# antonilo/unsupervised_detection

Measured on AMD Instinct MI355X. Metric: frame-pairs/sec per adversarial step, DAVIS 480p batch4, 1/2/4/8 GPU, higher is better.
Workload: dtype f32

## Files before the change

include/udet_debug.h:

```cpp
#ifndef UDET_DEBUG_H
#define UDET_DEBUG_H
#include <stddef.h>
#ifdef __cplusplus
extern "C" {
#endif
void udet_debug_force_conv(int bm, int bn, int ks);
void udet_debug_conv_fp16(int on);
void udet_debug_conv_fp16_grad_scale(float s);
void udet_debug_force_wgrad(int nsplit, int dma);
int udet_debug_last_wgrad(void);
int udet_debug_last_wgrad_reduce(void);
int udet_debug_conv2d_backward_filter_ex(const float* x, int ldx, int x_coff, const float* dy, int ldy, int y_coff, const float* y_saved, int act,
                                         float alpha, const float* w, const float* b, const float* gamma, float bn_c, float* dw, float* db,
                                         float* dgamma, float* dbeta, int n, int h, int wd, int cin, int cout, int k, int stride, int dilation,
                                         int up, void* workspace, size_t workspace_bytes, void* stream);
void udet_debug_upb_min_pixels(long v);
void udet_debug_set_tuning(int on);
void udet_debug_force_pair(int on);
int udet_debug_last_pair(void);
int udet_debug_conv2d_pair(const float* xa, const float* xb, const float* wa, const float* wb, const float* ba, const float* bb, float* ya, float* yb,
                           int na, int nb, int h, int w, int cin, int cout, int k, int stride, int dilation, int act, float alpha, void* workspace,
                           size_t workspace_bytes, void* stream);
#define UDET_DEBUG_UPCONV_WSETS_OFFSET 6400
size_t udet_debug_upconv_lowres_workspace_bytes(int ldx, int cin, int cout);
int udet_debug_upconv_lowres_fwd(const float* x, int ldx, const float* w, const float* bias, int act, float alpha, float* y, int ldy, int y_coff,
                                 float* xhat, int n, int h, int wd, int cin, int cout, int split, void* workspace, size_t workspace_bytes,
                                 void* stream);
int udet_debug_upconv_lowres_bwd(const float* dy, int ldy, int y_coff, const float* w, float* dx, int ldx, float* dxhat, int n, int h, int wd,
                                 int cin, int cout, void* workspace, size_t workspace_bytes, void* stream);
int udet_debug_upconv_tables(int h, int w, int backward, int* nseg, int* seg, int* seg_tap, int* taps, int taps_cap, int* ntaps);
int udet_debug_max_segs(void);
int udet_debug_last_conv(void);
#ifdef __cplusplus
}
#endif
#endif
```

unsupervised_detection_amd/_devel.py:

```python
from __future__ import annotations

import ctypes
import os

from ._ffi import check as _check, lib as _lib

_PATH = os.path.join(os.path.dirname(os.path.abspath(__file__)), "libudet_debug.so")
if not os.path.exists(_PATH):
    raise RuntimeError(f"{_PATH} is missing: build it with `make -C unsupervised_detection_amd/csrc`")
dbg = ctypes.CDLL(_PATH, mode=ctypes.RTLD_GLOBAL)
dbg.udet_debug_force_conv.restype = None
dbg.udet_debug_force_conv.argtypes = [ctypes.c_int, ctypes.c_int, ctypes.c_int]
dbg.udet_debug_last_conv.restype = ctypes.c_int
dbg.udet_debug_last_conv.argtypes = []
dbg.udet_debug_conv_fp16.restype = None
dbg.udet_debug_conv_fp16.argtypes = [ctypes.c_int]
dbg.udet_debug_conv_fp16_grad_scale.restype = None
dbg.udet_debug_conv_fp16_grad_scale.argtypes = [ctypes.c_float]
dbg.udet_debug_force_wgrad.restype = None
dbg.udet_debug_force_wgrad.argtypes = [ctypes.c_int, ctypes.c_int]
dbg.udet_debug_upb_min_pixels.restype = None
dbg.udet_debug_upb_min_pixels.argtypes = [ctypes.c_long]
dbg.udet_debug_set_tuning.restype = None
dbg.udet_debug_set_tuning.argtypes = [ctypes.c_int]
dbg.udet_debug_last_wgrad.restype = ctypes.c_int
dbg.udet_debug_last_wgrad.argtypes = []
dbg.udet_debug_force_pair.restype = None
dbg.udet_debug_force_pair.argtypes = [ctypes.c_int]
dbg.udet_debug_last_pair.restype = ctypes.c_int
dbg.udet_debug_last_pair.argtypes = []
dbg.udet_debug_conv2d_pair.restype = ctypes.c_int
dbg.udet_debug_conv2d_pair.argtypes = [ctypes.c_void_p] * 8 + [ctypes.c_int] * 10 + [ctypes.c_float, ctypes.c_void_p, ctypes.c_size_t, ctypes.c_void_p]
dbg.udet_debug_last_wgrad_reduce.restype = ctypes.c_int
dbg.udet_debug_last_wgrad_reduce.argtypes = []
_p, _i, _f = ctypes.c_void_p, ctypes.c_int, ctypes.c_float
dbg.udet_debug_conv2d_backward_filter_ex.restype = ctypes.c_int
dbg.udet_debug_conv2d_backward_filter_ex.argtypes = ([_p, _i, _i, _p, _i, _i, _p, _i, _f, _p, _p, _p, _f, _p, _p, _p, _p] + [_i] * 9
                                                     + [_p, ctypes.c_size_t, _p])
UPCONV_WSETS_OFFSET = 6400
dbg.udet_debug_upconv_lowres_workspace_bytes.restype = ctypes.c_size_t
dbg.udet_debug_upconv_lowres_workspace_bytes.argtypes = [_i, _i, _i]
dbg.udet_debug_upconv_lowres_fwd.restype = ctypes.c_int
dbg.udet_debug_upconv_lowres_fwd.argtypes = [_p, _i, _p, _p, _i, _f, _p, _i, _i, _p] + [_i] * 6 + [_p, ctypes.c_size_t, _p]
dbg.udet_debug_upconv_lowres_bwd.restype = ctypes.c_int
dbg.udet_debug_upconv_lowres_bwd.argtypes = [_p, _i, _i, _p, _p, _i, _p] + [_i] * 5 + [_p, ctypes.c_size_t, _p]
dbg.udet_debug_upconv_tables.restype = ctypes.c_int
dbg.udet_debug_upconv_tables.argtypes = [_i, _i, _i] + [_p] * 4 + [_i, _p]
dbg.udet_debug_max_segs.restype = ctypes.c_int
dbg.udet_debug_max_segs.argtypes = []


def upconv_tables(h: int, w: int, backward: bool):
    cap = 1024
    nseg, ntaps = ctypes.c_int(0), ctypes.c_int(0)
    seg, seg_tap, taps = (ctypes.c_int * 64)(), (ctypes.c_int * 17)(), (ctypes.c_int * (3 * cap))()
    st = dbg.udet_debug_upconv_tables(h, w, 1 if backward else 0, ctypes.addressof(nseg), ctypes.addressof(seg), ctypes.addressof(seg_tap),
                                      ctypes.addressof(taps), cap, ctypes.addressof(ntaps))
    _check(st)
    ns, nt = nseg.value, ntaps.value
    return dict(nseg=ns, seg=[tuple(seg[4 * s:4 * s + 4]) for s in range(ns)], seg_tap=list(seg_tap[:ns + 1]),
                taps=[tuple(taps[3 * t:3 * t + 3]) for t in range(nt)])
```

unsupervised_detection_amd/csrc/common.h:

```cpp
#pragma once
#include <hip/hip_runtime.h>
#include <hip/hip_ext.h>
#include <stdint.h>
#include <stdio.h>
#include <string>

#include "../../include/udet.h"

namespace udet {

void set_error(const char* fmt, ...);
int hip_fail(hipError_t e, const char* what);
#define UDET_HIP(x)                                   \
  do {                                                \
    hipError_t _e = (x);                              \
    if (_e != hipSuccess) return udet::hip_fail(_e, #x); \
  } while (0)
#define UDET_TRY(x)            \
  do {                         \
    int _s = (x);              \
    if (_s != 0) return _s;    \
  } while (0)

struct LaunchSink {
  hipEvent_t* ev;
  int n, cap;
};
extern thread_local LaunchSink* g_launch_sink;
bool launch_sink_next(hipEvent_t* a, hipEvent_t* b);
#define UDET_LAUNCH(kernel, grid, block, shmem, stream, ...)                                             \
  do {                                                                                                   \
    hipEvent_t ea_, eb_;                                                                                 \
    if (udet::g_launch_sink && udet::launch_sink_next(&ea_, &eb_))                                       \
      hipExtLaunchKernelGGL(kernel, grid, block, shmem, stream, ea_, eb_, 0, __VA_ARGS__);               \
    else                                                                                                 \
      hipLaunchKernelGGL(kernel, grid, block, shmem, stream, __VA_ARGS__);                               \
  } while (0)

enum Act { ACT_NONE = UDET_ACT_NONE, ACT_LEAKY = UDET_ACT_LEAKY, ACT_ELU = UDET_ACT_ELU };

__device__ __forceinline__ float elu_negative(float v) {
  const float e = __expf(v) - 1.0f;
  const float t = v * (1.f + v * (0.5f + v * (0.16666667f + v * (0.041666668f + v * (0.0083333338f + v * 0.0013888889f)))));
  return v > -0.25f ? t : e;
}
__device__ __forceinline__ float act_fwd(float v, int act, float alpha) {
  const float slope = act == ACT_LEAKY ? alpha : 1.f;
  float r = v > 0.f ? v : v * slope;
  if (act == ACT_ELU) r = v > 0.f ? v : elu_negative(v);
  return r;
}
__device__ __forceinline__ float act_dfo(float a, int act, float alpha) {
  const float ue = act == ACT_ELU ? 1.f : 0.f, us = act == ACT_LEAKY ? alpha : 1.f;
  return a > 0.f ? 1.f : fmaf(a, ue, us);
}

#define UDET_MAX_TAPS 49
struct ConvTap {
  int dy, dx, widx;
};

struct FastDiv {
  unsigned d, mul, sh;
};
inline FastDiv make_fastdiv(unsigned d) {
  FastDiv f;
  f.d = d; f.mul = 0; f.sh = 0;
  if (d > 1) {
    unsigned l = 0;
    while ((1u << l) < d) ++l;
    const unsigned long long pw = 1ull << (31 + l);
    f.mul = (unsigned)((pw + d - 1) / d);
    f.sh = l - 1;
  }
  return f;
}
__device__ __forceinline__ unsigned fdiv(unsigned n, const FastDiv& f) { return f.d == 1 ? n : (__umulhi(n, f.mul) >> f.sh); }

__host__ __device__ __forceinline__ constexpr int xcd_tile_order(int bid, int nwg) {
  const int q = nwg >> 3, r = nwg & 7, xcd = bid & 7, idx = bid >> 3;
  return (xcd < r ? xcd * (q + 1) : r * (q + 1) + (xcd - r) * q) + idx;
}
constexpr bool xcd_tile_order_permutes(int nwg) {
  unsigned long long seen = 0;
  for (int b = 0; b < nwg; ++b) {
    const int l = xcd_tile_order(b, nwg);
    if (l < 0 || l >= nwg || ((seen >> l) & 1)) return false;
    seen |= 1ull << l;
  }
  return true;
}
static_assert(xcd_tile_order_permutes(1) && xcd_tile_order_permutes(7) && xcd_tile_order_permutes(8), "xcd_tile_order");
static_assert(xcd_tile_order_permutes(9) && xcd_tile_order_permutes(13) && xcd_tile_order_permutes(64), "xcd_tile_order");
static_assert(xcd_tile_order(1, 13) == 2 && xcd_tile_order(8, 13) == 1 && xcd_tile_order(5, 13) == 10, "xcd 0..4 of 13 hold two tiles, 5..7 one");

struct ConvSeg {
  int oy, ox;
  int h, w;
  int prow0;
  FastDiv fd_hw, fd_w;
};
#define UDET_MAX_SEGS 16

struct ConvParams {
  const float* x;
  int ldx, x_coff;
  int N, H, W;
  int up_shift;
  const float* xa;
  int xact;
  float xalpha;
  const float* wp;
  int Kc, ldw;
  const float* bias;
  float* y;
  int ldy, y_coff, Cout;
  int OH, OW;
  int OHq, OWq;
  int osy, osx, ooy, oox;
  int isy, isx;
  int ntaps;
  ConvTap taps[UDET_MAX_TAPS];
  int ncls;
  int cls_tap[5];
  int nseg;
  ConvSeg seg[UDET_MAX_SEGS];
  int seg_tap[UDET_MAX_SEGS + 1];
  const ConvTap* tap_tab;
  int Mall;
  FastDiv fd_ohw, fd_ow;
  int kfast;
  const float* zero16;
  int act;
  float alpha;
  const float* res;
  int ldres, res_coff;
  float* y2;
  int ldy2, y2_coff;
  int accumulate;
  float* uo;
  int ldu, u_coff;
  const float* ua;
  int ldua, ua_coff, uact;
  float ualpha;
  int u_c0, u_c1;
  int ksplit;
  float* partial;
  size_t partial_cap;
  int ldp;
  int fold;
  int* tickets;
  int tail_full, tail_ks, tail_prow0;
  int f16;
  float f16_xscale;
  const float* wino_u;
  int wino_np;
  int kreal;
};
#define UDET_MAX_TICKETS 4096

int launch_conv(ConvParams& p, hipStream_t stream);
int launch_conv_pair(ConvParams& a, ConvParams& b, hipStream_t stream);
int launch_tap_gather(const ConvParams& g, const float* z, int ldz, hipStream_t stream);

struct PackJob {
  long src_off, dst_off, gamma_off, beta_off;
  long total;
  int T, R, C, Kc, ldw, k_split, k_gap, mode;
};

struct WgradParams {
  const float* x;
  int ldx, x_coff;
  int N, H, W, up_shift;
  int Cin;
  const float* dy;
  const float* ya;
  int ldy, y_coff, Cout;
  int yact;
  float yalpha;
  int OH, OW, isy, isx;
  int ycls, OHf, OWf;
  int ntaps;
  ConvTap taps[UDET_MAX_TAPS];
  float* dw;
  float* db;
  float* partial;
  size_t partial_floats;
  const float* zero16;
  int swapped, oCin, oCout, bias_m;
  int Cin4, Mpad;
  float* pbias;
  FastDiv fd_ohw, fd_ow;
  const float* w;
  const float* b;
  const float* gamma;
  float* dgamma;
  float* dbeta;
  float bn_c;
  int f16;
  float f16_yscale;
};
int launch_wgrad_T(WgradParams& p, int T, hipStream_t stream);
int launch_wgrad_up_T(const WgradParams& q, int H, int W, hipStream_t stream);
int launch_bn_finalize(float* dw, int T, int Cin, int Cout, const float* w, const float* b, const float* gamma, float bn_c, float* pd,
                       float* db, float* dgamma, float* dbeta, hipStream_t stream);
int launch_wgrad_up_combine(const float* deff, float* dw, int Cin, int Cout, hipStream_t stream);
size_t wgrad_partial_floats_needed(int T, int Cin, int Cout);

}
```

unsupervised_detection_amd/csrc/conv_igemm.hip:

```cpp
#include "conv_igemm_common.h"

namespace udet {

#define UDET_TILE_ROW(BM, BN, WM, WN) {BM, BN},
const int CONV_GEMM_TILES[CONV_GEMM_NTILES][2] = {UDET_GEMM_TILES(UDET_TILE_ROW)};
#undef UDET_TILE_ROW
bool conv_gemm_tile(int bm, int bn) {
  for (auto& t : CONV_GEMM_TILES)
    if (bm == t[0] && bn == t[1]) return true;
  return false;
}

int conv_xblocks(const ConvParams& p, int bm) {
  if (p.nseg == 0) return p.ncls * ((p.N * p.OHq * p.OWq + bm - 1) / bm);
  int x = 0;
  for (int s = 0; s < p.nseg; ++s) x += (p.N * p.seg[s].h * p.seg[s].w + bm - 1) / bm;
  return x;
}

static int launch_cfg(ConvParams& p, const ConvCfg& c, hipStream_t stream) {
  const int Mtot = p.N * p.OHq * p.OWq;
  dim3 grid(conv_xblocks(p, c.bm), (p.Cout + c.bn - 1) / c.bn, p.ksplit > 1 ? p.ksplit : 1);
  if (p.tail_ks > 1) {
    const int mtiles = (Mtot + c.bm - 1) / c.bm;
    p.tail_prow0 = (p.tail_full / mtiles) * Mtot + (p.tail_full % mtiles) * c.bm;
    grid.x = p.tail_full + (grid.x - p.tail_full) * p.tail_ks;
    grid.z = 1;
  }
  if (c.family == FAM_SELF_STAGING) UDET_TRY(launch_igemm_self(p, c.bm, c.bn, p.f16 != 0, grid, stream));
  else if (is_lds_dma(c.family)) UDET_TRY(launch_igemm_ring(p, c.bm, c.bn, c.family == FAM_DMA2 ? 2 : (c.family == FAM_DMA3 ? 3 : 4), p.f16 != 0, grid, stream));
  else UDET_TRY(launch_igemm_staged(p, c.bm, c.bn, c.family != FAM_PLAIN, grid, stream));
  if (p.tail_ks > 1) UDET_TRY(launch_splitk_tail_pass(p, stream));
  else if (p.ksplit > 1 && !p.fold) UDET_TRY(launch_splitk_second_pass(p, stream));
  return UDET_OK;
}

static int launch_pair_cfg(ConvParams& a, ConvParams& b, const ConvCfg& c, hipStream_t stream) {
  ConvPair pp;
  pp.p[0] = a; pp.p[1] = b;
  pp.xa = conv_xblocks(a, c.bm);
  dim3 grid(pp.xa + conv_xblocks(b, c.bm), (a.Cout + c.bn - 1) / c.bn, a.ksplit > 1 ? a.ksplit : 1);
  UDET_TRY(launch_igemm_ring_pair(pp, c.bm, c.bn, c.family == FAM_DMA3 ? 3 : 2, grid, stream));
  if (a.ksplit > 1) UDET_TRY(launch_splitk_pair_pass(pp, stream));
  return UDET_OK;
}

int launch_conv_gemm(ConvParams& p, const ConvCfg& c, hipStream_t stream) {
  if (!conv_gemm_tile(c.bm, c.bn)) return no_gemm_tile("conv", c.bm, c.bn);
  p.ksplit = c.ks > 1 ? c.ks : 1;
  p.fold = 0;
  p.tail_full = 0; p.tail_ks = 0; p.tail_prow0 = 0;
  if (p.ksplit > 1) {
    p.ldp = (p.Cout + 3) & ~3;
    p.fold = c.fold && p.tickets && cfg_tiles(p, c.bm, c.bn) <= UDET_MAX_TICKETS;
    const int Mtot = p.N * p.OHq * p.OWq, mtiles = (Mtot + c.bm - 1) / c.bm, xb = p.ncls * mtiles;
    if (c.tail > 0 && c.tail < xb && !p.nseg && is_lds_dma(c.family) && !(reinterpret_cast<uintptr_t>(p.partial) & 15)) {
      const long prow0 = (long)(c.tail / mtiles) * Mtot + (long)(c.tail % mtiles) * c.bm;
      if ((size_t)((long)p.ncls * Mtot - prow0) * p.ldp * p.ksplit <= p.partial_cap) {
        p.tail_full = c.tail; p.tail_ks = p.ksplit; p.ksplit = 1; p.fold = 0;
      }
    }
  }
  return launch_cfg(p, c, stream);
}

int launch_conv_gemm_pair(ConvParams& a, ConvParams& b, const ConvCfg& c, hipStream_t stream) {
  if (!conv_gemm_tile(c.bm, c.bn)) return no_gemm_tile("conv pair", c.bm, c.bn);
  const int cap = pair_max_ksplit(a, b);
  const int ks = c.ks > cap ? cap : (c.ks < 1 ? 1 : c.ks);
  for (ConvParams* q : {&a, &b}) {
    q->ksplit = ks; q->fold = 0; q->tail_full = 0; q->tail_ks = 0; q->tail_prow0 = 0;
    q->ldp = (q->Cout + 3) & ~3;
  }
  float* const base = a.partial;
  if (ks > 1) {
    if ((reinterpret_cast<uintptr_t>(base) & 15) != 0) { set_error("conv pair: unaligned split-K scratch"); return UDET_ERR_ALIGN; }
    size_t off = (size_t)ks * a.Mall * a.ldp;
    off = (off + 15) & ~(size_t)15;
    b.partial = base + off;
  }
  const int rc = launch_pair_cfg(a, b, c, stream);
  b.partial = base;
  return rc;
}

}
```

unsupervised_detection_amd/csrc/conv_igemm_ring.h:

```cpp
#pragma once
#include "conv_igemm_common.h"

namespace udet {

template <int BM, int BN, int WAVES_M, int WAVES_N, int NS, bool F16>
__device__ __forceinline__ void conv_igemm_dma_body(const ConvParams& p, const int bid_x, const int grid_x) {
  static_assert(NS >= 2 && NS <= 4, "stages");
  static_assert(WAVES_M * WAVES_N == 4, "4 MFMA waves");
  constexpr int BK = 32;
  constexpr int WTM = BM / WAVES_M, WTN = BN / WAVES_N;
  constexpr int TM = WTM / 32, TN = WTN / 32;
  static_assert(TM * 32 == WTM && TN * 32 == WTN && BM % 32 == 0, "tile");
  constexpr int A_LD = BM / 32;
  constexpr int B_F4_ROW = BN / 4;
  constexpr int B_LD = BK * B_F4_ROW / 256;
  static_assert(B_LD * 256 == BK * B_F4_ROW, "BK*BN/4 must be a multiple of 256");
  typedef __attribute__((address_space(3))) void* lds_ptr;

  __shared__ __attribute__((aligned(16))) float As[NS][BM][BK];
  __shared__ __attribute__((aligned(16))) float Bs[NS][BK][BN];
  __shared__ int rowoff[BM];
  __shared__ int2 tap_yx[UDET_MAX_TAPS];
  __shared__ int tap_w[UDET_MAX_TAPS];
  __shared__ int s_last;

  IGEMM_STAMP(0);
  const int tid = threadIdx.x;
  int spec_dy = 0, spec_dx = 0, spec_widx = 0;
  if (tid < UDET_MAX_TAPS) {
    spec_dy = p.taps[tid].dy;
    spec_dx = p.taps[tid].dx;
    spec_widx = p.taps[tid].widx;
  }
  const int role = __builtin_amdgcn_readfirstlane(tid >> 8);
  const int t = tid & 255;
  const int lane = t & 63, wave = __builtin_amdgcn_readfirstlane(t >> 6);
  const int wm = wave / WAVES_N, wn = wave % WAVES_N;
  const int li = lane & 31, lh = lane >> 5;

  int bid = bid_x;
  int kz = blockIdx.z, knz = p.ksplit;
  {
    int nwg = grid_x;
    if (p.tail_ks > 1) {
      nwg = p.tail_full;
      knz = 1;
      if (bid >= p.tail_full) {
        const int r = bid - p.tail_full;
        kz = r % p.tail_ks;
        bid = p.tail_full + r / p.tail_ks;
        knz = p.tail_ks;
      }
    }
    if (bid < nwg) {
      const int q = nwg >> 3, r = nwg & 7, xcd = bid & 7, idx = bid >> 3;
      bid = (xcd < r ? xcd * (q + 1) : r * (q + 1) + (xcd - r) * q) + idx;
    }
  }
  const TileCls tc = tile_cls<BM>(p, bid);
  const int OHWq = tc.OHWq, Mtot = tc.Mtot , m0 = tc.m0, tap0 = tc.tap0, ntc = tc.ntc, ooy = tc.ooy, oox = tc.oox;
  const int n0 = blockIdx.y * BN;
  const int Hs = p.H >> p.up_shift, Ws = p.W >> p.up_shift;
  IGEMM_STAMP(6);

  if (p.nseg == 0 && tap0 == 0) {
    if (tid < ntc) {
      tap_yx[tid] = make_int2(spec_dy, spec_dx);
      tap_w[tid] = spec_widx;
    }
  } else {
    for (int i = tid; i < ntc; i += 512) {
      const ConvTap tp = conv_tap(p, tap0 + i);
      tap_yx[i] = make_int2(tp.dy, tp.dx);
      tap_w[i] = tp.widx;
    }
  }
  const int Kc = p.Kc;
  const int tsh = Kc == 4 ? 3 : (Kc == 8 ? 2 : 1);
  const int tps = (p.kfast & 4) ? 1 << tsh : 1;
  const int nchunks = (p.kfast & 1) ? ntc * ((Kc + 31) >> 5) : ((p.kfast & 4) ? (ntc + tps - 1) >> tsh : (ntc * Kc + BK - 1) / BK);
  int c_begin = 0, c_end = nchunks;
  if (knz > 1) {
    c_begin = (int)((unsigned)(nchunks * kz) / (unsigned)knz);
    c_end = (int)((unsigned)(nchunks * (kz + 1)) / (unsigned)knz);
  }
  const long slab_off = p.tail_ks > 1 ? ((long)kz * (p.Mall - p.tail_prow0) - p.tail_prow0) * p.ldp : (long)kz * p.Mall * p.ldp;
  IGEMM_STAMP(7);

  if (role == 1) {
    __builtin_amdgcn_s_setprio(3);
    const int kq = lane & 7;
    const int kqs = kq ^ ((wave * 4 + (lane >> 4)) & 7);
    int a_base[A_LD], a_iy0[A_LD], a_ix0[A_LD];
#pragma unroll
    for (int j = 0; j < A_LD; ++j) {
      const int m = m0 + j * 32 + wave * 8 + (lane >> 3);
      if (m < Mtot) {
        const int n = (int)fdiv(m, tc.fd_ohw), rem = m - n * OHWq;
        const int qy = (int)fdiv(rem, tc.fd_ow), qx = rem - qy * tc.OWq;
        a_base[j] = n * Hs * Ws;
        a_iy0[j] = qy * p.isy;
        a_ix0[j] = qx * p.isx;
      } else {
        a_base[j] = 0;
        a_iy0[j] = -(1 << 28);
        a_ix0[j] = 0;
      }
    }
    const float* zero = p.zero16;
    const KOrder ko = korder(Kc, ntc);
    KCursor ka, kb[B_LD];
    ka.blk = ka.tap = ka.c = ka.w = 0;
#pragma unroll
    for (int j = 0; j < B_LD; ++j) kb[j] = ka;
    if (!(p.kfast & 5)) {
      ka = kc_init(ko, c_begin * BK + kqs * 4);
#pragma unroll
      for (int j = 0; j < B_LD; ++j) kb[j] = kc_init(ko, c_begin * BK + (t + j * 256) / B_F4_ROW);
    }
    auto issue_generic = [&](int buf) {
      int dy = 0, dx = 0;
      const bool a_ok = kc_valid(ko, ka);
      const int a_c = kc_chan(ko, ka);
      if (a_ok) {
        const int2 yx = tap_yx[ka.tap];
        dy = yx.x;
        dx = yx.y;
      }
#pragma unroll
      for (int j = 0; j < A_LD; ++j) {
        int iy = a_iy0[j] + dy, ix = a_ix0[j] + dx;
        const bool ok = a_ok && (unsigned)iy < (unsigned)p.H && (unsigned)ix < (unsigned)p.W;
        iy >>= p.up_shift;
        ix >>= p.up_shift;
        const float* src = ok ? p.x + ((size_t)(a_base[j] + iy * Ws + ix) * p.ldx + p.x_coff + a_c) : zero;
        __builtin_amdgcn_global_load_lds(src, (lds_ptr)&As[buf][j * 32 + wave * 8][0], 16, 0, 0);
      }
#pragma unroll
      for (int j = 0; j < B_LD; ++j) {
        const int c4 = (t + j * 256) % B_F4_ROW;
        const int n = n0 + c4 * 4;
        const bool ok = kc_valid(ko, kb[j]) && n < p.ldw;
        const int wi = ok ? tap_w[kb[j].tap] : 0;
        const float* src = ok ? p.wp + (((size_t)wi * Kc + kc_chan(ko, kb[j])) * p.ldw + n) : zero;
        __builtin_amdgcn_global_load_lds(src, (lds_ptr)(&Bs[buf][0][0] + (j * 256 + wave * 64) * 4), 16, 0, 0);
      }
      kc_advance(ko, ka, BK);
#pragma unroll
      for (int j = 0; j < B_LD; ++j) kc_advance(ko, kb[j], BK);
    };
    int a_off[A_LD];
#pragma unroll
    for (int j = 0; j < A_LD; ++j)
      a_off[j] = a_iy0[j] < -(1 << 27) ? 0 : (a_base[j] + a_iy0[j] * Ws + a_ix0[j]) * p.ldx + p.x_coff + kqs * 4;
    int b_off[B_LD], b_row[B_LD];
    bool b_col[B_LD];
#pragma unroll
    for (int j = 0; j < B_LD; ++j) {
      const int idx = t + j * 256, row = idx / B_F4_ROW, n = n0 + (idx - row * B_F4_ROW) * 4;
      b_row[j] = row;
      b_off[j] = row * p.ldw + n;
      b_col[j] = n < p.ldw;
    }
    int s_blk = c_begin == 0 ? 0 : __builtin_amdgcn_readfirstlane(c_begin / (ntc > 0 ? ntc : 1));
    int s_tap = __builtin_amdgcn_readfirstlane(c_begin - s_blk * ntc);
    auto issue_fast = [&](int buf) {
      const int2 yx = tap_yx[s_tap];
      const int dy = yx.x, dx = yx.y, c0 = s_blk << 5;
      const int tap_off = (dy * Ws + dx) * p.ldx + c0;
      const bool ch_ok = c0 + kqs * 4 < Kc;
#pragma unroll
      for (int j = 0; j < A_LD; ++j) {
        const int iy = a_iy0[j] + dy, ix = a_ix0[j] + dx;
        const bool ok = ch_ok && (unsigned)iy < (unsigned)p.H && (unsigned)ix < (unsigned)p.W;
        const float* src = ok ? p.x + (a_off[j] + tap_off) : zero;
        __builtin_amdgcn_global_load_lds(src, (lds_ptr)&As[buf][j * 32 + wave * 8][0], 16, 0, 0);
      }
      const float* wrow = p.wp + ((size_t)tap_w[s_tap] * Kc + c0) * p.ldw;
#pragma unroll
      for (int j = 0; j < B_LD; ++j) {
        const bool ok = b_col[j] && c0 + b_row[j] < Kc;
        const float* src = ok ? wrow + b_off[j] : zero;
        __builtin_amdgcn_global_load_lds(src, (lds_ptr)(&Bs[buf][0][0] + (j * 256 + wave * 64) * 4), 16, 0, 0);
      }
      if (++s_tap == ntc) { s_tap = 0; ++s_blk; }
    };
    const int ksh = Kc == 4 ? 2 : (Kc == 8 ? 3 : 4);
    const int a_sub = (kqs * 4) >> ksh, a_ch = (kqs * 4) - (a_sub << ksh);
    int b_sub[B_LD], b_poff[B_LD];
#pragma unroll
    for (int j = 0; j < B_LD; ++j) {
      b_sub[j] = b_row[j] >> ksh;
      b_poff[j] = (b_row[j] - (b_sub[j] << ksh)) * p.ldw + (b_off[j] - b_row[j] * p.ldw);
    }
    auto issue_pack = [&](int buf, int s_stage) {
      const int ta = s_stage * tps + a_sub;
      const bool ta_ok = ta < ntc;
      const int2 yx = tap_yx[ta_ok ? ta : 0];
      const int dy = yx.x, dx = yx.y;
      const int tap_off = (dy * Ws + dx) * p.ldx + a_ch - kqs * 4;
#pragma unroll
      for (int j = 0; j < A_LD; ++j) {
        const int iy = a_iy0[j] + dy, ix = a_ix0[j] + dx;
        const bool ok = ta_ok && (unsigned)iy < (unsigned)p.H && (unsigned)ix < (unsigned)p.W;
        const float* src = ok ? p.x + (a_off[j] + tap_off) : zero;
        __builtin_amdgcn_global_load_lds(src, (lds_ptr)&As[buf][j * 32 + wave * 8][0], 16, 0, 0);
      }
#pragma unroll
      for (int j = 0; j < B_LD; ++j) {
        const int tb = s_stage * tps + b_sub[j];
        const bool ok = b_col[j] && tb < ntc;
        const float* src = ok ? p.wp + ((size_t)tap_w[ok ? tb : 0] * Kc * p.ldw + b_poff[j]) : zero;
        __builtin_amdgcn_global_load_lds(src, (lds_ptr)(&Bs[buf][0][0] + (j * 256 + wave * 64) * 4), 16, 0, 0);
      }
// ... 136 lines not shown
```

unsupervised_detection_amd/csrc/conv_igemm_self.hip:

```cpp
#include "conv_igemm_dma.h"

namespace udet {

template <int BM, int BN, int WAVES_M, int WAVES_N, bool F16 = false>
__global__ __launch_bounds__(256, 3) void conv_igemm_dma4_kernel(const ConvParams p) {
  static_assert(WAVES_M * WAVES_N == 4, "4 waves");
  constexpr int BK = 16;
  constexpr int WTM = BM / WAVES_M, WTN = BN / WAVES_N;
  constexpr int TM = WTM / 32, TN = WTN / 32;
  static_assert(TM * 32 == WTM && TN * 32 == WTN && BM % 64 == 0 && BN % 32 == 0, "tile");
  using Lane = DmaLane<BM, BN, BK>;
  constexpr int B_LD = Lane::B_LD;

  __shared__ __attribute__((aligned(16))) float As[2][BM][BK];
  __shared__ __attribute__((aligned(16))) float Bs[2][BK][BN];
  __shared__ int rowoff[BM];
  __shared__ int2 tap_yx[UDET_MAX_TAPS];
  __shared__ int tap_w[UDET_MAX_TAPS];
  __shared__ int s_last;

  const int t = threadIdx.x;
  const int lane = t & 63, wave = __builtin_amdgcn_readfirstlane(t >> 6);
  const int wm = wave / WAVES_N, wn = wave % WAVES_N;
  const int li = lane & 31, lh = lane >> 5;

  const int bid = xcd_tile_order(blockIdx.x, gridDim.x);
  const TileCls tc = tile_cls<BM>(p, bid);
  const int Mtot = tc.Mtot , m0 = tc.m0, ntc = tc.ntc;
  const int n0 = blockIdx.y * BN;
  const int Hs = p.H >> p.up_shift, Ws = p.W >> p.up_shift;

  fill_tap_tables<256>(p, tc, tap_yx, tap_w, t);
  fill_rowoff<BM, 256>(p, tc, rowoff, t);
  const int Kc = p.Kc;
  const bool kfast = (p.kfast & 2) != 0;
  const int nchunks = kfast ? ntc * ((Kc + 15) >> 4) : (ntc * Kc + BK - 1) / BK;
  int c_begin, c_end;
  k_slice(nchunks, blockIdx.z, p.ksplit, c_begin, c_end);
  __syncthreads();

  Lane ln;
  dma_lane_init(ln, p, tc, t, lane, wave, n0, Hs, Ws);
  const KOrder ko = korder(Kc, ntc);
  ln.ka = kc_init(ko, kfast ? 0 : c_begin * BK + ln.kqs * 4);
#pragma unroll
  for (int j = 0; j < B_LD; ++j) ln.kb[j] = kc_init(ko, kfast ? 0 : c_begin * BK + (t + j * 256) / Lane::B_F4_ROW);
  const int ntc_ = ntc > 0 ? ntc : 1;
  int s_blk = __builtin_amdgcn_readfirstlane(c_begin / ntc_);
  int s_tap = __builtin_amdgcn_readfirstlane(c_begin - s_blk * ntc_);
  auto issue = [&](int buf) {
    if (kfast) dma_issue_fast<true>(p, ln, tap_yx, tap_w, As, Bs, buf, ntc, s_blk, s_tap);
    else dma_issue_generic<true>(p, ln, ko, tap_yx, tap_w, As, Bs, buf);
  };
  auto meet = [&]() {
    asm volatile("s_waitcnt vmcnt(0) lgkmcnt(0)" ::: "memory");
    __builtin_amdgcn_s_barrier();
    asm volatile("" ::: "memory");
  };

  floatx16 acc[TM][TN];
  acc_zero(acc);
  const float xscale = F16 ? p.f16_xscale : 1.f;

  if (c_begin < c_end) issue(0);
  meet();
  {
    int buf = 0;
    for (int c = c_begin; c < c_end; ++c) {
      if (c + 1 < c_end) issue(buf ^ 1);
      dma_compute_chunk<TM, TN, WTM, WTN, F16>(As, Bs, buf, acc, wm, wn, li, lh, xscale);
      meet();
      buf ^= 1;
    }
  }
  if constexpr (F16) acc_unscale(acc, xscale);
  igemm_store<TM, TN, WTM, WTN>(p, acc, rowoff, wm, wn, li, lh, n0, tc.prow0 + m0, Mtot, p.ksplit > 1,
                                (long)blockIdx.z * p.Mall * p.ldp, xpose_scratch<sizeof(As), sizeof(Bs)>(&As[0][0][0], &Bs[0][0][0], wave));
  if (p.ksplit > 1 && p.fold) splitk_fold<BM, BN, 256>(p, rowoff, &s_last, t, n0, tc.prow0 + m0, Mtot, blockIdx.y * gridDim.x + bid);
}

constexpr int self_waves_m(int bm, int bn) { return (bm % 64 == 0 && bn % 64 == 0 && bm <= 128) ? 2 : ((bn == 32 && bm % 128 == 0) ? 4 : 0); }
template <int BM, int BN, bool F16>
static void launch_self(const ConvParams& p, dim3 grid, hipStream_t stream) {
  constexpr int WM = self_waves_m(BM, BN);
  if constexpr (WM != 0) UDET_LAUNCH((conv_igemm_dma4_kernel<BM, BN, WM, 4 / WM, F16>), grid, dim3(256), 0, stream, p);
}
bool conv_self_staging_tile(int bm, int bn) { return conv_gemm_tile(bm, bn) && self_waves_m(bm, bn) != 0; }

int launch_igemm_self(const ConvParams& p, int bm, int bn, bool f16, dim3 grid, hipStream_t stream) {
  if (!conv_self_staging_tile(bm, bn)) {
    set_error("conv: no self-staging kernel for tile %dx%d", bm, bn);
    return UDET_ERR_UNSUPPORTED;
  }
#define UDET_TILE_LAUNCH(BM, BN, WM, WN)          \
  if (bm == BM && bn == BN) {                     \
    if (f16) launch_self<BM, BN, true>(p, grid, stream); \
    else launch_self<BM, BN, false>(p, grid, stream);    \
  }
  UDET_GEMM_TILES(UDET_TILE_LAUNCH)
#undef UDET_TILE_LAUNCH
  UDET_HIP(hipGetLastError());
  return UDET_OK;
}

}
```

unsupervised_detection_amd/csrc/conv_igemm_staged.hip:

```cpp
#include "conv_igemm_common.h"

namespace udet {

template <int BM, int BN, int BK, int WAVES_M, int WAVES_N, bool WS>
__global__ __launch_bounds__(WS ? 512 : 256, WS ? 4 : 2) void conv_igemm_kernel(const ConvParams p) {
  static_assert(WAVES_M * WAVES_N == 4, "4 waves");
  constexpr int NT = WS ? 512 : 256;
  constexpr int WTM = BM / WAVES_M, WTN = BN / WAVES_N;
  constexpr int TM = WTM / 32, TN = WTN / 32;
  static_assert(TM * 32 == WTM && TN * 32 == WTN, "wave tile must be a multiple of 32");
  constexpr int KQ = BK / 4;
  constexpr int LDA = BM + 32 / BK;
  constexpr int A_ROWS = 256 / KQ;
  constexpr int A_LD = BM / A_ROWS;
  static_assert(A_LD * A_ROWS == BM, "BM must be a multiple of 256/(BK/4)");
  constexpr int B_F4_ROW = BN / 4;
  constexpr int B_LD = BK * B_F4_ROW / 256;
  static_assert(B_LD * 256 == BK * B_F4_ROW, "BK*BN/4 must be a multiple of 256");

  __shared__ __attribute__((aligned(16))) float As[2][BK][LDA];
  __shared__ __attribute__((aligned(16))) float Bs[2][BK][BN];
  __shared__ int rowoff[BM];
  __shared__ int2 tap_yx[UDET_MAX_TAPS];
  __shared__ int tap_w[UDET_MAX_TAPS];
  __shared__ int s_last;

  const int tid = threadIdx.x;
  const int role = __builtin_amdgcn_readfirstlane(tid >> 8);
  const int t = tid & 255;
  const int lane = t & 63, wave = t >> 6;
  const int wm = wave / WAVES_N, wn = wave % WAVES_N;
  const int li = lane & 31, lh = lane >> 5;

  int bid = blockIdx.x;
  {
    const int nwg = gridDim.x, q = nwg >> 3, r = nwg & 7, xcd = bid & 7, idx = bid >> 3;
    bid = (xcd < r ? xcd * (q + 1) : r * (q + 1) + (xcd - r) * q) + idx;
  }
  const TileCls tc = tile_cls<BM>(p, bid);
  const int OHWq = tc.OHWq, Mtot = tc.Mtot , m0 = tc.m0, tap0 = tc.tap0, ntc = tc.ntc, ooy = tc.ooy, oox = tc.oox;
  const int n0 = blockIdx.y * BN;
  const int Hs = p.H >> p.up_shift, Ws = p.W >> p.up_shift;

  for (int i = tid; i < ntc; i += NT) {
    const ConvTap tp = conv_tap(p, tap0 + i);
    tap_yx[i] = make_int2(tp.dy, tp.dx);
    tap_w[i] = tp.widx;
  }
  for (int r = tid; r < BM; r += NT) {
    const int m = m0 + r;
    int off = -1;
    if (m < Mtot) {
      const int n = (int)fdiv(m, tc.fd_ohw), rem = m - n * OHWq;
      const int qy = (int)fdiv(rem, tc.fd_ow), qx = rem - qy * tc.OWq;
      off = (n * p.OH + qy * p.osy + ooy) * p.OW + qx * p.osx + oox;
    }
    rowoff[r] = off;
  }
  const int a_kq = t % KQ;
  int a_base[A_LD], a_iy0[A_LD], a_ix0[A_LD];
#pragma unroll
  for (int j = 0; j < A_LD; ++j) {
    const int r = t / KQ + j * A_ROWS;
    const int m = m0 + r;
    if (m < Mtot) {
      const int n = (int)fdiv(m, tc.fd_ohw), rem = m - n * OHWq;
      const int qy = (int)fdiv(rem, tc.fd_ow), qx = rem - qy * tc.OWq;
      a_base[j] = n * Hs * Ws;
      a_iy0[j] = qy * p.isy;
      a_ix0[j] = qx * p.isx;
    } else {
      a_base[j] = 0;
      a_iy0[j] = -(1 << 28);
      a_ix0[j] = 0;
    }
  }

  floatx16 acc[TM][TN];
#pragma unroll
  for (int i = 0; i < TM; ++i)
#pragma unroll
    for (int j = 0; j < TN; ++j)
#pragma unroll
      for (int r = 0; r < 16; ++r) acc[i][j][r] = 0.f;

  const int Kc = p.Kc;
  const int nchunks = (ntc * Kc + BK - 1) / BK;
  int c_begin = 0, c_end = nchunks;
  if (p.ksplit > 1) {
    c_begin = (int)((unsigned)(nchunks * blockIdx.z) / (unsigned)p.ksplit);
    c_end = (int)((unsigned)(nchunks * (blockIdx.z + 1)) / (unsigned)p.ksplit);
  }
  const KOrder ko = korder(Kc, ntc);
  KCursor ka = kc_init(ko, c_begin * BK + a_kq * 4), kb[B_LD];
#pragma unroll
  for (int j = 0; j < B_LD; ++j) kb[j] = kc_init(ko, c_begin * BK + (t + j * 256) / B_F4_ROW);
  __syncthreads();

  float4 ra[A_LD], rb[B_LD];
  auto load_chunk = [&]() {
    int dy = 0, dx = 0;
    const bool a_ok = kc_valid(ko, ka);
    const int a_c = kc_chan(ko, ka);
    if (a_ok) {
      const int2 yx = tap_yx[ka.tap];
      dy = yx.x;
      dx = yx.y;
    }
#pragma unroll
    for (int j = 0; j < A_LD; ++j) {
      int iy = a_iy0[j] + dy, ix = a_ix0[j] + dx;
      const bool ok = a_ok && (unsigned)iy < (unsigned)p.H && (unsigned)ix < (unsigned)p.W;
      float4 v = make_float4(0.f, 0.f, 0.f, 0.f);
      if (ok) {
        iy >>= p.up_shift;
        ix >>= p.up_shift;
        const size_t off = (size_t)(a_base[j] + iy * Ws + ix) * p.ldx + p.x_coff + a_c;
        v = *reinterpret_cast<const float4*>(p.x + off);
        if (p.xa) {
          const float4 a = *reinterpret_cast<const float4*>(p.xa + off);
          v.x *= act_dfo(a.x, p.xact, p.xalpha);
          v.y *= act_dfo(a.y, p.xact, p.xalpha);
          v.z *= act_dfo(a.z, p.xact, p.xalpha);
          v.w *= act_dfo(a.w, p.xact, p.xalpha);
        }
      }
      ra[j] = v;
    }
#pragma unroll
    for (int j = 0; j < B_LD; ++j) {
      const int c4 = (t + j * 256) % B_F4_ROW;
      const int n = n0 + c4 * 4;
      float4 v = make_float4(0.f, 0.f, 0.f, 0.f);
      if (kc_valid(ko, kb[j]) && n < p.ldw)
        v = *reinterpret_cast<const float4*>(p.wp + ((size_t)tap_w[kb[j].tap] * Kc + kc_chan(ko, kb[j])) * p.ldw + n);
      rb[j] = v;
    }
    kc_advance(ko, ka, BK);
#pragma unroll
    for (int j = 0; j < B_LD; ++j) kc_advance(ko, kb[j], BK);
  };
  auto store_chunk = [&](int buf) {
#pragma unroll
    for (int j = 0; j < A_LD; ++j) {
      const int r = t / KQ + j * A_ROWS;
      As[buf][a_kq * 4 + 0][r] = ra[j].x;
      As[buf][a_kq * 4 + 1][r] = ra[j].y;
      As[buf][a_kq * 4 + 2][r] = ra[j].z;
      As[buf][a_kq * 4 + 3][r] = ra[j].w;
    }
#pragma unroll
    for (int j = 0; j < B_LD; ++j) {
      const int idx = t + j * 256;
      const int krow = idx / B_F4_ROW, c4 = idx - krow * B_F4_ROW;
      *reinterpret_cast<float4*>(&Bs[buf][krow][c4 * 4]) = rb[j];
    }
  };

  auto compute_chunk = [&](int buf) {
    float a[2][TM], b[2][TN];
    auto frag = [&](int s, int kk) {
#pragma unroll
      for (int i = 0; i < TM; ++i) a[s][i] = As[buf][kk * 2 + lh][wm * WTM + i * 32 + li];
#pragma unroll
      for (int j = 0; j < TN; ++j) b[s][j] = Bs[buf][kk * 2 + lh][wn * WTN + j * 32 + li];
    };
    frag(0, 0);
#pragma unroll
    for (int kk = 0; kk < BK / 2; ++kk) {
      if (kk + 1 < BK / 2) frag((kk + 1) & 1, kk + 1);
#pragma unroll
      for (int i = 0; i < TM; ++i)
#pragma unroll
        for (int j = 0; j < TN; ++j)
          acc[i][j] = __builtin_amdgcn_mfma_f32_32x32x2f32(a[kk & 1][i], b[kk & 1][j], acc[i][j], 0, 0, 0);
      if (kk + 1 < BK / 2) __builtin_amdgcn_sched_group_barrier(0x100, TM + TN, 0);
      __builtin_amdgcn_sched_group_barrier(0x008, TM * TN, 0);
    }
  };

  if constexpr (WS) {
    auto handover = [&]() {
      asm volatile("s_waitcnt lgkmcnt(0)" ::: "memory");
      __builtin_amdgcn_s_barrier();
    };
    if (role == 1) {
      __builtin_amdgcn_s_setprio(3);
      if (c_begin < c_end) {
        load_chunk();
        store_chunk(0);
        if (c_begin + 1 < c_end) load_chunk();
      }
      handover();
      int buf = 0;
// ... 53 lines not shown
```

unsupervised_detection_amd/csrc/conv_select.hip:

```cpp
#include <mutex>

#include "common.h"
#include "conv_select.h"

namespace udet {

struct TileGeoms;
size_t conv_tile_lds_bytes(const ConvParams& p, int th, int cbmax, TileGeoms* gout, bool* big);
int launch_conv_tile(const ConvParams& p, int th, int cbmax, hipStream_t stream);

static int max_class_taps(const ConvParams& p) {
  int mx = 0;
  for (int c = 0; c < p.nseg; ++c) mx = p.seg_tap[c + 1] - p.seg_tap[c] > mx ? p.seg_tap[c + 1] - p.seg_tap[c] : mx;
  if (p.nseg) return mx;
  for (int c = 0; c < p.ncls; ++c) mx = p.cls_tap[c + 1] - p.cls_tap[c] > mx ? p.cls_tap[c + 1] - p.cls_tap[c] : mx;
  return mx;
}
static int ksplit_capacity(const ConvParams& p, size_t floats_per_split) {
  const int nchunks = (max_class_taps(p) * p.Kc + 31) / 32;
  int ks = nchunks / 2 > 64 ? 64 : nchunks / 2;
  while (ks > 1 && floats_per_split * ks > p.partial_cap) --ks;
  return ks < 1 ? 1 : ks;
}
int max_ksplit(const ConvParams& p) { return p.partial ? ksplit_capacity(p, (size_t)p.Mall * ((p.Cout + 3) & ~3)) : 1; }
int pair_max_ksplit(const ConvParams& a, const ConvParams& b) { return ksplit_capacity(a, ((size_t)a.Mall + b.Mall) * ((a.Cout + 3) & ~3) + 64); }
bool tile_ok(const ConvParams& p, int th, int cb) {
  if (p.nseg) return false;
  if (cb == 16 && p.Kc <= 16) return false;
  const size_t b = conv_tile_lds_bytes(p, th, cb, nullptr, nullptr);
  return b > 0 && b <= 96 * 1024 && p.Kc <= 256 && p.Cout <= 256;
}
bool dma_ok(const ConvParams& p) { return p.xa == nullptr && p.zero16 != nullptr && !(reinterpret_cast<uintptr_t>(p.zero16) & 15); }
bool tail_for_rounds(const ConvParams& p, int bm, int bn, int r, int kcap, int* full_x, int* ks) {
  if (p.nseg) return false;
  const int Mtot = p.N * p.OHq * p.OWq, X = p.ncls * ((Mtot + bm - 1) / bm), Y = (p.Cout + bn - 1) / bn;
  const long S = 256L * r, T = (long)X * Y, fullT = T / S * S;
  if (fullT == 0 || fullT == T) return false;
  const int fx = (int)(fullT / Y), rem_x = X - fx;
  if (fx <= 0 || rem_x <= 0) return false;
  long k = S / ((long)rem_x * Y);
  if (k > kcap) k = kcap;
  if (k < 2) return false;
  *full_x = fx;
  *ks = (int)k;
  return true;
}

static int heuristic_ksplit(long tiles, int cap) {
  const int ks = (int)((512 + tiles - 1) / tiles), half = cap / 2 > 0 ? cap / 2 : 1;
  return ks > half ? half : ks;
}
ConvCfg heuristic_cfg(const ConvParams& p) {
  ConvCfg c;
  c.family = FAM_WAVE_SPEC; c.tail = 0;
  if (p.Cout <= 32) { c.bn = 32; c.bm = 256; if (cfg_tiles(p, 256, 32) < 384) c.bm = 128; }
  else if (p.Cout <= 64) { c.bn = 64; c.bm = 128; if (cfg_tiles(p, 128, 64) < 384) c.bm = 64; }
  else if (p.Cout <= 96) { c.bn = 96; c.bm = 128; }
  else { c.bn = 128; c.bm = 128; if (cfg_tiles(p, 128, 128) < 320) { c.bn = 64; if (cfg_tiles(p, 128, 64) < 384) c.bm = 64; } }
  const long tiles = cfg_tiles(p, c.bm, c.bn);
  c.ks = tiles < 256 ? heuristic_ksplit(tiles, max_ksplit(p)) : 1;
  c.fold = 0;
  if (p.f16 && dma_ok(p)) c.family = FAM_DMA2;
  return c;
}
static ConvCfg pair_heuristic(const ConvParams& a, const ConvParams& b) {
  ConvCfg c = heuristic_cfg(b.Mall >= a.Mall ? b : a);
  c.family = FAM_DMA2; c.fold = 0; c.tail = 0;
  const long tiles = cfg_tiles(a, c.bm, c.bn) + cfg_tiles(b, c.bm, c.bn);
  c.ks = tiles < 256 ? heuristic_ksplit(tiles, pair_max_ksplit(a, b)) : 1;
  return c;
}

int run_conv_cfg(ConvParams& p, const ConvCfg& c, hipStream_t stream) {
  if (is_direct(c.family)) {
    p.ksplit = 1; p.fold = 0; p.tail_full = 0; p.tail_ks = 0;
    return c.family == FAM_THIN_K ? launch_conv_thin_k(p, stream) : launch_conv_thin_n(p, stream);
  }
  if (c.family == FAM_WINO) return launch_conv_wino(p, c.wino_variant(), c.ks, stream);
  if (c.family == FAM_TILE) {
    p.ksplit = 1;
    p.fold = 0;
    return launch_conv_tile(p, c.tile_height(), c.tile_channels(), stream);
  }
  return launch_conv_gemm(p, c, stream);
}

static ConvCfg runnable_cfg(const ConvParams& p, ConvCfg c) {
  const bool known = c.family == FAM_TILE ? (c.bm == 4 || c.bm == 8) && (c.bn == 16 || c.bn == 32)
                     : c.family == FAM_WINO ? c.bm >= 0 && c.bm <= 4
                     : is_direct(c.family) || (is_gemm(c.family) && conv_gemm_tile(c.bm, c.bn));
  if (!known) return heuristic_cfg(p);
  const int cap = c.family == FAM_WINO ? 16 : max_ksplit(p);
  if (c.ks < 1) c.ks = 1;
  if (c.ks > cap) { c.ks = cap; c.tail = 0; }
  c.fold = c.fold && p.tickets ? 1 : 0;
  if (c.tail < 0) c.tail = 0;
  if (stages_by_dma(c.family) && !dma_ok(p)) c.family = FAM_WAVE_SPEC;
  if (c.family == FAM_SELF_STAGING && !conv_self_staging_tile(c.bm, c.bn)) c.family = FAM_DMA2;
  if (p.f16 && dma_ok(p) && (c.family == FAM_PLAIN || c.family == FAM_WAVE_SPEC)) c.family = FAM_DMA2;
  if (is_direct(c.family) && (p.f16 || !(c.family == FAM_THIN_K ? conv_thin_k_ok(p) : conv_thin_n_ok(p)))) return heuristic_cfg(p);
  if (c.family == FAM_TILE && !tile_ok(p, c.tile_height(), c.tile_channels())) return heuristic_cfg(p);
  if (c.family == FAM_WINO && (!conv_wino_ok(p) || !conv_wino_variant_ok(p, c.wino_variant()))) return heuristic_cfg(p);
  return c;
}

struct ConvForce {
  int bm = 0, bn = 0, ks = -1, family = -1, fold = -1, tail_rounds = 0;
  bool any() const { return bm || family >= 0 || ks >= 0; }
};
static ConvForce g_force;
void conv_force_config(int bm, int bn, int ks) {
  ConvForce f;
  f.bm = bm & 0xffff; f.bn = bn;
  f.ks = ks < 0 ? ks : (ks & 0xff);
  f.tail_rounds = ks < 0 ? 0 : ((ks >> 8) & 0xff);
  f.fold = (bm >> 20) & 1 ? 0 : ((bm >> 21) & 1 ? 1 : -1);
  static const int BITS[][2] = {{16, FAM_PLAIN}, {17, FAM_DMA2}, {18, FAM_TILE}, {19, FAM_SELF_STAGING},
                                {22, FAM_DMA3}, {23, FAM_DMA4}, {24, FAM_THIN_K}, {25, FAM_WINO}};
  for (auto& b : BITS)
    if (f.family < 0 && ((bm >> b[0]) & 1)) f.family = b[1];
  g_force = f;
}
static void wino_operands_from_packed(ConvParams& p, hipStream_t stream) {
  int d9, w9[9];
  if (p.wino_u || p.f16 || p.xa || p.Kc % 8 != 0 || p.Kc < 8 || !conv_wino_geometry(p, &d9, w9)) return;
  static float* g_wino_scratch = nullptr;
  static size_t g_wino_cap = 0;
  static std::mutex mu;
  std::lock_guard<std::mutex> l(mu);
  const int np9 = conv_wino_np(p.Cout);
  const size_t need = (size_t)(p.Kc / 8) * 16 * 2 * np9 * 4;
  if (need > g_wino_cap) {
    (void)hipStreamSynchronize(stream);
    if (g_wino_scratch) (void)hipFree(g_wino_scratch);
    g_wino_scratch = nullptr; g_wino_cap = 0;
    if (hipMalloc(reinterpret_cast<void**>(&g_wino_scratch), need * sizeof(float)) == hipSuccess) g_wino_cap = need;
  }
  if (g_wino_scratch && launch_wino_from_packed(p, g_wino_scratch, np9, stream) == UDET_OK) { p.wino_u = g_wino_scratch; p.wino_np = np9; }
}
static void apply_forced(ConvParams& p, ConvCfg& c, hipStream_t stream) {
  const ConvForce& f = g_force;
  if (f.bm && f.family != FAM_WINO) { c.bm = f.bm; c.bn = f.bn; }
  if (f.ks >= 0) { c.ks = (f.ks > max_ksplit(p) && f.family != FAM_WINO) ? max_ksplit(p) : f.ks; c.tail = 0; }
  if (f.family >= 0) c.family = f.family;
  if (f.fold >= 0) c.fold = f.fold;
  if (f.tail_rounds > 0) {
    int fx = 0, k = 0;
    if (tail_for_rounds(p, c.bm, c.bn, f.tail_rounds, max_ksplit(p), &fx, &k)) { c.tail = fx; c.ks = c.ks >= 2 ? c.ks : k; c.fold = 0; }
  }
  if (f.family == FAM_TILE) { c.bm = f.bm == 4 ? 4 : 8; c.bn = f.bn == 16 ? 16 : 32; }
  if (f.family == FAM_THIN_K) c.family = conv_thin_k_ok(p) ? FAM_THIN_K : (conv_thin_n_ok(p) ? FAM_THIN_N : heuristic_cfg(p).family);
  if (f.family == FAM_WINO) {
    wino_operands_from_packed(p, stream);
    const int v = (f.bm & 7) == 4 ? 4 : (f.bm & 3);
    if (conv_wino_ok(p) && (conv_wino_variant_ok(p, v) || conv_wino_variant_ok(p, v ^ 1))) {
      c = ConvCfg::wino(conv_wino_variant_ok(p, v) ? v : (v ^ 1), f.ks < 0 ? 1 : c.ks);
    } else c = heuristic_cfg(p);
  }
}

static int g_debug_f16 = 0;
void conv_debug_f16(int on) { g_debug_f16 = on; }
int conv_debug_f16_on() { return g_debug_f16; }
static float g_debug_f16_grad_scale = 0.f;
void conv_debug_f16_grad_scale(float s) { g_debug_f16_grad_scale = s > 0.f ? s : 0.f; }
float conv_debug_f16_grad_scale_now() { return g_debug_f16 ? g_debug_f16_grad_scale : 0.f; }
static int conv_prepare(ConvParams& p) {
  if (g_debug_f16) p.f16 = 1;
  if (p.f16 && !(p.f16_xscale > 0.f)) p.f16_xscale = 1.f;
  if (p.f16 && conv_tuning_on()) p.f16_xscale = 1.f;
  if (p.Kc % 4 != 0 || p.ldx % 4 != 0 || p.x_coff % 4 != 0 || p.ldw % 4 != 0) {
    set_error("conv: Kc=%d ldx=%d x_coff=%d ldw=%d violate the 4-float alignment contract", p.Kc, p.ldx, p.x_coff, p.ldw);
    return UDET_ERR_ALIGN;
  }
  if (p.ntaps < 0 || p.ntaps > UDET_MAX_TAPS) {
    set_error("conv: ntaps=%d out of range", p.ntaps);
    return UDET_ERR_SHAPE;
  }
  if ((reinterpret_cast<uintptr_t>(p.x) | reinterpret_cast<uintptr_t>(p.wp)) & 15) {
    set_error("conv: x / packed weights must be 16-byte aligned");
    return UDET_ERR_ALIGN;
  }
  if (p.nseg) {
    if (p.nseg < 0 || p.nseg > UDET_MAX_SEGS || !p.tap_tab || p.up_shift || p.xa) {
      set_error("conv: malformed segmented launch");
      return UDET_ERR_ARG;
    }
    int prow = 0;
    for (int s = 0; s < p.nseg; ++s) {
      ConvSeg& g = p.seg[s];
      if (g.h < 1 || g.w < 1 || p.seg_tap[s + 1] - p.seg_tap[s] > UDET_MAX_TAPS || p.seg_tap[s + 1] < p.seg_tap[s]) {
        set_error("conv: segment %d is empty or has more than %d taps", s, UDET_MAX_TAPS);
        return UDET_ERR_SHAPE;
      }
      g.prow0 = prow;
      prow += p.N * g.h * g.w;
      g.fd_hw = make_fastdiv((unsigned)(g.h * g.w));
      g.fd_w = make_fastdiv((unsigned)g.w);
    }
    p.Mall = prow;
    p.ncls = 1; p.ntaps = 0; p.cls_tap[0] = p.cls_tap[1] = 0;
    p.OHq = p.seg[0].h; p.OWq = p.seg[0].w;
  } else {
    if (p.ncls != 4) {
      p.ncls = 1;
      p.cls_tap[0] = 0;
      p.cls_tap[1] = p.ntaps;
    }
    p.Mall = p.ncls * p.N * p.OHq * p.OWq;
  }
  p.fd_ohw = make_fastdiv((unsigned)(p.OHq * p.OWq));
  p.fd_ow = make_fastdiv((unsigned)p.OWq);
  p.kfast = 0;
  if (p.up_shift == 0) p.kfast = p.Kc >= 32 ? 3 : ((p.Kc >= 16 ? 2 : 0) | ((p.Kc == 4 || p.Kc == 8 || p.Kc == 16) ? 4 : 0));
  return UDET_OK;
}
static int g_last_cfg = 0;
int conv_last_config() { return g_last_cfg; }
static int config_word(const ConvCfg& c) { return (c.family & 0xff) | ((c.bm & 0xfff) << 8) | ((c.ks & 0xff) << 20); }

int launch_conv(ConvParams& p, hipStream_t stream) {
  UDET_TRY(conv_prepare(p));
  ConvCfg c;
  const uint64_t key = conv_key(p);
  if (!conv_cache_find(key, &c)) {
    if (conv_tuning_on()) {
      c = tune_conv(p, key, stream);
    } else {
      c = heuristic_cfg(p);
      if (!g_force.bm && !p.f16 && conv_thin_n_ok(p)) c.family = FAM_THIN_N;
      else if (!g_force.bm && !p.f16 && conv_thin_k_ok(p)) c.family = FAM_THIN_K;
    }
  }
  apply_forced(p, c, stream);
  c = runnable_cfg(p, c);
  g_last_cfg = config_word(c) | ((c.ks > 1 && c.fold && c.family != FAM_TILE ? 1 : 0) << 28) | ((c.ks > 1 && c.tail > 0 ? 1 : 0) << 29);
  return run_conv_cfg(p, c, stream);
}

static int g_force_pair = -1;
void conv_force_pair(int on) { g_force_pair = on; }
static int g_last_pair = 0;
int conv_last_pair() { return g_last_pair; }
static bool pair_compatible(const ConvParams& a, const ConvParams& b) {
  if (a.nseg || b.nseg || a.f16 || b.f16 || a.up_shift || b.up_shift || !dma_ok(a) || !dma_ok(b)) return false;
  if (a.Kc != b.Kc || a.Cout != b.Cout || a.ldw != b.ldw || a.ntaps != b.ntaps || a.ncls != b.ncls) return false;
  if (a.isy != b.isy || a.isx != b.isx || a.osy != b.osy || a.osx != b.osx || a.kfast != b.kfast) return false;
  if (!a.partial || a.partial != b.partial) return false;
  for (int c = 0; c <= a.ncls; ++c)
    if (a.cls_tap[c] != b.cls_tap[c]) return false;
  for (int t = 0; t < a.ntaps; ++t)
    if (a.taps[t].dy != b.taps[t].dy || a.taps[t].dx != b.taps[t].dx) return false;
  return true;
}
int launch_conv_pair(ConvParams& a, ConvParams& b, hipStream_t stream) {
  g_last_pair = 0;
  UDET_TRY(conv_prepare(a));
  UDET_TRY(conv_prepare(b));
  if (g_force_pair == 0 || (g_force.any() && g_force_pair != 1) || !pair_compatible(a, b)) {
    UDET_TRY(launch_conv(a, stream));
    return launch_conv(b, stream);
  }
  ConvCfg c;
  const uint64_t key = pair_key(a, b);
  if (pair_cache_find(key, &c)) {
    if (c.family >= 0) {
      if (!conv_gemm_tile(c.bm, c.bn) || (c.family != FAM_DMA2 && c.family != FAM_DMA3)) c = pair_heuristic(a, b);
      if (c.ks < 1) c.ks = 1;
    }
  } else {
    c = conv_tuning_on() ? tune_conv_pair(a, b, key, stream) : pair_heuristic(a, b);
  }
  if (g_force_pair == 1 && c.family < 0) c = pair_heuristic(a, b);
  if (c.family < 0) {
    UDET_TRY(launch_conv(a, stream));
    return launch_conv(b, stream);
  }
  g_last_pair = 1;
  g_last_cfg = config_word(c) | (1 << 30);
  return launch_conv_gemm_pair(a, b, c, stream);
}

}
```

unsupervised_detection_amd/csrc/conv_splitk.hip:

```cpp
#include "conv_igemm_common.h"

namespace udet {

template <int SL>
__global__ __launch_bounds__(256) void conv_splitk_epilogue_kernel(const ConvParams p) {
  const int Mall = p.Mall;
  const long total = (long)Mall * p.Cout;
  const int sl = threadIdx.x % SL;
  for (long e = ((long)blockIdx.x * 256 + threadIdx.x) / SL; e < total; e += (long)gridDim.x * (256 / SL)) {
    const int ma = (int)(e / p.Cout), n = (int)(e - (long)ma * p.Cout);
    float v = 0.f;
    const float* src = p.partial + (size_t)ma * p.ldp + n;
    const size_t slab = (size_t)Mall * p.ldp;
    int s = sl;
    for (; s + 3 * SL < p.ksplit; s += 4 * SL) {
      const float a0 = src[(size_t)s * slab], a1 = src[(size_t)(s + SL) * slab];
      const float a2 = src[(size_t)(s + 2 * SL) * slab], a3 = src[(size_t)(s + 3 * SL) * slab];
      v += a0;
      v += a1;
      v += a2;
      v += a3;
    }
    for (; s < p.ksplit; s += SL) v += src[(size_t)s * slab];
#pragma unroll
    for (int d = SL / 2; d > 0; d >>= 1) v += __shfl_xor(v, d, SL);
    if (sl != 0) continue;
    const int off = row_pixel_off(p, ma);
    conv_epilogue(p, off, n, v);
  }
}

__device__ __forceinline__ void splitk_epilogue4_body(const ConvParams& p, const int row0, const int ksplit, const int bid, const int grid) {
  const int nq = p.ldp >> 2;
  const long total = (long)(p.Mall - row0) * nq;
  const size_t slab = (size_t)(p.Mall - row0) * p.ldp;
  const bool vec = epilogue4_out_ok(p);
  for (long e = (long)bid * 256 + threadIdx.x; e < total; e += (long)grid * 256) {
    const int mr = (int)(e / nq), n = (int)(e - (long)mr * nq) * 4;
    const float4 v = splitk_sum4<load4_plain>(p.partial + (size_t)mr * p.ldp + n, slab, ksplit);
    const int off = row_pixel_off(p, row0 + mr);
    if (vec) {
      if (n < p.Cout) conv_epilogue4(p, off, n, v);
      continue;
    }
    if (n < p.Cout) conv_epilogue(p, off, n, v.x);
    if (n + 1 < p.Cout) conv_epilogue(p, off, n + 1, v.y);
    if (n + 2 < p.Cout) conv_epilogue(p, off, n + 2, v.z);
    if (n + 3 < p.Cout) conv_epilogue(p, off, n + 3, v.w);
  }
}
__global__ __launch_bounds__(256) void conv_splitk_epilogue4_kernel(const ConvParams p) {
  const bool tail = p.tail_ks > 1;
  splitk_epilogue4_body(p, tail ? p.tail_prow0 : 0, tail ? p.tail_ks : p.ksplit, blockIdx.x, gridDim.x);
}
__global__ __launch_bounds__(256) void conv_splitk_epilogue4_pair_kernel(const ConvPair pp) {
  const int second = __builtin_amdgcn_readfirstlane((int)blockIdx.x >= pp.xa ? 1 : 0);
  const ConvParams& p = pp.p[second];
  splitk_epilogue4_body(p, 0, p.ksplit, (int)blockIdx.x - (second ? pp.xa : 0), second ? (int)gridDim.x - pp.xa : pp.xa);
}

int launch_splitk_second_pass(const ConvParams& p, hipStream_t stream) {
  const long total = (long)p.Mall * p.Cout;
  const int sl = (p.ksplit >= 16 && total * 16 <= 262144) ? 16 : ((p.ksplit >= 4 && total * 4 <= 262144) ? 4 : 1);
  long nbl = (total * sl + 255) / 256;
  const int nb = (int)(nbl > 4096 ? 4096 : nbl);
  if (sl == 16) UDET_LAUNCH(conv_splitk_epilogue_kernel<16>, dim3(nb), dim3(256), 0, stream, p);
  else if (sl == 4) UDET_LAUNCH(conv_splitk_epilogue_kernel<4>, dim3(nb), dim3(256), 0, stream, p);
  else if (p.ldp % 4 == 0 && !(reinterpret_cast<uintptr_t>(p.partial) & 15)) {
    const long nb4l = ((long)p.Mall * (p.ldp >> 2) + 255) / 256;
    UDET_LAUNCH(conv_splitk_epilogue4_kernel, dim3((int)(nb4l > 4096 ? 4096 : nb4l)), dim3(256), 0, stream, p);
  } else UDET_LAUNCH(conv_splitk_epilogue_kernel<1>, dim3(nb), dim3(256), 0, stream, p);
  UDET_HIP(hipGetLastError());
  return UDET_OK;
}

int launch_splitk_tail_pass(const ConvParams& p, hipStream_t stream) {
  const long nb4l = ((long)(p.Mall - p.tail_prow0) * (p.ldp >> 2) + 255) / 256;
  UDET_LAUNCH(conv_splitk_epilogue4_kernel, dim3((int)(nb4l > 4096 ? 4096 : nb4l)), dim3(256), 0, stream, p);
  UDET_HIP(hipGetLastError());
  return UDET_OK;
}
int launch_splitk_pair_pass(ConvPair& pp, hipStream_t stream) {
  const ConvParams &a = pp.p[0], &b = pp.p[1];
  const long na = ((long)a.Mall * (a.ldp >> 2) + 255) / 256, nb = ((long)b.Mall * (b.ldp >> 2) + 255) / 256;
  pp.xa = (int)(na > 2048 ? 2048 : na);
  const int xb = (int)(nb > 2048 ? 2048 : nb);
  UDET_LAUNCH(conv_splitk_epilogue4_pair_kernel, dim3(pp.xa + xb), dim3(256), 0, stream, pp);
  UDET_HIP(hipGetLastError());
  return UDET_OK;
}

}
```

unsupervised_detection_amd/csrc/conv_thin.hip:

```cpp
#include "common.h"

namespace udet {

__device__ __forceinline__ void thin_epilogue(const ConvParams& p, int off, int n, float v) {
  if (p.bias) v += p.bias[n];
  v = act_fwd(v, p.act, p.alpha);
  if (p.y2) p.y2[(size_t)off * p.ldy2 + p.y2_coff + n] = v;
  if (p.res) v += p.res[(size_t)off * p.ldres + p.res_coff + n];
  float* dst = p.y + (size_t)off * p.ldy + p.y_coff + n;
  if (p.accumulate) v += *dst;
  *dst = v;
  if (p.uo && n >= p.u_c0 && n < p.u_c1)
    p.uo[(size_t)off * p.ldu + p.u_coff + n] = v * act_dfo(p.ua[(size_t)off * p.ldua + p.ua_coff + n], p.uact, p.ualpha);
}

template <int W>
__device__ __forceinline__ void thin_row_fetch(const ConvParams& p, int off0, int nvalid, int n, float (&accv)[W], float (&resv)[W], float (&uav)[W]) {
  const bool emit = p.uo && n >= p.u_c0 && n < p.u_c1;
#pragma unroll
  for (int u = 0; u < W; ++u) {
    const size_t off = (size_t)(off0 + u * p.osx);
    const bool on = u < nvalid;
    accv[u] = (p.accumulate && on) ? p.y[off * p.ldy + p.y_coff + n] : 0.f;
    resv[u] = (p.res && on) ? p.res[off * p.ldres + p.res_coff + n] : 0.f;
// ... 126 lines not shown
  const float* xb = p.x + (size_t)n * p.H * p.W * p.ldx + p.x_coff;
  const float* xt = xs_ + (2 * ty) * PW + tx;
  float a0 = 0.f, a1 = 0.f, b0 = 0.f, b1 = 0.f;
  constexpr int NX = (PIX * (CB / 4) + 255) / 256, NW = (T * CB + 255) / 256;
  float4 rx[NX];
  float2 rw[NW];
  auto fetch = [&](int c0) {
    const int cw = p.Kc - c0 < CB ? p.Kc - c0 : CB, cq = cw >> 2;
#pragma unroll
    for (int j = 0; j < NX; ++j) {
      const int e = t + j * 256;
      const int pix = e / (CB / 4), c4 = e - pix * (CB / 4);
      const int py = pix / PW, px = pix - py * PW;
      const int iy = iy0 + py, ix = ix0 + px;
      float4 v = make_float4(0.f, 0.f, 0.f, 0.f);
      if (e < PIX * (CB / 4) && c4 < cq && (unsigned)iy < (unsigned)p.H && (unsigned)ix < (unsigned)p.W)
        v = *reinterpret_cast<const float4*>(xb + (size_t)(iy * p.W + ix) * p.ldx + c0 + c4 * 4);
      rx[j] = v;
    }
#pragma unroll
    for (int j = 0; j < NW; ++j) {
      const int e = t + j * 256;
      const int tap = e / CB, ci = e - tap * CB;
      float2 w = make_float2(0.f, 0.f);
      if (e < T * CB && ci < cw) {
        const float* wr = p.wp + ((size_t)win.widx_at[tap] * p.Kc + c0 + ci) * p.ldw;
        w = make_float2(wr[0], p.Cout > 1 ? wr[1] : 0.f);
      }
      rw[j] = w;
    }
  };
  auto stash = [&]() {
#pragma unroll
    for (int j = 0; j < NX; ++j) {
      const int e = t + j * 256;
      if (e >= PIX * (CB / 4)) break;
      const int pix = e / (CB / 4), c4 = e - pix * (CB / 4);
      float* d = xs_ + (c4 * 4) * PIXP + pix;
      d[0] = rx[j].x; d[PIXP] = rx[j].y; d[2 * PIXP] = rx[j].z; d[3 * PIXP] = rx[j].w;
    }
#pragma unroll
    for (int j = 0; j < NW; ++j) {
      const int e = t + j * 256;
      if (e < T * CB) ws_[e] = rw[j];
    }
  };
  fetch(0);
  for (int c0 = 0; c0 < p.Kc; c0 += CB) {
    __syncthreads();
    stash();
    __syncthreads();
    if (c0 + CB < p.Kc) fetch(c0 + CB);
#pragma unroll 2
    for (int ci = 0; ci < CB; ++ci) {
      const float* xc = xt + ci * PIXP;
      const float2* wc = ws_ + ci;
      float col[KH + 1][KW];
#pragma unroll
      for (int r = 0; r < KH + 1; ++r)
#pragma unroll
        for (int c = 0; c < KW; ++c) col[r][c] = xc[r * PW + c];
#pragma unroll
      for (int r = 0; r < KH; ++r)
#pragma unroll
        for (int c = 0; c < KW; ++c) {
          const float2 w = wc[(r * KW + c) * CB];
          a0 = fmaf(col[r][c], w.x, a0);
          a1 = fmaf(col[r][c], w.y, a1);
          b0 = fmaf(col[r + 1][c], w.x, b0);
          b1 = fmaf(col[r + 1][c], w.y, b1);
        }
    }
  }
  const int ox = ox0 + tx;
  if (ox >= p.OWq) return;
#pragma unroll
  for (int h = 0; h < 2; ++h) {
    const int oy = oy0 + 2 * ty + h;
    if (oy >= p.OHq) break;
    const int off = (n * p.OH + oy * p.osy + p.ooy) * p.OW + ox * p.osx + p.oox;
    thin_epilogue(p, off, 0, h ? b0 : a0);
    if (p.Cout > 1) thin_epilogue(p, off, 1, h ? b1 : a1);
  }
}
static bool thin_n_window(const ConvParams& p, int* kh, ThinWin* win) {
  if (p.ncls > 1 || p.isy != 1 || p.isx != 1 || p.up_shift != 0 || (p.ntaps != 9 && p.ntaps != 25) || p.Kc % 4) return false;
  const int K = p.ntaps == 9 ? 3 : 5, h = (K - 1) / 2;
  for (int i = 0; i < 25; ++i) win->widx_at[i] = -1;
  for (int t = 0; t < p.ntaps; ++t) {
    const int r = p.taps[t].dy + h, c = p.taps[t].dx + h;
    if (r < 0 || r >= K || c < 0 || c >= K || win->widx_at[r * K + c] >= 0 || p.taps[t].widx < 0) return false;
    win->widx_at[r * K + c] = p.taps[t].widx;
  }
  *kh = K;
  return true;
}

static size_t thin_n_lds(const ConvParams& p, const ThinGeom& g) {
  const size_t pixp = (size_t)(g.PH * g.PW) | 1;
  return (((size_t)THIN_CB * pixp + 1) & ~(size_t)1) * sizeof(float) + (size_t)p.ntaps * THIN_CB * sizeof(float2);
}
static bool thin_n_pick(const ConvParams& p, int* th, ThinGeom* g) {
  const long t8 = (long)p.N * ((p.OHq + 7) / 8) * ((p.OWq + 31) / 32);
  for (int cand : {(t8 < 512 && p.OWq > 32) ? 4 : 8, 8}) {
    thin_geom(p, cand, 256 / cand, g);
    if (thin_n_lds(p, *g) <= 64 * 1024) { *th = cand; return true; }
  }
  return false;
}
bool conv_thin_n_ok(const ConvParams& p) {
  if (p.nseg) return false;
  if (p.Cout > 2 || p.Cout < 1 || p.xa != nullptr || p.Kc % 4 || p.ldw < 2 || p.ntaps < 1 || p.isy != p.isx || p.isy < 1 || p.isy > 2) return false;
  ThinGeom g;
  int th;
  return thin_n_pick(p, &th, &g);
}
int launch_conv_thin_n(const ConvParams& p, hipStream_t stream) {
  ThinGeom g;
  int th = 0;
  if (!conv_thin_n_ok(p) || !thin_n_pick(p, &th, &g)) { set_error("conv_thin_n: launch not eligible"); return UDET_ERR_UNSUPPORTED; }
  {
    int K = 0;
    ThinWin win;
    if (thin_n_window(p, &K, &win)) {
      const int tiles = p.N * ((p.OHq + 15) / 16) * ((p.OWq + 31) / 32);
      if (K == 3) UDET_LAUNCH((conv_thin_nw_kernel<3, 3, 8>), dim3(tiles), dim3(256), 0, stream, p, win);
      else UDET_LAUNCH((conv_thin_nw_kernel<5, 5, 8>), dim3(tiles), dim3(256), 0, stream, p, win);
      UDET_HIP(hipGetLastError());
      return UDET_OK;
    }
  }
  const int tw = 256 / th;
  const size_t lds = thin_n_lds(p, g);
  const int tiles = p.N * ((p.OHq + th - 1) / th) * ((p.OWq + tw - 1) / tw);
  if (th == 8) UDET_LAUNCH(conv_thin_n_kernel<8>, dim3(tiles), dim3(256), lds, stream, p, g);
  else UDET_LAUNCH(conv_thin_n_kernel<4>, dim3(tiles), dim3(256), lds, stream, p, g);
  UDET_HIP(hipGetLastError());
  return UDET_OK;
}

template <int T>
__global__ __launch_bounds__(256) void conv_thin_k_kernel(const ConvParams p, const ThinGeom g) {
  constexpr int TH = 8, TW = 16;
  extern __shared__ __attribute__((aligned(16))) float xs_[];
  float2* xs = reinterpret_cast<float2*>(xs_);
  const int PIX = g.PH * g.PW;
  const int t = threadIdx.x, lane = t & 63, wave = __builtin_amdgcn_readfirstlane(t >> 6);
  const int tiles_x = (p.OWq + TW - 1) / TW, tiles_y = (p.OHq + TH - 1) / TH;
  const int bid = blockIdx.x;
  const int bx = bid % tiles_x, by = (bid / tiles_x) % tiles_y, n = bid / (tiles_x * tiles_y);
  const int oy0 = by * TH, ox0 = bx * TW;
  const int iy0 = oy0 + g.min_dy, ix0 = ox0 + g.min_dx;
  const float* xb = p.x + (size_t)n * p.H * p.W * p.ldx + p.x_coff;
  const int co = blockIdx.y * 64 + lane;
  float w[T][2];
  int toff[T];
#pragma unroll
  for (int i = 0; i < T; ++i) {
    const bool on = i < p.ntaps && co < p.ldw;
    const float* src = p.wp + ((size_t)(i < p.ntaps ? p.taps[i].widx : 0) * p.Kc) * p.ldw + (co < p.ldw ? co : 0);
    w[i][0] = on ? src[0] : 0.f;
    w[i][1] = on ? src[p.ldw] : 0.f;
    toff[i] = i < p.ntaps ? (p.taps[i].dy - g.min_dy) * g.PW + (p.taps[i].dx - g.min_dx) : 0;
  }
  for (int pix = t; pix < PIX; pix += 256) {
    const int py = pix / g.PW, px = pix - py * g.PW;
    const int iy = iy0 + py, ix = ix0 + px;
    float2 v = make_float2(0.f, 0.f);
    if ((unsigned)iy < (unsigned)p.H && (unsigned)ix < (unsigned)p.W) v = *reinterpret_cast<const float2*>(xb + (size_t)(iy * p.W + ix) * p.ldx);
    xs[pix] = v;
  }
  __syncthreads();
  if (co >= p.Cout) return;
  for (int r = 0; r < 2; ++r) {
    const int ty = wave * 2 + r, oy = oy0 + ty;
    if (oy >= p.OHq) break;
    float out[TW];
#pragma unroll
    for (int tx = 0; tx < TW; tx += 4) {
      const float2* xr = xs + ty * g.PW + tx;
      float a0[4] = {0.f, 0.f, 0.f, 0.f}, a1[4] = {0.f, 0.f, 0.f, 0.f};
      if (ox0 + tx < p.OWq) {
#pragma unroll
        for (int i = 0; i < T; ++i) {
          const float2* q = xr + toff[i];
#pragma unroll
          for (int u = 0; u < 4; ++u) {
            const float2 v = q[u];
            a0[u] = fmaf(v.x, w[i][0], a0[u]);
            a1[u] = fmaf(v.y, w[i][1], a1[u]);
          }
        }
      }
#pragma unroll
      for (int u = 0; u < 4; ++u) out[tx + u] = a0[u] + a1[u];
    }
    thin_epilogue_row<TW>(p, (n * p.OH + oy * p.osy + p.ooy) * p.OW + ox0 * p.osx + p.oox, p.OWq - ox0, co, out);
  }
}

template <int KH, int KW>
__global__ __launch_bounds__(256) void conv_thin_kw_kernel(const ConvParams p, const ThinGeom g, const ThinWin win) {
  constexpr int TH = 8, TW = 16, T = KH * KW;
  extern __shared__ __attribute__((aligned(16))) float xs_[];
  float2* xs = reinterpret_cast<float2*>(xs_);
  const int PIX = g.PH * g.PW;
  const int t = threadIdx.x, lane = t & 63, wave = __builtin_amdgcn_readfirstlane(t >> 6);
  const int tiles_x = (p.OWq + TW - 1) / TW, tiles_y = (p.OHq + TH - 1) / TH;
  const int bid = blockIdx.x;
  const int bx = bid % tiles_x, by = (bid / tiles_x) % tiles_y, n = bid / (tiles_x * tiles_y);
  const int oy0 = by * TH, ox0 = bx * TW;
  const int iy0 = oy0 + g.min_dy, ix0 = ox0 + g.min_dx;
  const float* xb = p.x + (size_t)n * p.H * p.W * p.ldx + p.x_coff;
  const int co = blockIdx.y * 64 + lane;
  float w[T][2];
#pragma unroll
  for (int i = 0; i < T; ++i) {
    const float* src = p.wp + ((size_t)win.widx_at[i] * p.Kc) * p.ldw + (co < p.ldw ? co : 0);
    w[i][0] = co < p.ldw ? src[0] : 0.f;
    w[i][1] = co < p.ldw ? src[p.ldw] : 0.f;
  }
  for (int pix = t; pix < PIX; pix += 256) {
    const int py = pix / g.PW, px = pix - py * g.PW;
    const int iy = iy0 + py, ix = ix0 + px;
    float2 v = make_float2(0.f, 0.f);
    if ((unsigned)iy < (unsigned)p.H && (unsigned)ix < (unsigned)p.W) v = *reinterpret_cast<const float2*>(xb + (size_t)(iy * p.W + ix) * p.ldx);
    xs[pix] = v;
  }
  __syncthreads();
  if (co >= p.Cout) return;
  for (int r = 0; r < 2; ++r) {
    const int ty = wave * 2 + r, oy = oy0 + ty;
    if (oy >= p.OHq) break;
    const int off0 = (n * p.OH + oy * p.osy + p.ooy) * p.OW + ox0 * p.osx + p.oox;
    float accv[TW], resv[TW], uav[TW];
    thin_row_fetch<TW>(p, off0, p.OWq - ox0, co, accv, resv, uav);
    float out[TW];
#pragma unroll
    for (int tx = 0; tx < TW; tx += 4) {
      float a0[4] = {0.f, 0.f, 0.f, 0.f}, a1[4] = {0.f, 0.f, 0.f, 0.f};
      if (ox0 + tx < p.OWq) {
        const float2* xr = xs + ty * g.PW + tx;
#pragma unroll
        for (int wr = 0; wr < KH; ++wr) {
          float2 v[KW + 3];
#pragma unroll
          for (int wc = 0; wc < KW + 3; ++wc) v[wc] = xr[wr * g.PW + wc];
#pragma unroll
          for (int wc = 0; wc < KW; ++wc)
#pragma unroll
            for (int u = 0; u < 4; ++u) {
              a0[u] = fmaf(v[wc + u].x, w[wr * KW + wc][0], a0[u]);
              a1[u] = fmaf(v[wc + u].y, w[wr * KW + wc][1], a1[u]);
            }
        }
      }
#pragma unroll
      for (int u = 0; u < 4; ++u) out[tx + u] = a0[u] + a1[u];
    }
    thin_row_apply<TW>(p, off0, p.OWq - ox0, co, out, accv, resv, uav);
  }
}
static bool thin_window(const ConvParams& p, const ThinGeom& g, int* kh, int* kw, ThinWin* win) {
  const int KH = g.PH - 7, KW = g.PW - 15;
  if (!((KH == 3 && KW == 3) || (KH == 5 && KW == 5)) || p.ntaps != KH * KW) return false;
  for (int i = 0; i < 25; ++i) win->widx_at[i] = -1;
  for (int t = 0; t < p.ntaps; ++t) {
    const int pos = (p.taps[t].dy - g.min_dy) * KW + (p.taps[t].dx - g.min_dx);
    if (win->widx_at[pos] >= 0 || p.taps[t].widx < 0) return false;
    win->widx_at[pos] = p.taps[t].widx;
  }
  *kh = KH; *kw = KW;
  return true;
}

bool conv_thin_k_ok(const ConvParams& p) {
  if (p.nseg) return false;
  const int kr = p.kreal > 0 ? p.kreal : p.Kc;
  if (kr != 2 || p.Kc < 2 || p.ldx % 2 || p.x_coff % 2 || (reinterpret_cast<uintptr_t>(p.x) & 7)) return false;
  if (p.ncls == 4 || p.isy != 1 || p.isx != 1 || p.up_shift || p.xa != nullptr || p.ntaps < 1 || p.ntaps > 25 || p.Cout < 32) return false;
  ThinGeom g;
  thin_geom(p, 8, 16, &g);
  return (size_t)g.PH * g.PW * sizeof(float2) <= 32 * 1024;
}
int launch_conv_thin_k(const ConvParams& p, hipStream_t stream) {
  if (!conv_thin_k_ok(p)) { set_error("conv_thin_k: launch not eligible"); return UDET_ERR_UNSUPPORTED; }
  ThinGeom g;
  thin_geom(p, 8, 16, &g);
  const size_t lds = (size_t)g.PH * g.PW * sizeof(float2);
  const dim3 grid(p.N * ((p.OHq + 7) / 8) * ((p.OWq + 15) / 16), (p.Cout + 63) / 64);
  int kh = 0, kw = 0;
  ThinWin win;
  if (thin_window(p, g, &kh, &kw, &win)) {
    if (kh == 3) UDET_LAUNCH((conv_thin_kw_kernel<3, 3>), grid, dim3(256), lds, stream, p, g, win);
    else UDET_LAUNCH((conv_thin_kw_kernel<5, 5>), grid, dim3(256), lds, stream, p, g, win);
    UDET_HIP(hipGetLastError());
    return UDET_OK;
  }
  if (p.ntaps <= 9) UDET_LAUNCH(conv_thin_k_kernel<9>, grid, dim3(256), lds, stream, p, g);
  else UDET_LAUNCH(conv_thin_k_kernel<25>, grid, dim3(256), lds, stream, p, g);
  UDET_HIP(hipGetLastError());
  return UDET_OK;
}

}
```

unsupervised_detection_amd/csrc/conv_tile.hip:

```cpp
#include <type_traits>

#include "common.h"
#include "conv_epilogue.h"

namespace udet {

typedef float floatx16 __attribute__((ext_vector_type(16)));
typedef _Float16 halfx4 __attribute__((ext_vector_type(4)));

__device__ __forceinline__ void tile_epilogue(const ConvParams& p, int off, int n, float v) {
  if (p.bias) v += p.bias[n];
  v = act_fwd(v, p.act, p.alpha);
  if (p.y2) p.y2[(size_t)off * p.ldy2 + p.y2_coff + n] = v;
  if (p.res) v += p.res[(size_t)off * p.ldres + p.res_coff + n];
  float* dst = p.y + (size_t)off * p.ldy + p.y_coff + n;
  if (p.accumulate) v += *dst;
  *dst = v;
  if (p.uo && n >= p.u_c0 && n < p.u_c1)
    p.uo[(size_t)off * p.ldu + p.u_coff + n] = v * act_dfo(p.ua[(size_t)off * p.ldua + p.ua_coff + n], p.uact, p.ualpha);
}

struct TileGeom {
  int min_dy, min_dx, PH, PW;
};
struct TileGeoms {
  TileGeom g[4];
  int cb;
};

typedef float floatx4 __attribute__((ext_vector_type(4)));
#define TILE_MT_BIG 16
#define TILE_MW_BIG 3
#define TILE_MT_SMALL 8
#define TILE_MW_SMALL 2
template <int NW> struct TileAcc;
template <> struct TileAcc<32> { floatx16 v; };
template <> struct TileAcc<16> { floatx4 v[2]; };

template <int TH, int NW, int TILE_MT, int TILE_MW, bool F16 = false>
__global__ __launch_bounds__(256) void conv_tile_kernel(const ConvParams p, const TileGeoms gs) {
  constexpr int TW = 32;
  constexpr int TM = TH / 4;
  constexpr int NG = 64 / NW;
  constexpr int NQ4 = NW / 4;
  extern __shared__ __attribute__((aligned(16))) float4 smem4[];
  const int cls = blockIdx.z;
  const TileGeom g = gs.g[cls];
  const int tap0 = p.cls_tap[cls], ntc = p.cls_tap[cls + 1] - tap0;
  const int ooy = p.ncls > 1 ? (cls >> 1) : p.ooy, oox = p.ncls > 1 ? (cls & 1) : p.oox;
  const int PIX = g.PH * g.PW;
  const int PIXP = PIX | 1;
  const int CB = p.Kc < gs.cb ? p.Kc : gs.cb;
  const int CQB = CB >> 2;
  float4* T4 = smem4;
  float4* W4 = smem4 + (size_t)CQB * PIXP;
  int* tapoff = reinterpret_cast<int*>(W4 + ((size_t)ntc * CQB + NG) * NW);
  int* pixoff = tapoff + ntc;
  int* qoff = pixoff + PIX;

  const int t = threadIdx.x, lane = t & 63, wave = t >> 6;
  const int col = lane & (NW - 1), grp = lane / NW;
  const int tiles_x = (p.OWq + TW - 1) / TW, tiles_y = (p.OHq + TH - 1) / TH;
  const int bid = blockIdx.x;
  const int tx = bid % tiles_x, ty = (bid / tiles_x) % tiles_y, n = bid / (tiles_x * tiles_y);
  const int oy0 = ty * TH, ox0 = tx * TW;
  const int n0 = blockIdx.y * NW;
  const int iy0 = oy0 * p.isy + g.min_dy, ix0 = ox0 * p.isx + g.min_dx;
  const int Hs = p.H >> p.up_shift, Ws = p.W >> p.up_shift;
  const float* xb = p.x + (size_t)n * Hs * Ws * p.ldx + p.x_coff;

  for (int i = t; i < ntc; i += 256) tapoff[i] = (p.taps[tap0 + i].dy - g.min_dy) * g.PW + (p.taps[tap0 + i].dx - g.min_dx);
  for (int pix = t; pix < PIX; pix += 256) {
    const int py = pix / g.PW, px = pix - py * g.PW;
    const int iy = iy0 + py, ix = ix0 + px;
    int o = -1;
    if ((unsigned)iy < (unsigned)p.H && (unsigned)ix < (unsigned)p.W) o = ((iy >> p.up_shift) * Ws + (ix >> p.up_shift)) * p.ldx;
    pixoff[pix] = o;
  }

  TileAcc<NW> acc[TM];
#pragma unroll
  for (int i = 0; i < TM; ++i) {
    if constexpr (NW == 32) {
#pragma unroll
      for (int r = 0; r < 16; ++r) acc[i].v[r] = 0.f;
    } else {
#pragma unroll
      for (int h = 0; h < 2; ++h)
#pragma unroll
        for (int r = 0; r < 4; ++r) acc[i].v[h][r] = 0.f;
    }
  }
  int abase[TM];
#pragma unroll
  for (int i = 0; i < TM; ++i) abase[i] = ((wave * TM + i) * p.isy) * g.PW + col * p.isx;
  const int ahalf = 16 * p.isx;
  const float xscale = F16 ? p.f16_xscale : 1.f;

  float4 tv[TILE_MT];
  float4 wv[TILE_MW][4];
  auto fetch = [&](int c0, int cw) {
    const int cq = cw >> 2, NQ = ntc * cq;
    const int cq_shift = (cq & (cq - 1)) == 0 ? __builtin_ctz(cq) : -1;
#pragma unroll
    for (int u = 0; u < TILE_MT; ++u) {
      const int e = t + u * 256;
      tv[u] = make_float4(0.f, 0.f, 0.f, 0.f);
      if (e < PIX * cq) {
        const int pix = cq_shift >= 0 ? e >> cq_shift : e / cq, c4 = e - pix * cq;
        const int o = pixoff[pix];
        if (o >= 0) tv[u] = *reinterpret_cast<const float4*>(xb + (size_t)o + c0 + c4 * 4);
      }
    }
#pragma unroll
    for (int u = 0; u < TILE_MW; ++u) {
      const int e = t + u * 256;
      wv[u][0] = wv[u][1] = wv[u][2] = wv[u][3] = make_float4(0.f, 0.f, 0.f, 0.f);
      if (e < NQ * NQ4) {
        const int n4 = e % NQ4, q = e / NQ4;
        const int tap = cq_shift >= 0 ? q >> cq_shift : q / cq, c4 = q - tap * cq;
        const int nn = n0 + n4 * 4;
        if (nn < p.ldw) {
          const float* src = p.wp + ((size_t)p.taps[tap0 + tap].widx * p.Kc + c0 + c4 * 4) * p.ldw + nn;
          wv[u][0] = *reinterpret_cast<const float4*>(src);
          wv[u][1] = *reinterpret_cast<const float4*>(src + p.ldw);
          wv[u][2] = *reinterpret_cast<const float4*>(src + 2 * (size_t)p.ldw);
          wv[u][3] = *reinterpret_cast<const float4*>(src + 3 * (size_t)p.ldw);
        }
      }
    }
  };
  auto commit = [&](int cw) {
    const int cq = cw >> 2, NQ = ntc * cq;
    const int cq_shift = (cq & (cq - 1)) == 0 ? __builtin_ctz(cq) : -1;
#pragma unroll
    for (int u = 0; u < TILE_MT; ++u) {
      const int e = t + u * 256;
      if (e < PIX * cq) {
        const int pix = cq_shift >= 0 ? e >> cq_shift : e / cq, c4 = e - pix * cq;
        T4[(size_t)c4 * PIXP + pix] = tv[u];
      }
    }
#pragma unroll
    for (int u = 0; u < TILE_MW; ++u) {
      const int e = t + u * 256;
      if (e < NQ * NQ4) {
        const int n4 = e % NQ4, q = e / NQ4;
        float4* d = W4 + (size_t)q * NW + n4 * 4;
        d[0] = make_float4(wv[u][0].x, wv[u][1].x, wv[u][2].x, wv[u][3].x);
        d[1] = make_float4(wv[u][0].y, wv[u][1].y, wv[u][2].y, wv[u][3].y);
        d[2] = make_float4(wv[u][0].z, wv[u][1].z, wv[u][2].z, wv[u][3].z);
        d[3] = make_float4(wv[u][0].w, wv[u][1].w, wv[u][2].w, wv[u][3].w);
      }
    }
    for (int e = t; e < NG * NW; e += 256) W4[(size_t)NQ * NW + e] = make_float4(0.f, 0.f, 0.f, 0.f);
    for (int q = t; q < NQ + 3 * NG; q += 256) {
      int o = 0;
      if (q < NQ) {
        const int tap = cq_shift >= 0 ? q >> cq_shift : q / cq, c4 = q - tap * cq;
        o = c4 * PIXP + tapoff[tap];
      }
      qoff[q] = o;
    }
  };

  for (int c0 = -CB; c0 < p.Kc; c0 += CB) {
    const int cw = c0 < 0 ? CB : (p.Kc - c0 < CB ? p.Kc - c0 : CB);
    const int cq = cw >> 2, NQ = ntc * cq;
    __syncthreads();
    if (c0 >= 0) {
      commit(cw);
      __syncthreads();
    }
    if (c0 + CB < p.Kc) fetch(c0 + CB, p.Kc - (c0 + CB) < CB ? p.Kc - (c0 + CB) : CB);
    if (c0 < 0) continue;

    constexpr int NA = NW == 32 ? TM : 2 * TM;
    const int steps = (NQ + NG - 1) / NG;
    int q = grp;
    int off1 = qoff[q + NG];
    float4 b = W4[(size_t)q * NW + col];
    float4 a[NA];
    {
      const float4* ta = T4 + qoff[q];
#pragma unroll
      for (int i = 0; i < TM; ++i) {
        if constexpr (NW == 32) {
          a[i] = ta[abase[i]];
        } else {
          a[2 * i] = ta[abase[i]];
          a[2 * i + 1] = ta[abase[i] + ahalf];
        }
      }
    }
    for (int j = 0; j < steps; ++j) {
      float4 bn = b, an[NA];
#pragma unroll
      for (int i = 0; i < NA; ++i) an[i] = a[i];
      int off2 = 0;
      if (j + 1 < steps) {
        q += NG;
        off2 = qoff[q + NG];
        bn = W4[(size_t)q * NW + col];
        const float4* ta = T4 + off1;
#pragma unroll
        for (int i = 0; i < TM; ++i) {
          if constexpr (NW == 32) {
            an[i] = ta[abase[i]];
          } else {
            an[2 * i] = ta[abase[i]];
            an[2 * i + 1] = ta[abase[i] + ahalf];
          }
        }
      }
      if constexpr (F16) {
        const halfx4 bh = halfx4{(_Float16)b.x, (_Float16)b.y, (_Float16)b.z, (_Float16)b.w};
#pragma unroll
        for (int i = 0; i < TM; ++i) {
          if constexpr (NW == 32) {
// ... 34 lines not shown
      for (int i = 0; i < NA; ++i) a[i] = an[i];
      off1 = off2;
    }
  }

  if (F16 && xscale != 1.f) {
    const float inv = 1.f / xscale;
#pragma unroll
    for (int i = 0; i < TM; ++i) {
      if constexpr (NW == 32) {
#pragma unroll
        for (int r = 0; r < 16; ++r) acc[i].v[r] *= inv;
      } else {
#pragma unroll
        for (int h = 0; h < 2; ++h)
#pragma unroll
          for (int r = 0; r < 4; ++r) acc[i].v[h][r] *= inv;
      }
    }
  }
  const int nn = n0 + col;
  if (nn >= p.Cout) return;
  const bool plain = !p.y2 && !p.res && !p.accumulate && !p.uo;
  const float bias = p.bias ? p.bias[nn] : 0.f;
  auto rows = [&](auto&& emit) {
#pragma unroll
    for (int i = 0; i < TM; ++i) {
      const int oy = oy0 + wave * TM + i;
      if (oy >= p.OHq) continue;
      const int row = (n * p.OH + oy * p.osy + ooy) * p.OW + oox;
      if constexpr (NW == 32) {
#pragma unroll
        for (int r = 0; r < 16; ++r) {
          const int ox = ox0 + (r & 3) + 8 * (r >> 2) + 4 * grp;
          if (ox < p.OWq) emit(row, ox, acc[i].v[r]);
        }
      } else {
#pragma unroll
        for (int h = 0; h < 2; ++h)
#pragma unroll
          for (int r = 0; r < 4; ++r) {
            const int ox = ox0 + h * 16 + grp * 4 + r;
            if (ox < p.OWq) emit(row, ox, acc[i].v[h][r]);
          }
      }
    }
  };
  const EpiAct ea = epi_act(p);
  if (plain) {
    float* ycol = p.y + p.y_coff + nn;
    const int xstep = p.osx * p.ldy;
    if (p.act == ACT_ELU) rows([&](int row, int ox, float v) { ycol[(size_t)row * p.ldy + (size_t)ox * xstep] = act_fwd_c<true>(v + bias, ea.slope); });
    else rows([&](int row, int ox, float v) { ycol[(size_t)row * p.ldy + (size_t)ox * xstep] = act_fwd_c<false>(v + bias, ea.slope); });
    return;
  }
  const bool emit_u = p.uo && nn >= p.u_c0 && nn < p.u_c1;
  auto generic = [&](auto ELU) {
#pragma unroll
    for (int i = 0; i < TM; ++i) {
      const int oy = oy0 + wave * TM + i;
      if (oy >= p.OHq) continue;
      const int row = (n * p.OH + oy * p.osy + ooy) * p.OW + oox;
      constexpr int NE = NW == 32 ? 16 : 8;
      float rs[NE], ac[NE], ua[NE];
      int off[NE];
#pragma unroll
      for (int e = 0; e < NE; ++e) {
        const int ox = NW == 32 ? ox0 + (e & 3) + 8 * (e >> 2) + 4 * grp : ox0 + (e >> 2) * 16 + grp * 4 + (e & 3);
        off[e] = ox < p.OWq ? row + ox * p.osx : -1;
        rs[e] = ac[e] = ua[e] = 0.f;
        if (off[e] >= 0) {
          if (p.res) rs[e] = p.res[(size_t)off[e] * p.ldres + p.res_coff + nn];
          if (p.accumulate) ac[e] = p.y[(size_t)off[e] * p.ldy + p.y_coff + nn];
          if (emit_u) ua[e] = p.ua[(size_t)off[e] * p.ldua + p.ua_coff + nn];
        }
      }
#pragma unroll
      for (int e = 0; e < NE; ++e) {
        if (off[e] < 0) continue;
        float v;
        if constexpr (NW == 32) v = acc[i].v[e];
        else v = acc[i].v[e >> 2][e & 3];
        v = act_fwd_c<decltype(ELU)::value>(v + bias, ea.slope);
        if (p.y2) p.y2[(size_t)off[e] * p.ldy2 + p.y2_coff + nn] = v;
        if (p.res) v += rs[e];
        if (p.accumulate) v += ac[e];
        p.y[(size_t)off[e] * p.ldy + p.y_coff + nn] = v;
        if (emit_u) p.uo[(size_t)off[e] * p.ldu + p.u_coff + nn] = v * act_dfo_c(ua[e], ea);
      }
    }
  };
  if (p.act == ACT_ELU) generic(std::true_type());
  else generic(std::false_type());
}

size_t conv_tile_lds_bytes(const ConvParams& p, int th, int cbmax, TileGeoms* gout, bool* big) {
  if (big) *big = false;
  if (p.ntaps < 1 || p.xa != nullptr || p.Kc % 4 != 0 || p.isy != p.isx || p.isy < 1 || p.isy > 2) return 0;
  const int ncls = p.ncls > 1 ? p.ncls : 1;
  if (ncls > 4) return 0;
  if (cbmax != 32 && cbmax != 16) return 0;
  if (gout) gout->cb = cbmax;
  const size_t cb = p.Kc < cbmax ? p.Kc : cbmax;
  size_t worst = 0;
  for (int c = 0; c < ncls; ++c) {
    const int t0 = ncls > 1 ? p.cls_tap[c] : 0, t1 = ncls > 1 ? p.cls_tap[c + 1] : p.ntaps;
    int mn_y = 0, mx_y = 0, mn_x = 0, mx_x = 0;
    for (int t = t0; t < t1; ++t) {
      if (t == t0 || p.taps[t].dy < mn_y) mn_y = p.taps[t].dy;
      if (t == t0 || p.taps[t].dy > mx_y) mx_y = p.taps[t].dy;
      if (t == t0 || p.taps[t].dx < mn_x) mn_x = p.taps[t].dx;
      if (t == t0 || p.taps[t].dx > mx_x) mx_x = p.taps[t].dx;
    }
    TileGeom g;
    g.min_dy = mn_y; g.min_dx = mn_x;
    g.PH = (th - 1) * p.isy + (mx_y - mn_y) + 1;
    g.PW = 31 * p.isx + (mx_x - mn_x) + 1;
    if (gout) gout->g[c] = g;
    const size_t pix = (size_t)g.PH * g.PW, ntc = (size_t)(t1 - t0), cqb = cb / 4, nw = p.Cout <= 16 ? 16 : 32;
    const size_t ng = 64 / nw;
    const size_t bytes = (cqb * (pix | 1) + (ntc * cqb + ng) * nw) * 16 + (ntc + pix + ntc * cqb + 3 * ng + 8) * sizeof(float);
    if (pix * cqb > 256 * TILE_MT_BIG || ntc * cqb * (nw / 4) > 256 * TILE_MW_BIG) return 0;
    if (big && (pix * cqb > 256 * TILE_MT_SMALL || ntc * cqb * (nw / 4) > 256 * TILE_MW_SMALL)) *big = true;
    worst = bytes > worst ? bytes : worst;
  }
  return worst;
}

int launch_conv_tile(const ConvParams& p, int th, int cbmax, hipStream_t stream) {
  TileGeoms g;
  bool big = false;
  const size_t lds = conv_tile_lds_bytes(p, th, cbmax, &g, &big);
  if (lds == 0 || lds > 96 * 1024 || (th != 8 && th != 4)) {
    set_error("conv_tile: launch not eligible");
    return UDET_ERR_UNSUPPORTED;
  }
  typedef void (*Kern)(const ConvParams, const TileGeoms);
  static const Kern K[2][2][2] = {
      {{conv_tile_kernel<8, 32, TILE_MT_SMALL, TILE_MW_SMALL>, conv_tile_kernel<8, 32, TILE_MT_BIG, TILE_MW_BIG>},
       {conv_tile_kernel<8, 16, TILE_MT_SMALL, TILE_MW_SMALL>, conv_tile_kernel<8, 16, TILE_MT_BIG, TILE_MW_BIG>}},
      {{conv_tile_kernel<4, 32, TILE_MT_SMALL, TILE_MW_SMALL>, conv_tile_kernel<4, 32, TILE_MT_BIG, TILE_MW_BIG>},
       {conv_tile_kernel<4, 16, TILE_MT_SMALL, TILE_MW_SMALL>, conv_tile_kernel<4, 16, TILE_MT_BIG, TILE_MW_BIG>}}};
  static bool attr_set = false;
  if (!attr_set) {
    for (int a = 0; a < 2; ++a)
      for (int b = 0; b < 2; ++b)
        for (int c = 0; c < 2; ++c)
          (void)hipFuncSetAttribute(reinterpret_cast<const void*>(K[a][b][c]), hipFuncAttributeMaxDynamicSharedMemorySize, 96 * 1024);
    attr_set = true;
  }
  const int tiles = ((p.OWq + 31) / 32) * ((p.OHq + th - 1) / th) * p.N;
  const int ncls = p.ncls > 1 ? p.ncls : 1;
  const bool n16 = p.Cout <= 16;
  dim3 grid(tiles, n16 ? 1 : (p.Cout + 31) / 32, ncls);
  if (p.f16) {
    static const Kern K16[2][2][2] = {
        {{conv_tile_kernel<8, 32, TILE_MT_SMALL, TILE_MW_SMALL, true>, conv_tile_kernel<8, 32, TILE_MT_BIG, TILE_MW_BIG, true>},
         {conv_tile_kernel<8, 16, TILE_MT_SMALL, TILE_MW_SMALL, true>, conv_tile_kernel<8, 16, TILE_MT_BIG, TILE_MW_BIG, true>}},
        {{conv_tile_kernel<4, 32, TILE_MT_SMALL, TILE_MW_SMALL, true>, conv_tile_kernel<4, 32, TILE_MT_BIG, TILE_MW_BIG, true>},
         {conv_tile_kernel<4, 16, TILE_MT_SMALL, TILE_MW_SMALL, true>, conv_tile_kernel<4, 16, TILE_MT_BIG, TILE_MW_BIG, true>}}};
    static bool attr16 = false;
    if (!attr16) {
      for (int a = 0; a < 2; ++a)
        for (int b = 0; b < 2; ++b)
          for (int c = 0; c < 2; ++c)
            (void)hipFuncSetAttribute(reinterpret_cast<const void*>(K16[a][b][c]), hipFuncAttributeMaxDynamicSharedMemorySize, 96 * 1024);
      attr16 = true;
    }
    UDET_LAUNCH(K16[th == 4][n16][big], grid, dim3(256), lds, stream, p, g);
  } else {
    UDET_LAUNCH(K[th == 4][n16][big], grid, dim3(256), lds, stream, p, g);
  }
  UDET_HIP(hipGetLastError());
  return UDET_OK;
}

}
```

unsupervised_detection_amd/csrc/devel/api_debug.hip:

```cpp
#include <string.h>

#include <vector>

#include "../../../include/udet_debug.h"
#include "../conv_host.h"
#include "../plan_run.h"

using namespace udet;

extern "C" {
int udet_debug_last_conv(void) { return conv_last_config(); }
void udet_debug_force_conv(int bm, int bn, int ks) { conv_force_config(bm, bn, ks); }
void udet_debug_conv_fp16(int on) { conv_debug_f16(on); }
void udet_debug_conv_fp16_grad_scale(float s) { conv_debug_f16_grad_scale(s); }
void udet_debug_force_wgrad(int nsplit, int dma) { wgrad_force(nsplit, dma); }
int udet_debug_last_wgrad(void) { return wgrad_last_config(); }
int udet_debug_last_wgrad_reduce(void) { return wgrad_last_reduce(); }
int udet_debug_conv2d_backward_filter_ex(const float* x, int ldx, int x_coff, const float* dy, int ldy, int y_coff, const float* y_saved, int act,
                                         float alpha, const float* w, const float* b, const float* gamma, float bn_c, float* dw, float* db,
                                         float* dgamma, float* dbeta, int n, int h, int wd, int cin, int cout, int k, int stride, int dilation,
                                         int up, void* workspace, size_t workspace_bytes, void* stream_) {
  hipStream_t stream = (hipStream_t)stream_;
  if (!x || !dy || !dw || n < 1 || h < 1 || wd < 1 || cin < 1 || cout < 1 || k < 1 || k * k > UDET_MAX_TAPS || dilation < 1 ||
      (stride != 1 && stride != 2) || up < 0 || up > 2) {
    set_error("debug_backward_filter_ex: bad argument");
    return UDET_ERR_ARG;
  }
  if (ldx % 4 || x_coff % 4 || ldy % 4 || y_coff % 4) {
    set_error("debug_backward_filter_ex: ldx=%d x_coff=%d ldy=%d y_coff=%d must be multiples of 4", ldx, x_coff, ldy, y_coff);
    return UDET_ERR_ALIGN;
  }
  if (x_coff < 0 || y_coff < 0 || x_coff + round_up(cin, 4) > ldx || y_coff + round_up(cout, 4) > ldy) {
    set_error("debug_backward_filter_ex: channel window outside the buffer (x %d+%d of %d, dy %d+%d of %d)", x_coff, cin, ldx, y_coff, cout, ldy);
    return UDET_ERR_SHAPE;
  }
  if (gamma && (!w || !b || !db || !dgamma || !dbeta)) {
    set_error("debug_backward_filter_ex: a BN-folded layer needs w, b, db, dgamma and dbeta");
    return UDET_ERR_ARG;
  }
  if (up == 2 && (!gamma || y_saved || k != 3 || stride != 1 || dilation != 1)) {
    set_error("debug_backward_filter_ex: the class-structured form is a BN-folded 3x3 stride-1 layer on dU");
    return UDET_ERR_ARG;
  }
  if (!workspace || (reinterpret_cast<uintptr_t>(workspace) & 63) || workspace_bytes < 128 * sizeof(float)) {
    set_error("debug_backward_filter_ex: workspace must be 64-byte aligned and hold the zero block");
    return UDET_ERR_ARG;
  }
  float* zero = reinterpret_cast<float*>(workspace);
  const int us = up ? 1 : 0;
  WgradParams p;
  memset(&p, 0, sizeof(p));
  p.x = x; p.ldx = ldx; p.x_coff = x_coff; p.N = n; p.Cin = cin;
  p.dy = dy; p.ldy = ldy; p.y_coff = y_coff; p.Cout = cout;
  if (y_saved && act != UDET_ACT_NONE) { p.ya = y_saved; p.yact = act; p.yalpha = alpha; }
  p.dw = dw; p.db = db;
  p.partial = zero + 64; p.partial_floats = workspace_bytes / sizeof(float) - 64;
  p.zero16 = zero;
  p.f16_yscale = conv_debug_f16_grad_scale_now();
  if (gamma) { p.w = w; p.b = b; p.gamma = gamma; p.dgamma = dgamma; p.dbeta = dbeta; p.bn_c = bn_c; }
  ConvParams g;
  memset(&g, 0, sizeof(g));
  conv_setup_fwd(g, n, h << us, wd << us, k, k, stride, dilation);
  p.H = h << us; p.W = wd << us; p.up_shift = us;
  p.OH = g.OH; p.OW = g.OW; p.isy = p.isx = stride;
  p.ntaps = g.ntaps;
  memcpy(p.taps, g.taps, sizeof(g.taps));
  UDET_HIP(hipMemsetAsync(zero, 0, 64 * sizeof(float), stream));
  if (up == 2) return launch_wgrad_up_T(p, h, wd, stream);
  return launch_wgrad_T(p, k * k, stream);
}
void udet_debug_upb_min_pixels(long v) { plan_debug_upb_min_pixels(v); }
void udet_debug_force_pair(int on) { conv_force_pair(on); }
int udet_debug_last_pair(void) { return conv_last_pair(); }
int udet_debug_conv2d_pair(const float* xa, const float* xb, const float* wa, const float* wb, const float* ba, const float* bb, float* ya, float* yb,
                           int na, int nb, int h, int w, int cin, int cout, int k, int stride, int dilation, int act, float alpha, void* workspace,
                           size_t workspace_bytes, void* stream_) {
  hipStream_t stream = (hipStream_t)stream_;
  if (cin % 8 != 0 || k * k > UDET_MAX_TAPS) { set_error("debug_conv2d_pair: cin must be a multiple of 8"); return UDET_ERR_SHAPE; }
  const int kc = cin, ldw = round_up(cout, 4);
  const size_t wfl = ((size_t)k * k * kc * ldw + 63) & ~(size_t)63, part_fl = (size_t)4 << 20, zero_fl = 64 + UDET_MAX_TICKETS;
  if (workspace_bytes < (2 * wfl + part_fl + zero_fl) * sizeof(float)) { set_error("debug_conv2d_pair: workspace too small"); return UDET_ERR_ARG; }
  float* wpa = reinterpret_cast<float*>(workspace);
  float* wpb = wpa + wfl;
  float* part = wpb + wfl;
  float* zero = part + part_fl;
  UDET_HIP(hipMemsetAsync(zero, 0, zero_fl * sizeof(float), stream));
  UDET_TRY(launch_pack_weights(wa, wpa, k * k, cin, cout, kc, ldw, kc, 0, 0, nullptr, stream));
  UDET_TRY(launch_pack_weights(wb, wpb, k * k, cin, cout, kc, ldw, kc, 0, 0, nullptr, stream));
  ConvParams p[2];
  for (int i = 0; i < 2; ++i) {
    memset(&p[i], 0, sizeof(ConvParams));
    conv_setup_fwd(p[i], i ? nb : na, h, w, k, k, stride, dilation);
    p[i].x = i ? xb : xa; p[i].ldx = cin; p[i].wp = i ? wpb : wpa; p[i].Kc = kc; p[i].ldw = ldw; p[i].bias = i ? bb : ba;
    p[i].y = i ? yb : ya; p[i].ldy = cout; p[i].Cout = cout; p[i].act = act; p[i].alpha = alpha;
    p[i].partial = part; p[i].partial_cap = part_fl; p[i].zero16 = zero; p[i].tickets = reinterpret_cast<int*>(zero + 64);
  }
  return launch_conv_pair(p[0], p[1], stream);
}
}
namespace {
enum { UPC_TICKETS = 64, UPC_JOBS = UPC_TICKETS + UDET_MAX_TICKETS, UPC_JOBS_CAP = 192, UPC_TAB = UPC_JOBS + UPC_JOBS_CAP, UPC_TAB_CAP = 2048,
       UPC_WSETS = UPC_TAB + UPC_TAB_CAP, UPC_MIN_SLAB = 1 << 20 };
static_assert(UPC_WSETS == UDET_DEBUG_UPCONV_WSETS_OFFSET && UPC_WSETS % 64 == 0 && 8 * sizeof(PackJob) <= UPC_JOBS_CAP * sizeof(float), "workspace layout");
size_t upc_align64(size_t v) { return (v + 63) & ~(size_t)63; }
int upc_kct(int cout) { return round_up(cout, cout <= 4 ? 4 : 8); }
size_t upc_floats(int kc, int ldw) { return UPC_WSETS + upc_align64((size_t)4 * 36 * kc * ldw) + UPC_MIN_SLAB; }
int upc_check(const char* who, const void* a, const void* b, const void* c, const void* d, int n, int h, int wd, int cin, int cout, void* workspace,
              size_t workspace_bytes, size_t need_floats) {
  if (!a || !b || !c || !d || n < 1 || cin < 1 || cout < 1) { set_error("%s: bad argument", who); return UDET_ERR_ARG; }
  if (h < 2 || wd < 2) { set_error("%s: the source grid %d x %d must be at least 2 x 2 (one interior row / column and the last one)", who, h, wd); return UDET_ERR_SHAPE; }
  if ((long)n * (2 * h) * (2 * wd) >= (1L << 28)) { set_error("%s: grid too large", who); return UDET_ERR_SHAPE; }
  if (!workspace || (reinterpret_cast<uintptr_t>(workspace) & 63) || workspace_bytes < need_floats * sizeof(float)) {
    set_error("%s: workspace must be 64-byte aligned and hold %zu bytes", who, need_floats * sizeof(float));
    return UDET_ERR_ARG;
  }
  return UDET_OK;
}
int upc_stage(const Layer::SegLaunch& tab, const std::vector<PackJob>& jobs, const float* w, float* ws, hipStream_t stream) {
  if (tab.taps.size() * sizeof(ConvTap) > UPC_TAB_CAP * sizeof(float) || jobs.size() * sizeof(PackJob) > UPC_JOBS_CAP * sizeof(float)) {
    set_error("debug_upconv_lowres: table larger than its workspace slot");
    return UDET_ERR_ARG;
  }
  UDET_HIP(hipMemsetAsync(ws, 0, UPC_JOBS * sizeof(float), stream));
  UDET_HIP(hipMemcpyAsync(ws + UPC_JOBS, jobs.data(), jobs.size() * sizeof(PackJob), hipMemcpyHostToDevice, stream));
  UDET_HIP(hipMemcpyAsync(ws + UPC_TAB, tab.taps.data(), tab.taps.size() * sizeof(ConvTap), hipMemcpyHostToDevice, stream));
  return launch_pack_jobs(reinterpret_cast<const PackJob*>(ws + UPC_JOBS), (int)jobs.size(), w, ws, BN_C, stream);
}
UpbLane upc_lane(float* ws, size_t ws_floats, size_t sets_floats) {
  const size_t off = UPC_WSETS + upc_align64(sets_floats);
  return UpbLane{ws + off, ws_floats - off, ws, reinterpret_cast<int*>(ws + UPC_TICKETS), 0};
}
}
extern "C" {

size_t udet_debug_upconv_lowres_workspace_bytes(int ldx, int cin, int cout) {
  if (ldx < 1 || cin < 1 || cout < 1) return 0;
  const size_t f = upc_floats(ldx, round_up(cout, 4)), b = upc_floats(upc_kct(cout), round_up(cin, 4));
  return (f > b ? f : b) * sizeof(float);
}
int udet_debug_max_segs(void) { return UDET_MAX_SEGS; }

int udet_debug_upconv_lowres_fwd(const float* x, int ldx, const float* w, const float* bias, int act, float alpha, float* y, int ldy, int y_coff,
                                 float* xhat, int n, int h, int wd, int cin, int cout, int split, void* workspace, size_t workspace_bytes,
                                 void* stream_) {
  hipStream_t stream = (hipStream_t)stream_;
  const char* who = "debug_upconv_lowres_fwd";
  if (act != UDET_ACT_NONE && act != UDET_ACT_LEAKY && act != UDET_ACT_ELU) { set_error("%s: bad argument", who); return UDET_ERR_ARG; }
  if (ldx % 4 || ldy % 4 || y_coff % 4) { set_error("%s: ldx=%d ldy=%d y_coff=%d must be multiples of 4", who, ldx, ldy, y_coff); return UDET_ERR_ALIGN; }
  if (ldx < 4 || ldy < 4 || cin > ldx || y_coff < 0 || (cout >= 1 && y_coff + cout > ldy)) {
    set_error("%s: channel window outside the buffer (x %d of %d, y %d+%d of %d)", who, cin, ldx, y_coff, cout, ldy);
    return UDET_ERR_SHAPE;
  }
  if (split && cout > 16) { set_error("%s: the split form is the plan's for cout <= 16 only", who); return UDET_ERR_ARG; }
  Layer L;
  L.cin = cin; L.cout = cout;
  L.Kc = ldx; L.ldw = round_up(cout, 4);
  L.k_split = round_up(cin, cin <= 4 ? 4 : 8); L.k_gap = 0;
  L.upb = true; L.upb_bwd = false; L.upb_split = split != 0;
  L.wupb_off = UPC_WSETS;
  const size_t sets = (size_t)4 * 36 * L.Kc * L.ldw;
  UDET_TRY(upc_check(who, x, w, y, xhat, n, h, wd, cin, cout, workspace, workspace_bytes, upc_floats(L.Kc, L.ldw)));
  float* ws = reinterpret_cast<float*>(workspace);
  build_upb_launches(L, h, wd);
  std::vector<PackJob> jobs;
  PackJob base;
  memset(&base, 0, sizeof(base));
  base.gamma_off = base.beta_off = -1;
  upb_pack_jobs(L, base, jobs);
  int st = upc_stage(L.upb_f, jobs, w, ws, stream);
  if (st == UDET_OK) {
    UpbFwd a;
    a.N = n; a.h = h; a.w = wd;
    a.src = x; a.xhat = xhat; a.ld = ldx;
    a.wsets = ws + L.wupb_off; a.Kc = L.Kc; a.ldw = L.ldw; a.bias = bias;
    a.y = y; a.ldy = ldy; a.y_coff = y_coff; a.cout = cout; a.act = act; a.alpha = alpha;
    a.tab = &L.upb_f; a.tab_dev = reinterpret_cast<const ConvTap*>(ws + UPC_TAB); a.split = L.upb_split;
    a.lane = upc_lane(ws, workspace_bytes / sizeof(float), sets);
    st = upb_forward(a, stream);
  }
  (void)hipStreamSynchronize(stream);
  return st;
}

int udet_debug_upconv_lowres_bwd(const float* dy, int ldy, int y_coff, const float* w, float* dx, int ldx, float* dxhat, int n, int h, int wd,
                                 int cin, int cout, void* workspace, size_t workspace_bytes, void* stream_) {
  hipStream_t stream = (hipStream_t)stream_;
  const char* who = "debug_upconv_lowres_bwd";
  if (ldx % 4 || ldy % 4 || y_coff % 4) { set_error("%s: ldx=%d ldy=%d y_coff=%d must be multiples of 4", who, ldx, ldy, y_coff); return UDET_ERR_ALIGN; }
  const int kct = cout >= 1 ? upc_kct(cout) : 0;
  if (ldx < 4 || ldy < 4 || cin > ldx || y_coff < 0 || y_coff + kct > ldy) {
    set_error("%s: channel window outside the buffer (dy %d+%d of %d, dx %d of %d)", who, y_coff, kct, ldy, cin, ldx);
    return UDET_ERR_SHAPE;
  }
  Layer L;
  L.cin = cin; L.cout = cout;
  L.Kc = ldx; L.ldw = round_up(cout, 4);
  L.k_split = round_up(cin, cin <= 4 ? 4 : 8); L.k_gap = 0;
  L.KcT = kct; L.ldwT = round_up(cin, 4);
  L.upb = true; L.upb_bwd = true;
  L.wupbT_off = UPC_WSETS;
  const size_t sets = (size_t)4 * 36 * L.KcT * L.ldwT;
  UDET_TRY(upc_check(who, dy, w, dx, dxhat, n, h, wd, cin, cout, workspace, workspace_bytes, upc_floats(L.KcT, L.ldwT)));
  float* ws = reinterpret_cast<float*>(workspace);
  build_upb_launches(L, h, wd);
  std::vector<PackJob> all, jobs;
  PackJob base;
  memset(&base, 0, sizeof(base));
  base.gamma_off = base.beta_off = -1;
  upb_pack_jobs(L, base, all);
  for (const PackJob& j : all)
    if (j.mode == 10) jobs.push_back(j);
  int st = upc_stage(L.upb_b, jobs, w, ws, stream);
  if (st == UDET_OK) {
    UpbBwd a;
    a.N = n; a.h = h; a.w = wd;
    a.du = dy; a.lddu = ldy; a.du_coff = y_coff;
    a.wsetsT = ws + L.wupbT_off; a.KcT = L.KcT; a.ldwT = L.ldwT; a.cout = cout;
    a.dxhat = dxhat; a.dsrc = dx; a.ld = ldx; a.cin = cin;
    a.tab = &L.upb_b; a.tab_dev = reinterpret_cast<const ConvTap*>(ws + UPC_TAB);
    a.lane = upc_lane(ws, workspace_bytes / sizeof(float), sets);
    a.f16_xscale = conv_debug_f16_grad_scale_now();
    st = upb_dgrad(a, stream);
  }
  (void)hipStreamSynchronize(stream);
// ... 27 lines not shown
```

unsupervised_detection_amd/csrc/plan.h:

```cpp
#pragma once
#include <map>
#include <string>
#include <vector>

#include "common.h"

namespace udet {

struct ParamDesc {
  std::string name;
  int rank;
  int shape[4];
  size_t offset, count;
};
struct NetParams {
  std::vector<ParamDesc> p;
  size_t total = 0;
  int add(const std::string& name, int a, int b = 0, int c = 0, int d = 0);
  int find(const std::string& name) const;
};
enum { NET_PWC = 0, NET_GEN = 1, NET_REC = 2 };
const NetParams& net_params(int net);

struct Buf {
  std::string name;
  size_t off;
  int n, h, w, ld;
  size_t floats() const { return (size_t)n * h * w * ld; }
};

struct Layer {
  std::string name;
  int net;
  int kh, kw, cin, cout, stride, dil;
  bool transposed = false;
  bool up = false;
  int act = ACT_NONE;
  float alpha = 0.f;
  int w_idx = -1, b_idx = -1, g_idx = -1, be_idx = -1;
  int Kc = 0, ldw = 0, k_split = 0, k_gap = 0;
  size_t wp_off = 0;
  int KcT = 0, ldwT = 0;
  size_t wpT_off = 0;
  size_t bias_f_off = 0, scale_off = 0;
  size_t wu_off = 0, wuT_off = 0;
  size_t wino_off = 0, winoT_off = 0;
  int wino_np = 0, winoT_np = 0;
  bool upb = false;
  bool upb_bwd = false;
  bool upb_split = false;
  int xhat = -1, src = -1;
  size_t wupb_off = 0, wupbT_off = 0;
  struct SegLaunch {
    int nseg = 0;
    ConvSeg seg[UDET_MAX_SEGS];
    int seg_tap[UDET_MAX_SEGS + 1];
    std::vector<ConvTap> taps;
    size_t tab_off = 0;
  } upb_f, upb_b;
  int x = -1, x_coff = 0, y = -1, y_coff = 0;
  int res = -1, res_coff = 0, y2 = -1;
  int H = 0, W = 0;
  bool col2im = false;
  int ldz = 0, zbuf = -1;
  size_t wz_off = 0;
  bool x_in_slab = false, y_fanned_out = false;
  std::string pair_name;
};

struct Resolved {
  struct {
    int pyr[7][3];
    int est[7][5], flow[7], ctx[7][7];
    int up_feat[7], up_flow[7];
  } pwc;
  struct {
    int enc[2][9];
    int deconv[6], flow[6], upflow[6];
  } rec;
  int image, flow, mask, pred, image_next, flow_next, d_mask, flow_full;
  int pwc_x8, pwc_rflow2, pwc_c[7], pwc_slab[7];
  int gen_in, gen_a17, gen_d[18], gen_u[18];
  int rec_imgin, rec_fin, rec_conv6, rec_concat[6], rec_r[7], rec_rf[6], rec_flow[6];
  struct Grad {
    int pred, fin, conv6, u_conv6;
    int flow[6], concat[6], u_concat[6], r[7], rf[6];
    int p[6];
    int enc_du[2][9];
    int enc_dx[2][9], enc_ux[2][9];
  } grad[2];
};

struct Config {
  int batch, in_h, in_w, img_h, img_w;
  float flow_normalizer, cbn, epsilon;
  float lr, beta1, beta2, adam_eps, clip;
  unsigned long long noise_seed;
  int conv_fp16 = 0;
};

struct Plan {
  Config cfg;
  std::vector<Buf> bufs;
  std::map<std::string, int> buf_by_name;
  std::vector<Layer> pwc, gen, rec;
  size_t packed_floats = 0;
  size_t arena_floats = 0;
  enum { NLANE = 6, NCAND = 8, MAXCAND = 32 };
  std::vector<hipStream_t> cand;
  struct Placement {
    hipStream_t main = nullptr;
    hipStream_t lane[NLANE] = {};
    int queue[NLANE] = {};
    int nqueues = 1;
  };
  std::vector<Placement> placements;
  int placed = -1;
  hipEvent_t prefetch_ev = nullptr;
  hipEvent_t grad_ev[3] = {nullptr, nullptr, nullptr};
  bool prefetch_pending = false;
  std::vector<hipEvent_t> ev_pool, ev_pool_prefetch;
  size_t ev_next = 0, ev_next_prefetch = 0;
  bool in_prefetch = false;
  bool concurrent = true;
  bool enc_a_shared = false;
  size_t scratch_off[NLANE] = {}, scratch_floats = 0;
  size_t wgrad_off[NLANE] = {}, wgrad_floats = 0;
  ~Plan();
  size_t small_off = 0;
  size_t ticket_off = 0;
  size_t seg_off[3] = {0, 0, 0};
  size_t jobs_off[3] = {0, 0, 0};
  int njobs[3] = {0, 0, 0};
  struct ProfRec {
    int cat; double flops, bytes; hipEvent_t a, b; std::string name;
    double mfma_scale = 1.0;
    enum { MAXK = 16 };
    hipEvent_t kev[2 * MAXK];
    LaunchSink sink;
  };
  bool profiling = false;
  std::vector<ProfRec*> prof;
  long adam_t = 0;
  int* ovf_host = nullptr;
  hipEvent_t ovf_ev[3] = {nullptr, nullptr, nullptr};
  bool ovf_pending[3] = {false, false, false};
  long ovf_skipped = 0;
  int ovf_report_values = 0, ovf_report_nets = 0;
  bool pwc_packed = false;
  Resolved R;
  int add_buf(const std::string& name, int n, int h, int w, int ld);
  const Buf& buf(int id) const { return bufs[id]; }
  int bid(const std::string& name) const;
};

#define UDET_PACKJOB_CAP(layers) (8 * (layers) + 32)
#define UDET_SMALL_NOISE 256
#define UDET_SMALL_OVF 300
#define UDET_SMALL_SUMS 1024
Plan* plan_build(const Config& cfg);
void plan_debug_upb_min_pixels(long v);
void build_upb_launches(Layer& L, int h, int w);
void upb_pack_jobs(const Layer& L, const PackJob& base, std::vector<PackJob>& jobs);
enum { UDET_KNOB_ENC_A_LANE = 0, UDET_KNOB_REC_DEC_WGRAD_LANE = 1, UDET_KNOB_REC_ENC_WGRAD_LANE = 2, UDET_KNOB_GEN_WGRAD_LATE = 3, UDET_KNOB_NO_WGRAD_WINO = 6, UDET_KNOB_SKIP = 7, UDET_KNOB_NO_PAIRS = 8, UDET_KNOB_COUNT = 12 };
#ifdef UDET_EXPERIMENT
void plan_debug_knob(int id, long v);
long plan_knob(int id);
#else
constexpr long plan_knob(int) { return 0; }
#endif

int plan_init_workspace(Plan* P, float* ws, hipStream_t s);
int plan_pack_pwc(Plan* P, const float* w_pwc, float* ws, hipStream_t s);
int plan_pack_trainable(Plan* P, const float* w_gen, const float* w_rec, float* ws, hipStream_t s);
int plan_pwc_forward(Plan* P, const float* img1, const float* img2, float* ws, hipStream_t s);
int plan_forward(Plan* P, const float* img1, const float* img2, int ncalls, float* ws, hipStream_t s, bool prefetched = false);
int plan_prefetch(Plan* P, const float* img1, const float* img2, float* ws, hipStream_t s);
int plan_prefetch_consume(Plan* P, float* ws, hipStream_t s);
int plan_generator_forward(Plan* P, float* ws, hipStream_t s);
int plan_generator_layers(Plan* P, float* ws, hipStream_t s);
int plan_recover_forward(Plan* P, int ncalls, float* ws, hipStream_t s, bool inputs_prepacked = false, bool skip_enc_a = false, bool enc_a_input_packed = false);
int plan_losses(Plan* P, float* ws, hipStream_t s);
int plan_backward(Plan* P, int which, const float* w_gen, const float* w_rec, float* g_gen, float* g_rec, float* ws, hipStream_t s);
int plan_apply(Plan* P, int net, float* w, float* g, float* m, float* v, float* ws, hipStream_t s);
int plan_check_overflow(Plan* P, bool wait);
void plan_settle_adam_step(Plan* P);
int plan_lane_queues(Plan* P, hipStream_t s, int* queue);
int plan_pin_lanes(Plan* P, hipStream_t main, hipStream_t const* streams, int n);
enum { PROF_CONV_FWD = 0, PROF_CONV_DGRAD = 1, PROF_CONV_WGRAD = 2, PROF_WARP = 3, PROF_CORR = 4, PROF_NCAT = 5 };
void prof_begin(Plan* P, int cat, double flops, double bytes, hipStream_t s, const char* name = "");
void prof_end(Plan* P, hipStream_t s);

}
```

unsupervised_detection_amd/csrc/plan_exec.hip:

```cpp
#include <string.h>

#include "conv_select.h"
#include "elementwise.h"
#include "plan_run.h"

namespace udet {

static double layer_flops(const Layer& L, int N) {
  const int up = L.up ? 1 : 0;
  double oh, ow;
  if (L.transposed) { oh = 2.0 * L.H; ow = 2.0 * L.W; }
  else { oh = (double)(((L.H << up) + L.stride - 1) / L.stride); ow = (double)(((L.W << up) + L.stride - 1) / L.stride); }
  double taps = (double)L.kh * L.kw;
  if (L.transposed) taps /= 4.0;
  return 2.0 * N * oh * ow * L.cout * L.cin * taps;
}
static double layer_bytes(const Layer& L, int N) {
  const int up = L.up ? 1 : 0;
  const double ih = (double)(L.H << up), iw = (double)(L.W << up);
  double oh, ow;
  if (L.transposed) { oh = 2.0 * L.H; ow = 2.0 * L.W; }
  else { oh = (double)(((L.H << up) + L.stride - 1) / L.stride); ow = (double)(((L.W << up) + L.stride - 1) / L.stride); }
  return 4.0 * (N * ih * iw * L.cin + N * oh * ow * L.cout + (double)L.kh * L.kw * L.cin * L.cout + L.cout);
}

static inline bool skip_launch(int kind, int net) {
  const long k = plan_knob(UDET_KNOB_SKIP);
  if (!k) return false;
  const int bit = kind == 2 ? (net == NET_GEN ? 0 : 1) : (kind == 1 ? (net == NET_GEN ? 2 : 3) : (net == NET_PWC ? 4 : (net == NET_GEN ? 5 : 6)));
  return (k >> bit) & 1;
}

static inline int up_off(int parity, int t) { return parity == 0 ? (t == 0 ? -1 : 0) : (t == 0 ? 0 : 1); }
void setup_up_fwd(ConvParams& p, int N, int H, int W) {
  p.N = N; p.H = H; p.W = W;
  p.OH = 2 * H; p.OW = 2 * W; p.OHq = H; p.OWq = W;
  p.osy = p.osx = 2; p.ooy = p.oox = 0; p.isy = p.isx = 1;
  p.ncls = 4; p.ntaps = 16;
  for (int c = 0; c < 4; ++c) {
    p.cls_tap[c] = 4 * c;
    for (int t = 0; t < 4; ++t) {
      ConvTap& tp = p.taps[4 * c + t];
      tp.dy = up_off(c >> 1, t >> 1); tp.dx = up_off(c & 1, t & 1); tp.widx = 4 * c + t;
    }
  }
  p.cls_tap[4] = 16;
}
static void setup_up_dgrad(ConvParams& p, int N, int H, int W) {
  p.N = N; p.H = 2 * H; p.W = 2 * W;
  p.OH = H; p.OW = W; p.OHq = H; p.OWq = W;
  p.osy = p.osx = 1; p.ooy = p.oox = 0; p.isy = p.isx = 2;
  p.ncls = 1; p.ntaps = 16;
  for (int c = 0; c < 4; ++c)
    for (int t = 0; t < 4; ++t) {
      ConvTap& tp = p.taps[4 * c + t];
      tp.dy = (c >> 1) - 2 * up_off(c >> 1, t >> 1); tp.dx = (c & 1) - 2 * up_off(c & 1, t & 1); tp.widx = 4 * c + t;
    }
}

static void fill_segments(ConvParams& p, const Layer::SegLaunch& g, const ConvTap* tab_dev, int first = 0) {
  p.nseg = g.nseg - first;
  memcpy(p.seg, g.seg + first, sizeof(ConvSeg) * p.nseg);
  memcpy(p.seg_tap, g.seg_tap + first, sizeof(int) * (p.nseg + 1));
  p.tap_tab = tab_dev;
}
static void fill_lane(ConvParams& p, const UpbLane& ln, float f16_xscale) {
  p.partial = ln.partial; p.partial_cap = ln.partial_cap;
  p.zero16 = ln.zero16; p.tickets = ln.tickets;
  p.f16 = ln.f16; p.f16_xscale = f16_xscale;
}
int upb_forward(const UpbFwd& a, hipStream_t s) {
  const int h = a.h, w = a.w;
  UDET_TRY(launch_upb_ring(a.src, a.ld, a.N, h, w, a.xhat, s));
  ConvParams p;
  memset(&p, 0, sizeof(p));
  p.N = a.N; p.H = h + 2; p.W = w + 2;
  p.OH = 2 * h; p.OW = 2 * w;
  p.osy = p.osx = 2; p.isy = p.isx = 1;
  p.x = a.xhat; p.ldx = a.ld; p.x_coff = 0;
  p.wp = a.wsets; p.Kc = a.Kc; p.ldw = a.ldw; p.bias = a.bias;
  p.y = a.y; p.ldy = a.ldy; p.y_coff = a.y_coff; p.Cout = a.cout;
  p.act = a.act; p.alpha = a.alpha;
  fill_lane(p, a.lane, 1.f);
  const Layer::SegLaunch& F = *a.tab;
  if (a.split) {
    ConvParams q = p;
    q.OHq = h - 1; q.OWq = w - 1;
    q.ncls = 4;
    for (int c = 0; c < 4; ++c) {
      q.cls_tap[c] = q.ntaps;
      for (int t = F.seg_tap[c]; t < F.seg_tap[c + 1]; ++t) q.taps[q.ntaps++] = F.taps[t];
    }
    q.cls_tap[4] = q.ntaps;
    UDET_TRY(launch_conv(q, s));
    fill_segments(p, F, a.tab_dev, 4);
  } else {
    fill_segments(p, F, a.tab_dev);
  }
  return launch_conv(p, s);
}
int upb_dgrad(const UpbBwd& a, hipStream_t s) {
  const int h = a.h, w = a.w;
  ConvParams p;
  memset(&p, 0, sizeof(p));
  p.N = a.N; p.H = 2 * h; p.W = 2 * w;
  p.OH = h + 2; p.OW = w + 2;
  p.osy = p.osx = 1; p.isy = p.isx = 2;
  fill_segments(p, *a.tab, a.tab_dev);
  p.x = a.du; p.ldx = a.lddu; p.x_coff = a.du_coff;
  p.wp = a.wsetsT; p.Kc = a.KcT; p.ldw = a.ldwT; p.kreal = a.cout;
  p.y = a.dxhat; p.ldy = a.ld; p.y_coff = 0; p.Cout = a.cin;
  fill_lane(p, a.lane, a.f16_xscale);
  UDET_TRY(launch_conv(p, s));
  return launch_upb_ring_fold(a.dxhat, a.ld, a.N, h, w, a.dsrc, s);
}

#define UDET_F16_GRAD_SCALE 4096.f
static void fill_common(Plan* P, ConvParams& p, float* ws, int slot) {
  p.partial = ws + P->scratch_off[slot];
  p.partial_cap = P->scratch_floats;
  p.zero16 = ws + P->small_off + 60000;
  p.tickets = reinterpret_cast<int*>(ws + P->ticket_off) + (size_t)slot * UDET_MAX_TICKETS;
  p.f16 = P->cfg.conv_fp16;
  p.f16_xscale = 1.f;
}

static void bind_x(ConvParams& p, const Buf& b, int coff, float* ws) { p.x = ws + b.off; p.ldx = b.ld; p.x_coff = coff; }
static void bind_y(ConvParams& p, const Buf& b, int coff, int cout, float* ws) { p.y = ws + b.off; p.ldy = b.ld; p.y_coff = coff; p.Cout = cout; }
static void bind_w(ConvParams& p, size_t off, int Kc, int ldw, float* ws) { p.wp = ws + off; p.Kc = Kc; p.ldw = ldw; }
static void bind_res(ConvParams& p, const Buf& b, int coff, float* ws) { p.res = ws + b.off; p.ldres = b.ld; p.res_coff = coff; }
static void bind_y2(ConvParams& p, const Buf& b, float* ws) { p.y2 = ws + b.off; p.ldy2 = b.ld; p.y2_coff = 0; }
static void bind_wino(ConvParams& p, size_t off, int np, float* ws) { p.wino_u = ws + off; p.wino_np = np; }
static void bind_emit(Plan* P, ConvParams& p, const Emit& em, int coff, float* ws) {
  const Buf &bu = P->buf(em.ubuf), &bua = P->buf(em.abuf);
  p.uo = ws + bu.off; p.ldu = bu.ld; p.u_coff = coff;
  p.ua = ws + bua.off; p.ldua = bua.ld; p.ua_coff = coff;
  p.uact = em.act; p.ualpha = em.alpha; p.u_c0 = em.c0; p.u_c1 = em.c1;
}

static UpbLane upb_lane(Plan* P, float* ws, int slot) {
  ConvParams c;
  fill_common(P, c, ws, slot);
  return UpbLane{c.partial, c.partial_cap, c.zero16, c.tickets, c.f16};
}

static int run_fwd_upb(Plan* P, const Layer& L, int N, float* ws, const Lane& ln) {
  hipStream_t s = ln.s;
  const Buf &bs = P->buf(L.src), &bp = P->buf(L.xhat), &by = P->buf(L.y);
  prof_begin(P, PROF_CONV_FWD, layer_flops(L, N) * 9.0 / 16.0, layer_bytes(L, N), s, L.name.c_str());
  UpbFwd a;
  a.N = N; a.h = bs.h; a.w = bs.w;
  a.src = ws + bs.off; a.xhat = ws + bp.off; a.ld = bp.ld;
  a.wsets = ws + L.wupb_off; a.Kc = L.Kc; a.ldw = L.ldw; a.bias = ws + L.bias_f_off;
  a.y = ws + by.off; a.ldy = by.ld; a.y_coff = L.y_coff; a.cout = L.cout;
  a.act = L.act; a.alpha = L.alpha;
  a.tab = &L.upb_f; a.tab_dev = reinterpret_cast<const ConvTap*>(ws + L.upb_f.tab_off); a.split = L.upb_split;
  a.lane = upb_lane(P, ws, ln.slot);
  UDET_TRY(upb_forward(a, s));
  prof_end(P, s);
  return UDET_OK;
}

int run_dgrad_upb(Plan* P, const Layer& L, int N, int du, int dxhat, int dsrc, float* ws, const Lane& ln) {
  hipStream_t s = ln.s;
  if (skip_launch(1, L.net)) return UDET_OK;
  const Buf &bu = P->buf(du), &bp = P->buf(dxhat), &bd = P->buf(dsrc);
  prof_begin(P, PROF_CONV_DGRAD, layer_flops(L, N) * 9.0 / 16.0, layer_bytes(L, N), s, L.name.c_str());
  UpbBwd a;
  a.N = N; a.h = bd.h; a.w = bd.w;
  a.du = ws + bu.off; a.lddu = bu.ld; a.du_coff = L.y_coff;
  a.wsetsT = ws + L.wupbT_off; a.KcT = L.KcT; a.ldwT = L.ldwT; a.cout = L.cout;
  a.dxhat = ws + bp.off; a.dsrc = ws + bd.off; a.ld = bp.ld; a.cin = L.cin;
  a.tab = &L.upb_b; a.tab_dev = reinterpret_cast<const ConvTap*>(ws + L.upb_b.tab_off);
  a.lane = upb_lane(P, ws, ln.slot);
  a.f16_xscale = UDET_F16_GRAD_SCALE;
  UDET_TRY(upb_dgrad(a, s));
  prof_end(P, s);
  return UDET_OK;
}

static bool up_form(const Layer& L) { return L.up && L.wu_off; }
static int fwd_launches(const Layer& L) { return L.transposed ? conv_dgrad_classes(2, 2 * L.H, 2 * L.W) : 1; }
static bool fwd_is_plain(const Layer& L) { return !L.transposed && !L.up && !L.upb && !L.col2im; }
static bool fwd_params(Plan* P, const Layer& L, int N, int cls, float* ws, int slot, ConvParams& p) {
  memset(&p, 0, sizeof(p));
  if (L.transposed) {
    if (!conv_setup_dgrad(p, cls, N, 2 * L.H, 2 * L.W, L.kh, L.kw, 2, 1)) return false;
  } else if (up_form(L)) {
    setup_up_fwd(p, N, L.H, L.W);
  } else {
    conv_setup_fwd(p, N, L.H << (L.up ? 1 : 0), L.W << (L.up ? 1 : 0), L.kh, L.kw, L.stride, L.dil);
    p.up_shift = L.up ? 1 : 0;
  }
  bind_x(p, P->buf(L.x), L.x_coff, ws);
  bind_w(p, up_form(L) ? L.wu_off : L.wp_off, L.Kc, L.ldw, ws); p.bias = ws + L.bias_f_off;
  bind_y(p, P->buf(L.y), L.y_coff, L.cout, ws);
  p.act = L.act; p.alpha = L.alpha;
  if (L.res >= 0) bind_res(p, P->buf(L.res), L.res_coff, ws);
  if (L.y2 >= 0) bind_y2(p, P->buf(L.y2), ws);
  if (L.wino_off) bind_wino(p, L.wino_off, L.wino_np, ws);
  fill_common(P, p, ws, slot);
  return true;
}

int run_fwd(Plan* P, const Layer& L, int N, float* ws, const Lane& ln) {
  hipStream_t s = ln.s;
  if (skip_launch(0, L.net)) return UDET_OK;
  if (L.upb) return run_fwd_upb(P, L, N, ws, ln);
  const Buf &bx = P->buf(L.x), &by = P->buf(L.y);
  prof_begin(P, PROF_CONV_FWD, layer_flops(L, N) * (up_form(L) ? 4.0 / 9.0 : 1.0), layer_bytes(L, N), s, L.name.c_str());
  bool direct_head = false;
  if (L.col2im && !P->cfg.conv_fp16 && L.Kc <= 64) {
    ConvParams q;
    memset(&q, 0, sizeof(q));
    if (L.transposed) (void)conv_setup_dgrad(q, 0, N, 2 * L.H, 2 * L.W, L.kh, L.kw, 2, 1);
    else conv_setup_fwd(q, N, L.H, L.W, L.kh, L.kw, L.stride, L.dil);
    q.Kc = L.Kc; q.ldw = L.ldw; q.Cout = L.cout;
    if (q.ncls != 4) { q.ncls = 1; q.cls_tap[0] = 0; q.cls_tap[1] = q.ntaps; }
    direct_head = conv_thin_n_ok(q);
  }
  if (L.col2im && !direct_head && fwd_launches(L) == 1) {
    const Buf& bz = P->buf(L.zbuf);
    ConvParams p;
    memset(&p, 0, sizeof(p));
    conv_setup_fwd(p, N, L.H, L.W, 1, 1, 1, 1);
    bind_x(p, bx, L.x_coff, ws);
    bind_w(p, L.wz_off, L.Kc, L.ldz, ws);
    bind_y(p, bz, 0, L.kh * L.kw * L.cout, ws);
    fill_common(P, p, ws, ln.slot);
    UDET_TRY(launch_conv(p, s));
    ConvParams g;
    memset(&g, 0, sizeof(g));
    if (L.transposed) conv_setup_dgrad(g, 0, N, 2 * L.H, 2 * L.W, L.kh, L.kw, 2, 1);
    else conv_setup_fwd(g, N, L.H, L.W, L.kh, L.kw, 1, 1);
    g.H = L.H; g.W = L.W;
    g.bias = ws + L.bias_f_off;
    bind_y(g, by, L.y_coff, L.cout, ws);
    UDET_TRY(launch_tap_gather(g, ws + bz.off, bz.ld, s));
    prof_end(P, s);
    return UDET_OK;
  }
  for (int cls = 0; cls < fwd_launches(L); ++cls) {
    ConvParams p;
    if (!fwd_params(P, L, N, cls, ws, ln.slot, p)) continue;
    UDET_TRY(launch_conv(p, s));
    if (P->profiling && (conv_last_config() & 0xff) == FAM_WINO) P->prof.back()->mfma_scale = 4.0 / 9.0;
  }
  prof_end(P, s);
  return UDET_OK;
}

static bool up_form_T(const Layer& L) { return L.up && L.wuT_off; }
static int dgrad_launches(const Layer& L) { return up_form_T(L) ? 1 : conv_dgrad_classes(L.stride, L.H << (L.up ? 1 : 0), L.W << (L.up ? 1 : 0)); }
static bool dgrad_is_plain(const Layer& L) { return !L.up && !L.upb && !L.transposed && dgrad_launches(L) == 1; }
static bool dgrad_params(Plan* P, const Layer& L, int N, int cls, int dy, bool dy_is_du, int dx, int dx_coff, int accumulate, int res,
                         const Emit& em, float* ws, int slot, ConvParams& p) {
  const int up = L.up ? 1 : 0;
  memset(&p, 0, sizeof(p));
  if (up_form_T(L)) setup_up_dgrad(p, N, L.H, L.W);
  else if (!conv_setup_dgrad(p, cls, N, L.H << up, L.W << up, L.kh, L.kw, L.stride, L.dil)) return false;
  bind_x(p, P->buf(dy), L.y_coff, ws);
  if (L.act != ACT_NONE && !dy_is_du) { p.xa = ws + P->buf(L.y2 >= 0 ? L.y2 : L.y).off; p.xact = L.act; p.xalpha = L.alpha; }
  bind_w(p, up_form_T(L) ? L.wuT_off : L.wpT_off, L.KcT, L.ldwT, ws); p.kreal = L.cout;
  bind_y(p, P->buf(dx), dx_coff, L.cin, ws);
  p.accumulate = accumulate;
  if (res >= 0) bind_res(p, P->buf(res), 0, ws);
  if (em.ubuf >= 0) bind_emit(P, p, em, dx_coff, ws);
  if (L.winoT_off && !up_form_T(L)) bind_wino(p, L.winoT_off, L.winoT_np, ws);
  fill_common(P, p, ws, slot);
  p.f16_xscale = UDET_F16_GRAD_SCALE;
  return true;
}

int run_dgrad(Plan* P, const Layer& L, int N, int dy, bool dy_is_du, int dx, int dx_coff, int accumulate, int res, const Emit& em, float* ws,
              const Lane& ln) {
  hipStream_t s = ln.s;
  if (skip_launch(1, L.net)) return UDET_OK;
  const Buf &bdy = P->buf(dy), &ba = P->buf(L.y2 >= 0 ? L.y2 : L.y);
  if (ba.ld != bdy.ld) {
    set_error("dgrad(%s): gradient/activation layout mismatch (%d vs %d)", L.name.c_str(), bdy.ld, ba.ld);
    return UDET_ERR_SHAPE;
  }
  prof_begin(P, PROF_CONV_DGRAD, layer_flops(L, N) * (up_form_T(L) ? 4.0 / 9.0 : 1.0), layer_bytes(L, N), s, L.name.c_str());
  for (int cls = 0; cls < dgrad_launches(L); ++cls) {
    ConvParams p;
    if (!dgrad_params(P, L, N, cls, dy, dy_is_du, dx, dx_coff, accumulate, res, em, ws, ln.slot, p)) continue;
    UDET_TRY(launch_conv(p, s));
    if (P->profiling && (conv_last_config() & 0xff) == FAM_WINO) P->prof.back()->mfma_scale = 4.0 / 9.0;
  }
  prof_end(P, s);
  return UDET_OK;
}

int run_wgrad(Plan* P, const Layer& L, int N, int dy, bool dy_is_du, const float* w_flat, float* g_flat, float* ws, const Lane& ln) {
  hipStream_t s = ln.s;
  if (skip_launch(2, L.net)) return UDET_OK;
  const NetParams& np = net_params(L.net);
  const int act_buf = L.y2 >= 0 ? L.y2 : L.y;
  const Buf &bx = P->buf(L.x), &bdy = P->buf(dy), &ba = P->buf(act_buf);
  const int up = L.up ? 1 : 0;
  ConvParams g;
  memset(&g, 0, sizeof(g));
  conv_setup_fwd(g, N, L.H << up, L.W << up, L.kh, L.kw, L.stride, L.dil);
  WgradParams q;
  memset(&q, 0, sizeof(q));
  q.x = ws + bx.off; q.ldx = bx.ld; q.x_coff = L.x_coff;
  q.N = N; q.H = L.H << up; q.W = L.W << up; q.up_shift = up; q.Cin = L.cin;
  q.dy = ws + bdy.off; q.ldy = bdy.ld; q.y_coff = L.y_coff; q.Cout = L.cout;
  if (L.act != ACT_NONE && !dy_is_du) { q.ya = ws + ba.off; q.yact = L.act; q.yalpha = L.alpha; }
  q.OH = g.OH; q.OW = g.OW; q.isy = q.isx = L.stride;
  q.ntaps = g.ntaps;
  memcpy(q.taps, g.taps, sizeof(g.taps));
  q.dw = g_flat + np.p[L.w_idx].offset;
  q.db = g_flat + np.p[L.b_idx].offset;
  q.partial = ws + P->wgrad_off[ln.slot];
  q.zero16 = ws + P->small_off + 60000;
  q.partial_floats = P->wgrad_floats;
  q.f16 = P->cfg.conv_fp16;
  q.f16_yscale = UDET_F16_GRAD_SCALE;
  if (L.g_idx >= 0) {
    q.w = w_flat + np.p[L.w_idx].offset;
    q.b = w_flat + np.p[L.b_idx].offset;
    q.gamma = w_flat + np.p[L.g_idx].offset;
    q.dgamma = g_flat + np.p[L.g_idx].offset;
    q.dbeta = g_flat + np.p[L.be_idx].offset;
    q.bn_c = BN_C;
  }
  if (L.up && L.wu_off && L.g_idx >= 0 && dy_is_du) {
    prof_begin(P, PROF_CONV_WGRAD, layer_flops(L, N) * 4.0 / 9.0, layer_bytes(L, N), s, L.name.c_str());
    const int rc = launch_wgrad_up_T(q, L.H, L.W, s);
    prof_end(P, s);
    return rc;
  }
  prof_begin(P, PROF_CONV_WGRAD, layer_flops(L, N), layer_bytes(L, N), s, L.name.c_str());
  const int rc = launch_wgrad_T(q, L.kh * L.kw, s);
  if (P->profiling && (wgrad_last_config() >> 20) == 3) P->prof.back()->mfma_scale = 4.0 / 9.0;
  prof_end(P, s);
  return rc;
}

int run_fwd_pair(Plan* P, const Layer& La, int Na, const Layer& Lb, int Nb, float* ws, const Lane& ln) {
  if (!pairs_on(P) || !fwd_is_plain(La) || !fwd_is_plain(Lb)) {
    UDET_TRY(run_fwd(P, La, Na, ws, ln));
    return run_fwd(P, Lb, Nb, ws, ln);
  }
  if (skip_launch(0, La.net)) return UDET_OK;
  ConvParams a, b;
  fwd_params(P, La, Na, 0, ws, ln.slot, a);
  fwd_params(P, Lb, Nb, 0, ws, ln.slot, b);
  a.wino_u = b.wino_u = nullptr; a.wino_np = b.wino_np = 0;
  prof_begin(P, PROF_CONV_FWD, layer_flops(La, Na) + layer_flops(Lb, Nb), layer_bytes(La, Na) + layer_bytes(Lb, Nb), ln.s, La.pair_name.c_str());
  const int rc = launch_conv_pair(a, b, ln.s);
  prof_end(P, ln.s);
  return rc;
}
int run_dgrad_pair(Plan* P, const DgradJob& ja, const DgradJob& jb, float* ws, const Lane& ln) {
  ConvParams a, b;
  auto one_launch = [&](const DgradJob& j, ConvParams& p) {
    return dgrad_is_plain(*j.L) && dgrad_params(P, *j.L, j.N, 0, j.dy, true, j.dx, j.dx_coff, j.accumulate, -1, j.em, ws, ln.slot, p);
  };
  if (!pairs_on(P, 1) || !one_launch(ja, a) || !one_launch(jb, b)) {
    UDET_TRY(run_dgrad(P, *ja.L, ja.N, ja.dy, true, ja.dx, ja.dx_coff, ja.accumulate, -1, ja.em, ws, ln));
    return run_dgrad(P, *jb.L, jb.N, jb.dy, true, jb.dx, jb.dx_coff, jb.accumulate, -1, jb.em, ws, ln);
  }
  if (skip_launch(1, ja.L->net)) return UDET_OK;
  a.wino_u = b.wino_u = nullptr;
  prof_begin(P, PROF_CONV_DGRAD, layer_flops(*ja.L, ja.N) + layer_flops(*jb.L, jb.N), layer_bytes(*ja.L, ja.N) + layer_bytes(*jb.L, jb.N), ln.s,
             ja.L->pair_name.c_str());
  const int rc = launch_conv_pair(a, b, ln.s);
  prof_end(P, ln.s);
  return rc;
}

}
```

unsupervised_detection_amd/csrc/plan_run.h:

```cpp
#pragma once
#include "plan.h"

namespace udet {

static const float BN_C = 0.99950037468777316f;

struct Lane {
  hipStream_t s;
  int slot;
};
Lane lane_of(Plan* P, hipStream_t main, int i);
hipEvent_t next_event(Plan* P);
void order_after(Plan* P, const Lane& from, const Lane& to);

struct Emit {
  int ubuf = -1, abuf = -1, c0 = 0, c1 = 0, act = ACT_NONE;
  float alpha = 0.f;
};
struct DgradJob {
  const Layer* L;
  int N, dy, dx, dx_coff, accumulate;
  Emit em;
};
inline bool pairs_on(const Plan* P, int dir = 0) { return !P->cfg.conv_fp16 && !((plan_knob(UDET_KNOB_NO_PAIRS) >> dir) & 1); }
int run_fwd(Plan* P, const Layer& L, int N, float* ws, const Lane& ln);
int run_fwd_pair(Plan* P, const Layer& La, int Na, const Layer& Lb, int Nb, float* ws, const Lane& ln);
int run_dgrad(Plan* P, const Layer& L, int N, int dy, bool dy_is_du, int dx, int dx_coff, int accumulate, int res, const Emit& em, float* ws,
              const Lane& ln);
int run_dgrad_pair(Plan* P, const DgradJob& ja, const DgradJob& jb, float* ws, const Lane& ln);
int run_dgrad_upb(Plan* P, const Layer& L, int N, int du, int dxhat, int dsrc, float* ws, const Lane& ln);
int run_wgrad(Plan* P, const Layer& L, int N, int dy, bool dy_is_du, const float* w_flat, float* g_flat, float* ws, const Lane& ln);
struct UpbLane {
  float* partial;
  size_t partial_cap;
  const float* zero16;
  int* tickets;
  int f16;
};
struct UpbFwd {
  int N, h, w;
  const float* src;
  float* xhat;
  int ld;
  const float* wsets;
  int Kc, ldw;
  const float* bias;
  float* y;
  int ldy, y_coff, cout, act;
  float alpha;
  const Layer::SegLaunch* tab;
  const ConvTap* tab_dev;
  bool split;
  UpbLane lane;
};
struct UpbBwd {
  int N, h, w;
  const float* du;
  int lddu, du_coff;
  const float* wsetsT;
  int KcT, ldwT, cout;
  float* dxhat;
  float* dsrc;
  int ld, cin;
  const Layer::SegLaunch* tab;
  const ConvTap* tab_dev;
  float f16_xscale;
  UpbLane lane;
};
int upb_forward(const UpbFwd& a, hipStream_t s);
int upb_dgrad(const UpbBwd& a, hipStream_t s);

}
```

unsupervised_detection_amd/csrc/plan_step.hip:

```cpp
#include "conv_host.h"
#include "elementwise.h"
#include "plan_run.h"

namespace udet {

static const int PWC_CH[7] = {0, 16, 32, 64, 96, 128, 196};
static const char* const WARP_NAME[7] = {"", "", "warp_costvol2", "warp_costvol3", "warp_costvol4", "warp_costvol5", "warp_costvol6"};

static int pwc_forward_on(Plan* P, const float* img1, const float* img2, float* ws, const Lane& L0, const Lane& LH) {
  if (!P->pwc_packed) {
    set_error("pwc_forward: call udet_pack_pwc first");
    return UDET_ERR_ARG;
  }
  const Config& c = P->cfg;
  const Resolved& R = P->R;
  const int B = c.batch;
  hipStream_t s = L0.s;
  auto fwd = [&](int layer, int N, const Lane& ln) { return run_fwd(P, P->pwc[layer], N, ws, ln); };
  UDET_TRY(launch_pack_pwc_input(img1, img2, ws + P->buf(R.pwc_x8).off, (long)B * c.in_h * c.in_w, s));
  for (int l = 1; l <= 6; ++l)
    for (int j = 0; j < 3; ++j) UDET_TRY(fwd(R.pwc.pyr[l][j], 2 * B, L0));
  for (int l = 6; l >= 2; --l) {
    const int h = c.in_h >> l, w = c.in_w >> l, C = PWC_CH[l];
    const Buf& cb = P->buf(R.pwc_c[l]);
// ... 40 lines not shown

int plan_prefetch(Plan* P, const float* img1, const float* img2, float* ws, hipStream_t s) {
  const Lane L0 = lane_of(P, s, 0), LC = lane_of(P, s, 4), LH = lane_of(P, s, 5);
  P->in_prefetch = true;
  P->ev_next_prefetch = 0;
  order_after(P, L0, LC);
  int rc = pwc_forward_on(P, img1, img2, ws, LC, LH);
  P->in_prefetch = false;
  UDET_TRY(rc);
  UDET_TRY(plan_prepare_flow(P, P->R.flow_next, ws, LC.s));
  UDET_TRY(plan_prepare_image(P, img1, P->R.image_next, ws, LC.s));
  if (!P->prefetch_ev) (void)hipEventCreateWithFlags(&P->prefetch_ev, hipEventDisableTiming);
  (void)hipEventRecord(P->prefetch_ev, LC.s);
  P->prefetch_pending = true;
  return UDET_OK;
}

int plan_generator_forward(Plan* P, float* ws, hipStream_t s) {
  const Config& c = P->cfg;
  const long HW = (long)c.img_h * c.img_w;
  const Lane L0 = lane_of(P, s, 0);
  double* part = reinterpret_cast<double*>(ws + P->small_off + 4096);
  UDET_TRY(launch_gen_input(ws + P->buf(P->R.image).off, ws + P->buf(P->R.flow).off, part, ws + P->buf(P->R.gen_in).off, c.batch, HW, s));
  for (const auto& L : P->gen) UDET_TRY(run_fwd(P, L, c.batch, ws, L0));
  return UDET_OK;
}
int plan_generator_layers(Plan* P, float* ws, hipStream_t s) {
  const Lane L0 = lane_of(P, s, 0);
  for (const auto& L : P->gen) UDET_TRY(run_fwd(P, L, P->cfg.batch, ws, L0));
  return UDET_OK;
}

static int rec_resize(Plan* P, int src, int dst, int N, float* ws, hipStream_t s) {
  const Buf &a = P->buf(src), &b = P->buf(dst);
  return launch_resize_bilinear_fwd(ws + a.off, a.ld, 0, N, a.h, a.w, ws + b.off, b.ld, 0, b.h, b.w, a.ld, 1.f, 1.f, s);
}
static int dec_src(const Resolved& R, int k) { return k == 5 ? R.rec_conv6 : R.rec_concat[k + 1]; }

static int share_enc_a_output(Plan* P, const Layer& L, int ncalls, float* ws, hipStream_t s) {
  const Buf& y = P->buf(L.y);
  if (ncalls > 1 && L.y_fanned_out) return launch_share_samples(ws + y.off, (long)P->cfg.batch * y.h * y.w, y.ld, L.y_coff, L.cout, ncalls, s);
  return UDET_OK;
}
static int plan_rec_image_branch(Plan* P, int ncalls, float* ws, const Lane& ln, bool with_layers = true) {
  const Config& c = P->cfg;
  if (ncalls < 1) return UDET_OK;
  const long Ppix = (long)c.batch * c.img_h * c.img_w;
  UDET_TRY(launch_pack_imgin(ws + P->buf(P->R.image).off, ws + P->buf(P->R.rec_imgin).off, Ppix, 1, ln.s));
  if (!with_layers) return UDET_OK;
  for (int i = 0; i < 9; ++i) {
    const Layer& L = P->rec[P->R.rec.enc[0][i]];
    UDET_TRY(run_fwd(P, L, c.batch, ws, ln));
    UDET_TRY(share_enc_a_output(P, L, ncalls, ws, ln.s));
  }
  P->enc_a_shared = true;
  return UDET_OK;
}

int plan_recover_forward(Plan* P, int ncalls, float* ws, hipStream_t s, bool inputs_prepacked, bool skip_enc_a, bool enc_a_input_packed) {
  const Config& c = P->cfg;
  const Resolved& R = P->R;
  const int B = c.batch, N = ncalls * B;
  const long Ppix = (long)B * c.img_h * c.img_w;
  const Lane L0 = lane_of(P, s, 0);
  if (!inputs_prepacked)
    UDET_TRY(launch_mask_rec_inputs(ws + P->buf(R.gen_a17).off, ws + P->buf(R.flow).off, ws + P->buf(R.mask).off, ws + P->buf(R.rec_fin).off,
                                    Ppix, ncalls, s));
  if (ncalls < 1) return UDET_OK;
  auto enc = [&](int e, int i) -> const Layer& { return P->rec[R.rec.enc[e][i]]; };
  if (!skip_enc_a && pairs_on(P)) {
    if (!inputs_prepacked && !enc_a_input_packed) UDET_TRY(plan_rec_image_branch(P, ncalls, ws, L0, false));
    for (int i = 0; i < 9; ++i) {
      const Layer& La = enc(0, i);
      UDET_TRY(run_fwd_pair(P, La, inputs_prepacked ? N : B, enc(1, i), N, ws, L0));
      if (!inputs_prepacked) UDET_TRY(share_enc_a_output(P, La, ncalls, ws, s));
    }
    P->enc_a_shared = !inputs_prepacked;
  } else {
    if (!skip_enc_a) {
      if (inputs_prepacked) {
        for (int i = 0; i < 9; ++i) UDET_TRY(run_fwd(P, enc(0, i), N, ws, L0));
        P->enc_a_shared = false;
      } else {
        UDET_TRY(plan_rec_image_branch(P, ncalls, ws, L0));
      }
    }
    for (int i = 0; i < 9; ++i) UDET_TRY(run_fwd(P, enc(1, i), N, ws, L0));
  }
  for (int k = 5; k >= 1; --k) {
    const Layer& dcl = P->rec[R.rec.deconv[k]];
    if (!dcl.upb) UDET_TRY(rec_resize(P, dec_src(R, k), R.rec_r[k + 1], N, ws, s));
    UDET_TRY(run_fwd(P, dcl, N, ws, L0));
    if (k < 5) {
      UDET_TRY(rec_resize(P, R.rec_flow[k + 1], R.rec_rf[k + 1], N, ws, s));
      UDET_TRY(run_fwd(P, P->rec[R.rec.upflow[k]], N, ws, L0));
    }
    UDET_TRY(run_fwd(P, P->rec[R.rec.flow[k]], N, ws, L0));
  }
  const Buf& f1 = P->buf(R.rec_flow[1]);
  return launch_resize_bilinear_fwd(ws + f1.off, f1.ld, 0, N, f1.h, f1.w, ws + P->buf(R.pred).off, 2, 0, c.img_h, c.img_w, 2, 1.f, 1.f, s);
}

int plan_losses(Plan* P, float* ws, hipStream_t s) {
  const Config& c = P->cfg;
  float* sm = ws + P->small_off;
  const long HW = (long)c.img_h * c.img_w;
  return launch_losses(ws + P->buf(P->R.flow).off, ws + P->buf(P->R.mask).off, ws + P->buf(P->R.pred).off, HW,
                       c.batch, c.cbn, c.epsilon, (float)(c.img_w * c.img_h * c.batch), sm + 8192, sm, sm + 16, sm + UDET_SMALL_SUMS, s);
}

int plan_prefetch_consume(Plan* P, float* ws, hipStream_t s) {
  if (!P->prefetch_pending) {
    set_error("forward_prefetched: no udet_prefetch_flow is pending");
    return UDET_ERR_ARG;
  }
  (void)hipStreamWaitEvent(s, P->prefetch_ev, 0);
  P->prefetch_pending = false;
  const Buf &fn = P->buf(P->R.flow_next), &in = P->buf(P->R.image_next);
  UDET_HIP(hipMemcpyAsync(ws + P->buf(P->R.flow).off, ws + fn.off, fn.floats() * sizeof(float), hipMemcpyDeviceToDevice, s));
  UDET_HIP(hipMemcpyAsync(ws + P->buf(P->R.image).off, ws + in.off, in.floats() * sizeof(float), hipMemcpyDeviceToDevice, s));
  return UDET_OK;
}

int plan_forward(Plan* P, const float* img1, const float* img2, int ncalls, float* ws, hipStream_t s, bool prefetched) {
  P->ev_next = 0;
  const Lane L0 = lane_of(P, s, 0), LI = lane_of(P, s, 1);
  if (prefetched) {
    UDET_TRY(plan_prefetch_consume(P, ws, s));
    img1 = img2 = nullptr;
  } else if (img1 && P->prefetch_pending) {
    (void)hipStreamWaitEvent(s, P->prefetch_ev, 0);
  }
  order_after(P, L0, LI);
  if (img1) UDET_TRY(plan_prepare_image(P, img1, P->R.image, ws, LI.s));
  hipEvent_t e_img = nullptr;
  if (LI.s != L0.s) {
    e_img = next_event(P);
    (void)hipEventRecord(e_img, LI.s);
  }
  const bool paired = pairs_on(P);
  UDET_TRY(plan_rec_image_branch(P, ncalls, ws, LI, !paired));
  if (img1) {
    UDET_TRY(pwc_forward_on(P, img1, img2, ws, L0, lane_of(P, s, 2)));
    UDET_TRY(plan_prepare_flow(P, P->R.flow, ws, s));
  }
  if (e_img) (void)hipStreamWaitEvent(s, e_img, 0);
  UDET_TRY(plan_generator_forward(P, ws, s));
  order_after(P, LI, L0);
  UDET_TRY(plan_recover_forward(P, ncalls, ws, s, false, !paired, paired));
  if (ncalls == 3) UDET_TRY(plan_losses(P, ws, s));
  return UDET_OK;
}

static int rec_backward(Plan* P, int N, const Resolved::Grad& G, bool with_wgrad, bool need_dfin, const float* w_rec, float* g_rec, float* ws,
                        const Lane& LD, const Lane& LW, const Lane* LAp = nullptr, const Lane* LWdecp = nullptr) {
  const Config& c = P->cfg;
  const Resolved& R = P->R;
  hipStream_t s = LD.s;
  const Lane LWdec = LWdecp ? *LWdecp : LW;
  auto wgrad_on = [&](const Lane& lw, const Layer& L, int dy, bool is_du, int n) -> int {
    order_after(P, LD, lw);
    return run_wgrad(P, L, n < 0 ? N : n, dy, is_du, w_rec, g_rec, ws, lw);
  };
  auto wgrad = [&](const Layer& L, int dy, bool is_du, int n = -1) -> int { return wgrad_on(LW, L, dy, is_du, n); };
  auto wgrad_dec = [&](const Layer& L, int dy, bool is_du) -> int { return wgrad_on(LWdec, L, dy, is_du, -1); };
  const Lane LA = LAp ? *LAp : LD;
  const bool a_own_lane = LA.s != LD.s;
  const int ncopies = N / c.batch;
  const bool a_shared = P->enc_a_shared && ncopies > 1;
  const Emit none;
  const float LEAK = 0.2f;
  {
    const Buf& df1 = P->buf(G.flow[1]);
    UDET_TRY(launch_resize_bilinear_bwd(ws + P->buf(G.pred).off, 2, 0, N, c.img_h, c.img_w, ws + df1.off, df1.ld, 0, df1.h, df1.w, 2, 0, s));
  }
  for (int k = 1; k <= 5; ++k) {
    const int dconcat = G.concat[k], uconcat = G.u_concat[k];
    const Layer* fl = &P->rec[R.rec.flow[k]];
    const Layer* dc = &P->rec[R.rec.deconv[k]];
    Emit em;
    em.ubuf = uconcat; em.abuf = fl->x; em.c0 = 0; em.c1 = dc->cout; em.act = ACT_LEAKY; em.alpha = LEAK;
    UDET_TRY(run_dgrad(P, *fl, N, G.flow[k], false, dconcat, 0, k == 1 ? 0 : 1, -1, em, ws, LD));
    if (with_wgrad) UDET_TRY(wgrad_dec(*fl, G.flow[k], false));
    if (k < 5) {
      const Layer* uf = &P->rec[R.rec.upflow[k]];
      if (with_wgrad) UDET_TRY(wgrad_dec(*uf, dconcat, false));
      UDET_TRY(run_dgrad(P, *uf, N, dconcat, false, G.rf[k + 1], 0, 0, -1, none, ws, LD));
      const Buf &drf = P->buf(G.rf[k + 1]), &dfn = P->buf(G.flow[k + 1]);
      UDET_TRY(launch_resize_bilinear_bwd(ws + drf.off, drf.ld, 0, N, drf.h, drf.w, ws + dfn.off, dfn.ld, 0, dfn.h, dfn.w, drf.ld, 0, s));
    }
    if (with_wgrad) {
      if (dc->upb) {
        order_after(P, LD, LWdec);
        UDET_TRY(rec_resize(P, dec_src(R, k), R.rec_r[k + 1], N, ws, LWdec.s));
      }
      UDET_TRY(wgrad_dec(*dc, uconcat, true));
    }
    if (dc->upb_bwd) {
      UDET_TRY(run_dgrad_upb(P, *dc, N, uconcat, G.p[k + 1], G.concat[k + 1], ws, LD));
      continue;
    }
    const int dr = G.r[k + 1];
    UDET_TRY(run_dgrad(P, *dc, N, uconcat, true, dr, 0, 0, -1, none, ws, LD));
    const Buf& bdr = P->buf(dr);
    const Buf& dsrc = P->buf(k == 5 ? G.conv6 : G.concat[k + 1]);
    UDET_TRY(launch_resize_bilinear_bwd(ws + bdr.off, bdr.ld, 0, N, bdr.h, bdr.w, ws + dsrc.off, dsrc.ld, 0, dsrc.h, dsrc.w,
                                        bdr.ld, 0, s));
  }
  {
    const Buf &d6 = P->buf(G.conv6), &a6 = P->buf(R.rec_conv6), &u6 = P->buf(G.u_conv6);
    UDET_TRY(launch_emit_du(ws + d6.off, ws + a6.off, ws + u6.off, (long)N * d6.h * d6.w, d6.ld, 0, d6.ld, ACT_LEAKY, LEAK, s));
  }
  if (a_own_lane) order_after(P, LD, LA);
  const bool pair_enc = pairs_on(P, 1) && with_wgrad && !a_own_lane;
  for (int i = 8; i >= 0; --i) {
    DgradJob job[2];
    int njob = 0;
    for (int e = 0; e < 2; ++e) {
      if (e == 0 && !with_wgrad) continue;
      const Layer* L = &P->rec[R.rec.enc[e][i]];
      const int du = G.enc_du[e][i];
      const bool shared = e == 0 && a_shared;
      const int Ne = shared ? c.batch : N;
      const bool own = e == 0 && a_own_lane;
      const Lane& LE = own ? LA : LD;
      hipStream_t se = LE.s;
      if (shared && i == 8) {
        const Buf& u = P->buf(du);
        UDET_TRY(launch_fold_samples(ws + u.off, (long)c.batch * u.h * u.w, u.ld, L->y_coff, L->cout, ncopies, se));
      }
      if (with_wgrad) {
        if (own) UDET_TRY(run_wgrad(P, *L, Ne, du, true, w_rec, g_rec, ws, LA));
        else UDET_TRY(wgrad(*L, du, true, Ne));
      }
      if (i == 0) {
        if (e == 1 && need_dfin) UDET_TRY(run_dgrad(P, *L, N, du, true, G.fin, 0, 0, -1, none, ws, LD));
        continue;
      }
      const int dx = G.enc_dx[e][i];
      const bool slab_in = L->x_in_slab;
      Emit em;
      em.ubuf = G.enc_ux[e][i]; em.abuf = L->x; em.c0 = 0; em.c1 = L->cin; em.act = ACT_LEAKY; em.alpha = LEAK;
      if (shared && slab_in) {
        const Buf& d = P->buf(dx);
        UDET_TRY(launch_fold_samples(ws + d.off, (long)c.batch * d.h * d.w, d.ld, L->x_coff, L->cin, ncopies, se));
      }
      if (pair_enc) {
        job[njob].L = L; job[njob].N = Ne; job[njob].dy = du; job[njob].dx = dx; job[njob].dx_coff = L->x_coff;
        job[njob].accumulate = slab_in ? 1 : 0; job[njob].em = em;
        ++njob;
        continue;
      }
      UDET_TRY(run_dgrad(P, *L, Ne, du, true, dx, L->x_coff, slab_in ? 1 : 0, -1, em, ws, LE));
    }
    if (njob == 2) UDET_TRY(run_dgrad_pair(P, job[0], job[1], ws, LD));
    else if (njob == 1) UDET_TRY(run_dgrad(P, *job[0].L, job[0].N, job[0].dy, true, job[0].dx, job[0].dx_coff, job[0].accumulate, -1, job[0].em, ws, LD));
  }
  if (a_own_lane) order_after(P, LA, LD);
  if (with_wgrad && LWdec.s != LW.s) order_after(P, LWdec, LD);
  return UDET_OK;
}

static int backward_recover(Plan* P, const float* w_rec, float* g_rec, float* ws, const Lane& LD, const Lane& LW, const Lane* LA = nullptr,
                            const Lane* LWdec = nullptr) {
  const Config& c = P->cfg;
  const Resolved& R = P->R;
  const long BHW = (long)c.batch * c.img_h * c.img_w;
  UDET_TRY(launch_rec_loss_bwd(ws + P->buf(R.flow).off, ws + P->buf(R.mask).off, ws + P->buf(R.pred).off, ws + P->buf(R.grad[0].pred).off, BHW,
                               c.cbn, 1.0f / (float)(c.img_w * c.img_h * c.batch), LD.s));
  return rec_backward(P, 3 * c.batch, R.grad[0], true, false, w_rec, g_rec, ws, LD, LW, LA, LWdec);
}

static int backward_generator(Plan* P, const float* w_gen, float* g_gen, float* ws, const Lane& LD, const Lane& LW, const Lane* LWlate = nullptr,
                              int nlate = 0) {
  const Config& c = P->cfg;
  const Resolved& R = P->R;
  const int B = c.batch;
  const long HW = (long)c.img_h * c.img_w;
  hipStream_t s = LD.s;
  float* sm = ws + P->small_off;
  UDET_TRY(launch_gen_loss_bwd(ws + P->buf(R.flow).off, ws + P->buf(R.mask).off, ws + P->buf(R.pred).off, sm + 16,
                               ws + P->buf(R.grad[1].pred).off, ws + P->buf(R.d_mask).off, HW, B, c.cbn, s));
  UDET_TRY(rec_backward(P, 2 * B, R.grad[1], false, true, nullptr, nullptr, ws, LD, LD));
  UDET_TRY(launch_mask_bwd(ws + P->buf(R.d_mask).off, ws + P->buf(R.grad[1].fin).off, ws + P->buf(R.flow).off, ws + P->buf(R.mask).off,
                           ws + P->buf(R.gen_d[17]).off, B * HW, s));
  for (int i = 16; i >= 0; --i) {
    const Layer& L = P->gen[i];
    const bool has_act = L.act != ACT_NONE;
    const int dy = has_act ? R.gen_u[i + 1] : R.gen_d[i + 1];
    const Lane& LWi = (LWlate && i < nlate) ? *LWlate : LW;
    order_after(P, LD, LWi);
    UDET_TRY(run_wgrad(P, L, B, dy, has_act, w_gen, g_gen, ws, LWi));
    if (i == 0) break;
    const int res = i == 6 ? R.gen_d[11] : (i == 3 ? R.gen_d[14] : (i == 1 ? R.gen_d[15] : -1));
    const int dx = R.gen_d[i];
    const Layer& Lp = P->gen[i - 1];
    const int ap = Lp.y2 >= 0 ? Lp.y2 : Lp.y;
    {
      Emit em;
      if (Lp.act != ACT_NONE) { em.ubuf = R.gen_u[i]; em.abuf = ap; em.c0 = 0; em.c1 = L.cin; em.act = Lp.act; em.alpha = Lp.alpha; }
      UDET_TRY(run_dgrad(P, L, B, dy, has_act, dx, 0, 0, res, em, ws, LD));
    }
  }
  return UDET_OK;
}

int plan_backward(Plan* P, int which, const float* w_gen, const float* w_rec, float* g_gen, float* g_rec, float* ws, hipStream_t s) {
  P->ev_next = 0;
  const Lane L0 = lane_of(P, s, 0), L1 = lane_of(P, s, 1), L2 = lane_of(P, s, 2), L3 = lane_of(P, s, 3);
  auto mark = [&](int net) {
    if (!P->grad_ev[net]) (void)hipEventCreateWithFlags(&P->grad_ev[net], hipEventDisableTiming);
    (void)hipEventRecord(P->grad_ev[net], s);
  };
  if (which == 3) {
    order_after(P, L0, L1);
    const int la = (int)plan_knob(UDET_KNOB_ENC_A_LANE);
    const Lane LA = lane_of(P, s, la > 0 && la < Plan::NLANE ? la : 0);
    const int lw = (int)plan_knob(UDET_KNOB_REC_DEC_WGRAD_LANE), le = (int)plan_knob(UDET_KNOB_REC_ENC_WGRAD_LANE);
    const Lane LWD = lane_of(P, s, lw > 0 && lw < Plan::NLANE ? lw : 3);
    const Lane LWE = lane_of(P, s, le > 0 && le < Plan::NLANE ? le : 2);
    UDET_TRY(backward_recover(P, w_rec, g_rec, ws, L0, LWE, la > 0 ? &LA : nullptr, &LWD));
    if (LWE.s != L2.s) order_after(P, LWE, L0);
    const long kl = plan_knob(UDET_KNOB_GEN_WGRAD_LATE);
    const int nlate = kl > 0 ? (int)kl : (kl < 0 ? 0 : 4);
    order_after(P, L2, L0);
    mark(NET_REC);
    UDET_TRY(backward_generator(P, w_gen, g_gen, ws, L1, L3, nlate > 0 ? &L2 : nullptr, nlate));
    order_after(P, L2, L0);
    order_after(P, L1, L0);
    order_after(P, L3, L0);
    mark(NET_GEN);
  } else if (which == 2) {
    UDET_TRY(backward_recover(P, w_rec, g_rec, ws, L0, L2, nullptr, &L3));
    order_after(P, L2, L0);
    mark(NET_REC);
  } else {
    UDET_TRY(backward_generator(P, w_gen, g_gen, ws, L0, L3));
    order_after(P, L3, L0);
    mark(NET_GEN);
  }
  return UDET_OK;
}

}
```

Measured before the change: 501.0.

## Skip dgrad output channel blocks for encoder-A skip segments when no wgrad

When the recovery-network backward pass runs without weight gradients, the input gradients flowing into encoder A's skip-connection channels are not needed. The change adds a column-skip range to the conv parameters, shrinks the grid's channel dimension, and remaps block indices so those output-channel blocks are never computed. It also skips them in the split-K reduce. Pairing and tuning are disabled or neutralised when a skip is active, and a debug mask can turn trimming off. The risk is wrong results if a skipped range is actually consumed downstream, or a partially covered block at the range edges.

Result: no change. 503.5 (median of 6 runs) (+0.5%).

```diff
diff --git a/include/udet_debug.h b/include/udet_debug.h
--- a/include/udet_debug.h
+++ b/include/udet_debug.h
@@ -15,6 +15,7 @@
                                          float* dgamma, float* dbeta, int n, int h, int wd, int cin, int cout, int k, int stride, int dilation,
                                          int up, void* workspace, size_t workspace_bytes, void* stream);
 void udet_debug_upb_min_pixels(long v);
+void udet_debug_rec_trim(int mask);
 void udet_debug_set_tuning(int on);
 void udet_debug_force_pair(int on);
 int udet_debug_last_pair(void);
diff --git a/unsupervised_detection_amd/_devel.py b/unsupervised_detection_amd/_devel.py
--- a/unsupervised_detection_amd/_devel.py
+++ b/unsupervised_detection_amd/_devel.py
@@ -21,6 +21,8 @@
 dbg.udet_debug_force_wgrad.argtypes = [ctypes.c_int, ctypes.c_int]
 dbg.udet_debug_upb_min_pixels.restype = None
 dbg.udet_debug_upb_min_pixels.argtypes = [ctypes.c_long]
+dbg.udet_debug_rec_trim.restype = None
+dbg.udet_debug_rec_trim.argtypes = [ctypes.c_int]
 dbg.udet_debug_set_tuning.restype = None
 dbg.udet_debug_set_tuning.argtypes = [ctypes.c_int]
 dbg.udet_debug_last_wgrad.restype = ctypes.c_int
diff --git a/unsupervised_detection_amd/csrc/common.h b/unsupervised_detection_amd/csrc/common.h
--- a/unsupervised_detection_amd/csrc/common.h
+++ b/unsupervised_detection_amd/csrc/common.h
@@ -156,7 +156,10 @@
   const float* wino_u;
   int wino_np;
   int kreal;
-};
+  int skip_c0, skip_c1;
+  int nskip_b0, nskip_nb, nskip_lo, nskip_hi;
+};
+__device__ __forceinline__ int conv_nblock(const ConvParams& p) { return (int)blockIdx.y + ((int)blockIdx.y >= p.nskip_b0 ? p.nskip_nb : 0); }
 #define UDET_MAX_TICKETS 4096
 
 int launch_conv(ConvParams& p, hipStream_t stream);
diff --git a/unsupervised_detection_amd/csrc/conv_igemm.hip b/unsupervised_detection_amd/csrc/conv_igemm.hip
--- a/unsupervised_detection_amd/csrc/conv_igemm.hip
+++ b/unsupervised_detection_amd/csrc/conv_igemm.hip
@@ -20,7 +20,7 @@
 
 static int launch_cfg(ConvParams& p, const ConvCfg& c, hipStream_t stream) {
   const int Mtot = p.N * p.OHq * p.OWq;
-  dim3 grid(conv_xblocks(p, c.bm), (p.Cout + c.bn - 1) / c.bn, p.ksplit > 1 ? p.ksplit : 1);
+  dim3 grid(conv_xblocks(p, c.bm), (p.Cout + c.bn - 1) / c.bn - p.nskip_nb, p.ksplit > 1 ? p.ksplit : 1);
   if (p.tail_ks > 1) {
     const int mtiles = (Mtot + c.bm - 1) / c.bm;
     p.tail_prow0 = (p.tail_full / mtiles) * Mtot + (p.tail_full % mtiles) * c.bm;
@@ -71,6 +71,7 @@
   for (ConvParams* q : {&a, &b}) {
     q->ksplit = ks; q->fold = 0; q->tail_full = 0; q->tail_ks = 0; q->tail_prow0 = 0;
     q->ldp = (q->Cout + 3) & ~3;
+    q->nskip_b0 = q->nskip_nb = q->nskip_lo = q->nskip_hi = 0;
   }
   float* const base = a.partial;
   if (ks > 1) {
diff --git a/unsupervised_detection_amd/csrc/conv_igemm_ring.h b/unsupervised_detection_amd/csrc/conv_igemm_ring.h
--- a/unsupervised_detection_amd/csrc/conv_igemm_ring.h
+++ b/unsupervised_detection_amd/csrc/conv_igemm_ring.h
@@ -59,7 +59,7 @@
   }
   const TileCls tc = tile_cls<BM>(p, bid);
   const int OHWq = tc.OHWq, Mtot = tc.Mtot , m0 = tc.m0, tap0 = tc.tap0, ntc = tc.ntc, ooy = tc.ooy, oox = tc.oox;
-  const int n0 = blockIdx.y * BN;
+  const int n0 = conv_nblock(p) * BN;
   const int Hs = p.H >> p.up_shift, Ws = p.W >> p.up_shift;
   IGEMM_STAMP(6);
 
diff --git a/unsupervised_detection_amd/csrc/conv_igemm_self.hip b/unsupervised_detection_amd/csrc/conv_igemm_self.hip
--- a/unsupervised_detection_amd/csrc/conv_igemm_self.hip
+++ b/unsupervised_detection_amd/csrc/conv_igemm_self.hip
@@ -27,7 +27,7 @@
   const int bid = xcd_tile_order(blockIdx.x, gridDim.x);
   const TileCls tc = tile_cls<BM>(p, bid);
   const int Mtot = tc.Mtot , m0 = tc.m0, ntc = tc.ntc;
-  const int n0 = blockIdx.y * BN;
+  const int n0 = conv_nblock(p) * BN;
   const int Hs = p.H >> p.up_shift, Ws = p.W >> p.up_shift;
 
   fill_tap_tables<256>(p, tc, tap_yx, tap_w, t);
diff --git a/unsupervised_detection_amd/csrc/conv_igemm_staged.hip b/unsupervised_detection_amd/csrc/conv_igemm_staged.hip
--- a/unsupervised_detection_amd/csrc/conv_igemm_staged.hip
+++ b/unsupervised_detection_amd/csrc/conv_igemm_staged.hip
@@ -39,7 +39,7 @@
   }
   const TileCls tc = tile_cls<BM>(p, bid);
   const int OHWq = tc.OHWq, Mtot = tc.Mtot , m0 = tc.m0, tap0 = tc.tap0, ntc = tc.ntc, ooy = tc.ooy, oox = tc.oox;
-  const int n0 = blockIdx.y * BN;
+  const int n0 = conv_nblock(p) * BN;
   const int Hs = p.H >> p.up_shift, Ws = p.W >> p.up_shift;
 
   for (int i = tid; i < ntc; i += NT) {
diff --git a/unsupervised_detection_amd/csrc/conv_select.hip b/unsupervised_detection_amd/csrc/conv_select.hip
--- a/unsupervised_detection_amd/csrc/conv_select.hip
+++ b/unsupervised_detection_amd/csrc/conv_select.hip
@@ -71,7 +71,18 @@
   return c;
 }
 
+static void set_nskip(ConvParams& p, int bn) {
+  p.nskip_b0 = p.nskip_nb = p.nskip_lo = p.nskip_hi = 0;
+  if (bn <= 0 || p.skip_c1 <= p.skip_c0 || p.skip_c0 < 0) return;
+  const int nblk = (p.Cout + bn - 1) / bn;
+  const int b0 = (p.skip_c0 + bn - 1) / bn, b1 = p.skip_c1 >= p.Cout ? nblk : p.skip_c1 / bn;
+  if (b1 <= b0 || b1 - b0 >= nblk) return;
+  p.nskip_b0 = b0; p.nskip_nb = b1 - b0;
+  p.nskip_lo = b0 * bn; p.nskip_hi = b1 * bn < p.Cout ? b1 * bn : p.Cout;
+}
+
 int run_conv_cfg(ConvParams& p, const ConvCfg& c, hipStream_t stream) {
+  set_nskip(p, c.family == FAM_THIN_K ? 64 : (c.family == FAM_TILE ? (p.Cout <= 16 ? 0 : 32) : (is_gemm(c.family) ? c.bn : 0)));
   if (is_direct(c.family)) {
     p.ksplit = 1; p.fold = 0; p.tail_full = 0; p.tail_ks = 0;
     return c.family == FAM_THIN_K ? launch_conv_thin_k(p, stream) : launch_conv_thin_n(p, stream);
@@ -225,7 +236,10 @@
   const uint64_t key = conv_key(p);
   if (!conv_cache_find(key, &c)) {
     if (conv_tuning_on()) {
+      const int s0 = p.skip_c0, s1 = p.skip_c1;
+      p.skip_c0 = p.skip_c1 = 0;
       c = tune_conv(p, key, stream);
+      p.skip_c0 = s0; p.skip_c1 = s1;
     } else {
       c = heuristic_cfg(p);
       if (!g_force.bm && !p.f16 && conv_thin_n_ok(p)) c.family = FAM_THIN_N;
@@ -244,6 +258,7 @@
 int conv_last_pair() { return g_last_pair; }
 static bool pair_compatible(const ConvParams& a, const ConvParams& b) {
   if (a.nseg || b.nseg || a.f16 || b.f16 || a.up_shift || b.up_shift || !dma_ok(a) || !dma_ok(b)) return false;
+  if (a.skip_c1 > a.skip_c0 || b.skip_c1 > b.skip_c0) return false;
   if (a.Kc != b.Kc || a.Cout != b.Cout || a.ldw != b.ldw || a.ntaps != b.ntaps || a.ncls != b.ncls) return false;
   if (a.isy != b.isy || a.isx != b.isx || a.osy != b.osy || a.osx != b.osx || a.kfast != b.kfast) return false;
   if (!a.partial || a.partial != b.partial) return false;
diff --git a/unsupervised_detection_amd/csrc/conv_splitk.hip b/unsupervised_detection_amd/csrc/conv_splitk.hip
--- a/unsupervised_detection_amd/csrc/conv_splitk.hip
+++ b/unsupervised_detection_amd/csrc/conv_splitk.hip
@@ -9,6 +9,7 @@
   const int sl = threadIdx.x % SL;
   for (long e = ((long)blockIdx.x * 256 + threadIdx.x) / SL; e < total; e += (long)gridDim.x * (256 / SL)) {
     const int ma = (int)(e / p.Cout), n = (int)(e - (long)ma * p.Cout);
+    if (n >= p.nskip_lo && n < p.nskip_hi) continue;
     float v = 0.f;
     const float* src = p.partial + (size_t)ma * p.ldp + n;
     const size_t slab = (size_t)Mall * p.ldp;
@@ -37,6 +38,7 @@
   const bool vec = epilogue4_out_ok(p);
   for (long e = (long)bid * 256 + threadIdx.x; e < total; e += (long)grid * 256) {
     const int mr = (int)(e / nq), n = (int)(e - (long)mr * nq) * 4;
+    if (n >= p.nskip_lo && n < p.nskip_hi) continue;
     const float4 v = splitk_sum4<load4_plain>(p.partial + (size_t)mr * p.ldp + n, slab, ksplit);
     const int off = row_pixel_off(p, row0 + mr);
     if (vec) {
diff --git a/unsupervised_detection_amd/csrc/conv_thin.hip b/unsupervised_detection_amd/csrc/conv_thin.hip
--- a/unsupervised_detection_amd/csrc/conv_thin.hip
+++ b/unsupervised_detection_amd/csrc/conv_thin.hip
@@ -302,7 +302,7 @@
   const int oy0 = by * TH, ox0 = bx * TW;
   const int iy0 = oy0 + g.min_dy, ix0 = ox0 + g.min_dx;
   const float* xb = p.x + (size_t)n * p.H * p.W * p.ldx + p.x_coff;
-  const int co = blockIdx.y * 64 + lane;
+  const int co = conv_nblock(p) * 64 + lane;
   float w[T][2];
   int toff[T];
 #pragma unroll
@@ -362,7 +362,7 @@
   const int oy0 = by * TH, ox0 = bx * TW;
   const int iy0 = oy0 + g.min_dy, ix0 = ox0 + g.min_dx;
   const float* xb = p.x + (size_t)n * p.H * p.W * p.ldx + p.x_coff;
-  const int co = blockIdx.y * 64 + lane;
+  const int co = conv_nblock(p) * 64 + lane;
   float w[T][2];
 #pragma unroll
   for (int i = 0; i < T; ++i) {
@@ -438,7 +438,7 @@
   ThinGeom g;
   thin_geom(p, 8, 16, &g);
   const size_t lds = (size_t)g.PH * g.PW * sizeof(float2);
-  const dim3 grid(p.N * ((p.OHq + 7) / 8) * ((p.OWq + 15) / 16), (p.Cout + 63) / 64);
+  const dim3 grid(p.N * ((p.OHq + 7) / 8) * ((p.OWq + 15) / 16), (p.Cout + 63) / 64 - p.nskip_nb);
   int kh = 0, kw = 0;
   ThinWin win;
   if (thin_window(p, g, &kh, &kw, &win)) {
diff --git a/unsupervised_detection_amd/csrc/conv_tile.hip b/unsupervised_detection_amd/csrc/conv_tile.hip
--- a/unsupervised_detection_amd/csrc/conv_tile.hip
+++ b/unsupervised_detection_amd/csrc/conv_tile.hip
@@ -64,7 +64,7 @@
   const int bid = blockIdx.x;
   const int tx = bid % tiles_x, ty = (bid / tiles_x) % tiles_y, n = bid / (tiles_x * tiles_y);
   const int oy0 = ty * TH, ox0 = tx * TW;
-  const int n0 = blockIdx.y * NW;
+  const int n0 = conv_nblock(p) * NW;
   const int iy0 = oy0 * p.isy + g.min_dy, ix0 = ox0 * p.isx + g.min_dx;
   const int Hs = p.H >> p.up_shift, Ws = p.W >> p.up_shift;
   const float* xb = p.x + (size_t)n * Hs * Ws * p.ldx + p.x_coff;
@@ -405,7 +405,7 @@
   const int tiles = ((p.OWq + 31) / 32) * ((p.OHq + th - 1) / th) * p.N;
   const int ncls = p.ncls > 1 ? p.ncls : 1;
   const bool n16 = p.Cout <= 16;
-  dim3 grid(tiles, n16 ? 1 : (p.Cout + 31) / 32, ncls);
+  dim3 grid(tiles, n16 ? 1 : (p.Cout + 31) / 32 - p.nskip_nb, ncls);
   if (p.f16) {
     static const Kern K16[2][2][2] = {
         {{conv_tile_kernel<8, 32, TILE_MT_SMALL, TILE_MW_SMALL, true>, conv_tile_kernel<8, 32, TILE_MT_BIG, TILE_MW_BIG, true>},
diff --git a/unsupervised_detection_amd/csrc/devel/api_debug.hip b/unsupervised_detection_amd/csrc/devel/api_debug.hip
--- a/unsupervised_detection_amd/csrc/devel/api_debug.hip
+++ b/unsupervised_detection_amd/csrc/devel/api_debug.hip
@@ -70,6 +70,7 @@
   return launch_wgrad_T(p, k * k, stream);
 }
 void udet_debug_upb_min_pixels(long v) { plan_debug_upb_min_pixels(v); }
+void udet_debug_rec_trim(int mask) { plan_debug_rec_trim(mask); }
 void udet_debug_force_pair(int on) { conv_force_pair(on); }
 int udet_debug_last_pair(void) { return conv_last_pair(); }
 int udet_debug_conv2d_pair(const float* xa, const float* xb, const float* wa, const float* wb, const float* ba, const float* bb, float* ya, float* yb,
diff --git a/unsupervised_detection_amd/csrc/plan.h b/unsupervised_detection_amd/csrc/plan.h
--- a/unsupervised_detection_amd/csrc/plan.h
+++ b/unsupervised_detection_amd/csrc/plan.h
@@ -160,6 +160,7 @@
 #define UDET_SMALL_SUMS 1024
 Plan* plan_build(const Config& cfg);
 void plan_debug_upb_min_pixels(long v);
+void plan_debug_rec_trim(int mask);
 void build_upb_launches(Layer& L, int h, int w);
 void upb_pack_jobs(const Layer& L, const PackJob& base, std::vector<PackJob>& jobs);
 enum { UDET_KNOB_ENC_A_LANE = 0, UDET_KNOB_REC_DEC_WGRAD_LANE = 1, UDET_KNOB_REC_ENC_WGRAD_LANE = 2, UDET_KNOB_GEN_WGRAD_LATE = 3, UDET_KNOB_NO_WGRAD_WINO = 6, UDET_KNOB_SKIP = 7, UDET_KNOB_NO_PAIRS = 8, UDET_KNOB_COUNT = 12 };
diff --git a/unsupervised_detection_amd/csrc/plan_exec.hip b/unsupervised_detection_amd/csrc/plan_exec.hip
--- a/unsupervised_detection_amd/csrc/plan_exec.hip
+++ b/unsupervised_detection_amd/csrc/plan_exec.hip
@@ -111,6 +111,7 @@
   p.wp = a.wsetsT; p.Kc = a.KcT; p.ldw = a.ldwT; p.kreal = a.cout;
   p.y = a.dxhat; p.ldy = a.ld; p.y_coff = 0; p.Cout = a.cin;
   fill_lane(p, a.lane, a.f16_xscale);
+  p.skip_c0 = a.skip_c0; p.skip_c1 = a.skip_c1;
   UDET_TRY(launch_conv(p, s));
   return launch_upb_ring_fold(a.dxhat, a.ld, a.N, h, w, a.dsrc, s);
 }
@@ -161,7 +162,7 @@
   return UDET_OK;
 }
 
-int run_dgrad_upb(Plan* P, const Layer& L, int N, int du, int dxhat, int dsrc, float* ws, const Lane& ln) {
+int run_dgrad_upb(Plan* P, const Layer& L, int N, int du, int dxhat, int dsrc, float* ws, const Lane& ln, const ColSkip& skip) {
   hipStream_t s = ln.s;
   if (skip_launch(1, L.net)) return UDET_OK;
   const Buf &bu = P->buf(du), &bp = P->buf(dxhat), &bd = P->buf(dsrc);
@@ -174,6 +175,7 @@
   a.tab = &L.upb_b; a.tab_dev = reinterpret_cast<const ConvTap*>(ws + L.upb_b.tab_off);
   a.lane = upb_lane(P, ws, ln.slot);
   a.f16_xscale = UDET_F16_GRAD_SCALE;
+  a.skip_c0 = skip.c0; a.skip_c1 = skip.c1;
   UDET_TRY(upb_dgrad(a, s));
   prof_end(P, s);
   return UDET_OK;
@@ -273,7 +275,7 @@
 }
 
 int run_dgrad(Plan* P, const Layer& L, int N, int dy, bool dy_is_du, int dx, int dx_coff, int accumulate, int res, const Emit& em, float* ws,
-              const Lane& ln) {
+              const Lane& ln, const ColSkip& skip) {
   hipStream_t s = ln.s;
   if (skip_launch(1, L.net)) return UDET_OK;
   const Buf &bdy = P->buf(dy), &ba = P->buf(L.y2 >= 0 ? L.y2 : L.y);
@@ -285,6 +287,7 @@
   for (int cls = 0; cls < dgrad_launches(L); ++cls) {
     ConvParams p;
     if (!dgrad_params(P, L, N, cls, dy, dy_is_du, dx, dx_coff, accumulate, res, em, ws, ln.slot, p)) continue;
+    p.skip_c0 = skip.c0; p.skip_c1 = skip.c1;
     UDET_TRY(launch_conv(p, s));
     if (P->profiling && (conv_last_config() & 0xff) == FAM_WINO) P->prof.back()->mfma_scale = 4.0 / 9.0;
   }
diff --git a/unsupervised_detection_amd/csrc/plan_run.h b/unsupervised_detection_amd/csrc/plan_run.h
--- a/unsupervised_detection_amd/csrc/plan_run.h
+++ b/unsupervised_detection_amd/csrc/plan_run.h
@@ -17,6 +17,9 @@
   int ubuf = -1, abuf = -1, c0 = 0, c1 = 0, act = ACT_NONE;
   float alpha = 0.f;
 };
+struct ColSkip {
+  int c0 = 0, c1 = 0;
+};
 struct DgradJob {
   const Layer* L;
   int N, dy, dx, dx_coff, accumulate;
@@ -26,9 +29,9 @@
 int run_fwd(Plan* P, const Layer& L, int N, float* ws, const Lane& ln);
 int run_fwd_pair(Plan* P, const Layer& La, int Na, const Layer& Lb, int Nb, float* ws, const Lane& ln);
 int run_dgrad(Plan* P, const Layer& L, int N, int dy, bool dy_is_du, int dx, int dx_coff, int accumulate, int res, const Emit& em, float* ws,
-              const Lane& ln);
+              const Lane& ln, const ColSkip& skip = ColSkip());
 int run_dgrad_pair(Plan* P, const DgradJob& ja, const DgradJob& jb, float* ws, const Lane& ln);
-int run_dgrad_upb(Plan* P, const Layer& L, int N, int du, int dxhat, int dsrc, float* ws, const Lane& ln);
+int run_dgrad_upb(Plan* P, const Layer& L, int N, int du, int dxhat, int dsrc, float* ws, const Lane& ln, const ColSkip& skip = ColSkip());
 int run_wgrad(Plan* P, const Layer& L, int N, int dy, bool dy_is_du, const float* w_flat, float* g_flat, float* ws, const Lane& ln);
 struct UpbLane {
   float* partial;
@@ -65,6 +68,7 @@
   const Layer::SegLaunch* tab;
   const ConvTap* tab_dev;
   float f16_xscale;
+  int skip_c0 = 0, skip_c1 = 0;
   UpbLane lane;
 };
 int upb_forward(const UpbFwd& a, hipStream_t s);
diff --git a/unsupervised_detection_amd/csrc/plan_step.hip b/unsupervised_detection_amd/csrc/plan_step.hip
--- a/unsupervised_detection_amd/csrc/plan_step.hip
+++ b/unsupervised_detection_amd/csrc/plan_step.hip
@@ -216,6 +216,8 @@
   return UDET_OK;
 }
 
+static int g_rec_trim_off = 0;
+void plan_debug_rec_trim(int mask) { g_rec_trim_off = mask; }
 static int rec_backward(Plan* P, int N, const Resolved::Grad& G, bool with_wgrad, bool need_dfin, const float* w_rec, float* g_rec, float* ws,
                         const Lane& LD, const Lane& LW, const Lane* LAp = nullptr, const Lane* LWdecp = nullptr) {
   const Config& c = P->cfg;
@@ -234,6 +236,14 @@
   const bool a_shared = P->enc_a_shared && ncopies > 1;
   const Emit none;
   const float LEAK = 0.2f;
+  const bool trim_a = !with_wgrad && !(g_rec_trim_off & 1);
+  auto a_segment = [&](int k) {
+    static const int A_AT_LEVEL[7] = {-1, 0, 1, 3, 5, 7, 8};
+    const Layer& La = P->rec[R.rec.enc[0][A_AT_LEVEL[k]]];
+    ColSkip sk;
+    if (trim_a) { sk.c0 = La.y_coff; sk.c1 = La.y_coff + La.cout; }
+    return sk;
+  };
   {
     const Buf& df1 = P->buf(G.flow[1]);
     UDET_TRY(launch_resize_bilinear_bwd(ws + P->buf(G.pred).off, 2, 0, N, c.img_h, c.img_w, ws + df1.off, df1.ld, 0, df1.h, df1.w, 2, 0, s));
@@ -244,7 +254,7 @@
     const Layer* dc = &P->rec[R.rec.deconv[k]];
     Emit em;
     em.ubuf = uconcat; em.abuf = fl->x; em.c0 = 0; em.c1 = dc->cout; em.act = ACT_LEAKY; em.alpha = LEAK;
-    UDET_TRY(run_dgrad(P, *fl, N, G.flow[k], false, dconcat, 0, k == 1 ? 0 : 1, -1, em, ws, LD));
+    UDET_TRY(run_dgrad(P, *fl, N, G.flow[k], false, dconcat, 0, k == 1 ? 0 : 1, -1, em, ws, LD, a_segment(k)));
     if (with_wgrad) UDET_TRY(wgrad_dec(*fl, G.flow[k], false));
     if (k < 5) {
       const Layer* uf = &P->rec[R.rec.upflow[k]];
@@ -261,11 +271,11 @@
       UDET_TRY(wgrad_dec(*dc, uconcat, true));
     }
     if (dc->upb_bwd) {
-      UDET_TRY(run_dgrad_upb(P, *dc, N, uconcat, G.p[k + 1], G.concat[k + 1], ws, LD));
+      UDET_TRY(run_dgrad_upb(P, *dc, N, uconcat, G.p[k + 1], G.concat[k + 1], ws, LD, a_segment(k + 1)));
       continue;
     }
     const int dr = G.r[k + 1];
-    UDET_TRY(run_dgrad(P, *dc, N, uconcat, true, dr, 0, 0, -1, none, ws, LD));
+    UDET_TRY(run_dgrad(P, *dc, N, uconcat, true, dr, 0, 0, -1, none, ws, LD, a_segment(k + 1)));
     const Buf& bdr = P->buf(dr);
     const Buf& dsrc = P->buf(k == 5 ? G.conv6 : G.concat[k + 1]);
     UDET_TRY(launch_resize_bilinear_bwd(ws + bdr.off, bdr.ld, 0, N, bdr.h, bdr.w, ws + dsrc.off, dsrc.ld, 0, dsrc.h, dsrc.w,
```
